# microsoft/aurora

Hardware: AMD Instinct MI355X
Metric: forecast-steps/sec (6h step) 0.25deg ERA5 721x1440x13 (higher is better)
Workload: dtype bf16; 1 GPU; AuroraPretrained(autocast=True) 1.3B, 0.25deg ERA5 721x1440, 13 levels, T=2, batch 1 per GPU, one forward step (BASELINE.json configs[1]); parallelism=1 GPU

## Files before the change

### aurora_amd/build.py

```python

from __future__ import annotations

import os
import subprocess
import sys
from pathlib import Path

PKG = Path(__file__).resolve().parent
CSRC = PKG / "csrc"
LIB = PKG / "_lib" / "libaurora_hip.so"
SOURCES = ("runtime.hip", "gemm.hip", "gemm_f32.hip", "gemm_ln512.hip", "gemm_a4.hip", "attention.hip", "norm.hip", "embed.hip", "perceiver_attention.hip", "perceiver_out.hip", "band.hip",
           "model.hip", "model_weights.hip", "model_grid.hip", "step.hip", "regrid.hip", "conservative_regrid.hip", "planes.hip", "scores.hip", "ensemble_scores.hip", "ensemble_quantiles.hip", "spectra.hip", "event_scores.hip",
           "field_stats.hip", "probability_scores.hip", "diagnostics.hip", "conditional_scores.hip", "region_scores.hip", "objects.hip", "field_quantiles.hip", "object_matches.hip", "nearest_event.hip")
ARCH = "gfx950"
COMPILE_FLAGS = (f"--offload-arch={ARCH}", "-O3", "-std=c++17", "-fPIC", "-mllvm", "-amdgpu-mfma-vgpr-form=1")


def _hipcc() -> str:
    for cand in (os.environ.get("HIPCC"), "/opt/rocm/bin/hipcc", "hipcc"):
        if cand and (os.path.isabs(cand) and os.path.exists(cand) or not os.path.isabs(cand)):
            return cand
    raise RuntimeError("hipcc not found")


def is_stale() -> bool:
    if not LIB.exists():
        return True
    built = LIB.stat().st_mtime
    deps = [d for pat in ("*.hip", "*.h", "*.inc") for d in CSRC.glob(pat)] + [PKG.parent / "include" / "aurora_hip.h"]
    return any(d.stat().st_mtime > built for d in deps)


def build_library(force: bool = False, verbose: bool = True) -> Path:
    if not force and not is_stale():
        return LIB
    LIB.parent.mkdir(parents=True, exist_ok=True)
    objs = []
    procs = []
    for src in SOURCES:
        obj = LIB.parent / (src.replace(".hip", ".o"))
        cmd = [_hipcc(), *COMPILE_FLAGS, *os.environ.get("AURORA_BUILD_FLAGS", "").split(), "-c", str(CSRC / src), "-o", str(obj)]
        if verbose:
            print(" ".join(cmd), flush=True)
        procs.append((src, subprocess.Popen(cmd, stdout=subprocess.PIPE, stderr=subprocess.STDOUT)))
        objs.append(obj)
    for src, pr in procs:
        out, _ = pr.communicate()
        if pr.returncode != 0:
            raise RuntimeError(f"hipcc failed on {src}:\n{out.decode(errors='replace')}")
    cmd = [_hipcc(), f"--offload-arch={ARCH}", "-shared", "-fPIC", *map(str, objs), "-o", str(LIB)]
    if verbose:
        print(" ".join(cmd), flush=True)
    res = subprocess.run(cmd, stdout=subprocess.PIPE, stderr=subprocess.STDOUT)
    if res.returncode != 0:
        raise RuntimeError(f"link failed:\n{res.stdout.decode(errors='replace')}")
    for o in objs:
        o.unlink(missing_ok=True)
    return LIB


if __name__ == "__main__":
    print(build_library(force="--force" in sys.argv))
```

### aurora_amd/csrc/model.h

```cpp
#pragma once

#include <math.h>
#include <stdlib.h>
#include <string.h>

#include <algorithm>
#include <array>
#include <exception>
#include <map>
#include <memory>
#include <stdexcept>
#include <string>
#include <vector>

#include "band.h"
#include "common.h"

namespace aurora {

struct Fail {
  int code;
};
#define REQUIRE(cond, ...)               \
  do {                                   \
    if (!(cond)) {                       \
      ::aurora::set_error(__VA_ARGS__);  \
      throw ::aurora::Fail{AURORA_E_ARG}; \
    }                                    \
  } while (0)
#define GUARDED(...)                                    \
  try {                                                 \
    __VA_ARGS__;                                        \
    return AURORA_OK;                                   \
  } catch (const ::aurora::Fail& f) {                   \
    return f.code;                                      \
  } catch (const std::exception& e) {                   \
    ::aurora::set_error("internal error: %s", e.what()); \
    return AURORA_E_LAUNCH;                             \
  }
inline void ok(int code) {
  if (code != AURORA_OK) throw Fail{code};
}
inline void hip_ok(hipError_t e, const char* what) {
  if (e != hipSuccess) {
    set_error("%s: %s", what, hipGetErrorString(e));
    throw Fail{AURORA_E_LAUNCH};
  }
}
inline int round_up(int x, int m) { return (x + m - 1) / m * m; }

struct DevBuf {
  void* p = nullptr;
  size_t bytes = 0;
  DevBuf() = default;
  explicit DevBuf(size_t n) : bytes(n) { hip_ok(hipMalloc(&p, n ? n : 16), "hipMalloc"); }
  DevBuf(const DevBuf&) = delete;
  DevBuf& operator=(const DevBuf&) = delete;
  DevBuf(DevBuf&& o) noexcept : p(o.p), bytes(o.bytes) { o.p = nullptr; }
  DevBuf& operator=(DevBuf&& o) noexcept {
    if (this != &o) {
      if (p) (void)hipFree(p);
      p = o.p; bytes = o.bytes; o.p = nullptr;
    }
    return *this;
  }
  ~DevBuf() { if (p) (void)hipFree(p); }
  float* f() const { return static_cast<float*>(p); }
};

struct Arena {
  char* base = nullptr;
  size_t cap = 0, top = 0, peak = 0;
  void* take(size_t bytes) {
    const size_t at = (top + 255) & ~size_t(255);
    top = at + bytes;
    if (top > peak) peak = top;
    return base + at;
  }
  ~Arena() { if (base) (void)hipFree(base); }
};

struct Tensor {
  DevBuf buf;
  std::vector<int64_t> shape;
  int64_t numel = 0;
  float* f() const { return buf.f(); }
};

struct Block {
  std::string prefix;
  int dim, stage, heads, hidden;
  bool shifted;
  const float *gain1, *shift1, *gain2, *shift2;
  const float *qkv_b, *proj_b, *fc1_b, *fc2_b;
  const void *fc1_w, *fc2_w;
};
struct AttnSet { std::vector<DevBuf> own; std::vector<const void*> qkv, proj; };
struct Resampler {
  struct Layer {
    const float *to_q, *to_kv, *to_out, *fc1_w, *fc1_b, *fc2_w, *fc2_b, *ln1_w, *ln1_b, *ln2_w, *ln2_b;
    const float *ln_k_w = nullptr, *ln_k_b = nullptr, *ln_q_w = nullptr, *ln_q_b = nullptr;
    int inner, head_dim, hidden, dim, ctx_dim;
    float v_l1;
    int f16_mode;
    const void *to_kv_s = nullptr, *to_out_s = nullptr, *fc1_s = nullptr, *fc2_s = nullptr;
  };
  std::vector<Layer> layers;
  std::vector<DevBuf> own;
  DevBuf vs_w, vs_ws;
  int n_s = 0, n_vs = 0, vs_lq = 0;
};

enum SrcKind { SRC_SURF, SRC_STATIC, SRC_DYN, SRC_ATMOS };
struct Channel {
  std::string name;
  SrcKind kind;
  int src;
  int transform;
  float tw0 = 0.f, tw1 = 0.f, tb = 0.f;
};
struct EmbedPack {
  DevBuf w, ws;
  int K = 0, Kpad = 0, groups = 1;
  float l1 = 0.f;
  std::vector<int> channels;
};
struct HeadGroup {
  std::vector<std::string> names;
  DevBuf w, b;
  int groups = 1;
  DevBuf ws, bs;
  int n_pad = 0;
};

struct DevTables { DevBuf tok, grp; int n_windows = 0, n_tok = 0; bool has_grp = false; };
struct DevPlan {
  DevBuf tok, grp, send_idx;
  int n_windows = 0, n_tok = 0, n_own = 0, n_halo = 0, n_interior = 0;
  int recv_off[2] = {0, 0}, recv_cnt[2] = {0, 0}, send_cnt[2] = {0, 0};
  bool has_grp = false;
};

}

struct aurora_hip_model {
  int D = 0, P = 0, Cl = 0, perceiver_heads = 0, n_stages = 0;
  int enc_depths[4] = {0}, dec_depths[4] = {0}, enc_heads[4] = {0}, dec_heads[4] = {0}, window[3] = {0};
  int enc_depth = 1, dec_depth = 1, max_history = 2, lora_steps = 40, lora_mode = 0;
  bool stabilise = false, use_lora = false, autocast = false;
  float ln_eps = 1e-5f;
  double timestep_hours = 6;
  std::vector<std::string> surf_vars, static_vars, atmos_vars;
  int variant = 0;
  bool dynamic_vars = false, atmos_static_vars = false, clamp_first = false, index_bug = false;
  std::vector<double> level_condition;
  std::vector<std::string> sep_perceiver, mod_heads, pos_surf, pos_atmos, surf_inputs, density_vars, angle_vars;
  std::map<std::string, int> diff_index;
  std::vector<aurora::Channel> surf_channels, atmos_channels;
  std::vector<std::string> surf_heads, surf_out;
  std::vector<std::string> atmos_heads;

  std::map<std::string, aurora::Tensor> w;
  std::map<std::string, aurora::Tensor> w16;
  bool finalized = false;
  std::vector<aurora::Block> blocks;
  aurora::DevBuf mod, lead_emb, enc_q0;
  std::vector<aurora::DevBuf> keep;
  std::map<int, aurora::AttnSet> attn_sets;
  struct Merge { const void* w; const float *ln_w, *ln_b; };
  struct Split { const void *w1, *w2; const float *ln_w, *ln_b; };
  std::vector<Merge> merges;
  std::vector<Split> splits;
  aurora::Resampler enc_rs, dec_rs, dec_rs_alt;
  bool has_alt = false;

  bool have_grid = false;
  int n_lat = 0, n_lon = 0, Hp = 0, Wp = 0, n_levels = 0;
  int full_Hp = 0;
  std::vector<double> levels;
  aurora::DevBuf pos_scale, enc_bias, dec_queries, dec_q, dec_q_alt, stats;
  std::vector<size_t> surf_stat_off, static_stat_off, atmos_stat_off;
  size_t one_stat_off = 0;
  std::vector<size_t> static_lvl_stat_off;
  std::vector<double> static_loc;
  std::map<std::array<int64_t, 3>, aurora::EmbedPack> embed_packs;
  float enc_bias_max = 0.f;
  aurora::DevBuf surf_w0_s, surf_w2_s;
  float surf_l1_0 = 0.f, surf_b0 = 0.f, surf_c = 0.f;
  bool surf_chain = false;
  aurora::HeadGroup head_surf, head_main, head_alt;
  float dec_out_bound = 0.f, dec_out_bound_alt = 0.f;
  std::map<std::pair<int, int>, aurora::DevTables> tables;
  std::vector<aurora::Res> stage_res;
  std::vector<std::array<int, 2>> merge_pad;

  aurora_hip_band band{0, 1, nullptr, nullptr, nullptr};
  std::vector<std::vector<std::array<int, 2>>> rows;
  std::map<std::pair<int, int>, aurora::DevPlan> plans;
  void* stage_send = nullptr;
  void* stage_recv = nullptr;
  int64_t staging_bytes = 0, staging_need = 0;
  bool sharded() const { return band.world > 1; }
  int fuse_ln = 1;
  bool split_attention = false;
  bool qkv_planes = true;
  bool reassoc_out = true;
  bool score_weights = true;

  aurora::DevBuf abs_enc, dyn_planes, ctx_max;
  aurora::DevBuf tickets;
  bool split_k = true;
  int abs_B = 0;
  struct Pinned { float* host = nullptr; size_t bytes = 0; hipEvent_t done = nullptr; };
  Pinned pinned[4];
  int pinned_next = 0;
  ~aurora_hip_model() {
    for (auto& t : timed) { (void)hipEventDestroy(t.e0); (void)hipEventDestroy(t.e1); }
    for (auto& e : event_pool) (void)hipEventDestroy(e);
    for (auto& s : pinned) {
      if (s.host) (void)hipHostFree(s.host);
      if (s.done) (void)hipEventDestroy(s.done);
    }
  }
  aurora::Arena arena;
  bool dry = false;
  int64_t generation = 0;

  struct Timed { int kind; double work; hipEvent_t e0, e1; };
  uint32_t profile_mask = 0;
  std::vector<Timed> timed;
  std::vector<hipEvent_t> event_pool;

  const float* W(const std::string& name) const {
    auto it = w.find(name);
    REQUIRE(it != w.end(), "missing weight '%s'", name.c_str());
    return it->second.f();
  }
  const aurora::Tensor& T_(const std::string& name) const {
    auto it = w.find(name);
    REQUIRE(it != w.end(), "missing weight '%s'", name.c_str());
    return it->second;
  }
  bool has(const std::string& name) const { return w.count(name) != 0; }
  int bb() const { return autocast ? AURORA_BF16 : AURORA_F32; }
  size_t bbs() const { return autocast ? 2 : 4; }
  int stage_dim(int s) const { return D << s; }
};

namespace aurora {

typedef aurora_hip_model Model;

enum Kind { K_LINEAR_BF16, K_LINEAR_F32, K_WINDOW_ATTENTION, K_LAYERNORM, K_MERGE_LN, K_SPLIT_LN, K_PATCHIFY,
            K_PERCEIVER_ATTENTION, K_ASSEMBLE, K_UNPATCHIFY, K_COPY2D, K_ABSMAX, K_LINEAR_LN, K_GATHER, K_PERCEIVER_OUT, K_COUNT };

hipEvent_t take_event(Model& m);

template <typename F>
void timed(Model& m, void* stream, int kind, double work, F&& fn) {
  if (m.dry) return;
  const bool on = (m.profile_mask >> kind) & 1u;
  hipEvent_t e0 = nullptr, e1 = nullptr;
  if (on) {
    e0 = take_event(m);
    e1 = take_event(m);
    hip_ok(hipEventRecord(e0, (hipStream_t)stream), "hipEventRecord");
  }
  ok(fn());
  if (on) {
    hip_ok(hipEventRecord(e1, (hipStream_t)stream), "hipEventRecord");
    m.timed.push_back({kind, work, e0, e1});
  }
}

constexpr int SPLIT_TICKETS = 4096;

struct LinearOp {
  const void *A, *W;
  const float* bias;
  void* C;
  int64_t lda, ldw, ldc, M;
  int N, K, dtype, act = AURORA_ACT_NONE, f32_gemm = -1, batch = 1;
  void* C2 = nullptr;
  const float *res = nullptr, *guard = nullptr;
  int64_t ldc2 = 0, ldr = 0, sa = 0, sw = 0, sbias = 0, sc = 0;
  float limit = 0.f;
  LinearOp(const void* A_, int64_t lda_, const void* W_, int64_t ldw_, const float* bias_, void* C_, int64_t ldc_, int64_t M_, int N_,
           int K_, int dtype_)
      : A(A_), W(W_), bias(bias_), C(C_), lda(lda_), ldw(ldw_), ldc(ldc_), M(M_), N(N_), K(K_), dtype(dtype_) {}
  LinearOp& activation(int a) { act = a; return *this; }
  LinearOp& second_output(void* c2, int64_t ld) { C2 = c2; ldc2 = ld; return *this; }
  LinearOp& residual(const float* r, int64_t ld) { res = r; ldr = ld; return *this; }
  LinearOp& f32_mode(int mode) { f32_gemm = mode; return *this; }
  LinearOp& guarded_by(const float* word, float lim) { guard = word; limit = lim; return *this; }
  LinearOp& batched(int n, int64_t a, int64_t w, int64_t b, int64_t c) { batch = n; sa = a; sw = w; sbias = b; sc = c; return *this; }
};

struct Launcher {
  Model& m;
  void* stream;
  void linear(const LinearOp& o) {
    void* ws = nullptr;
    int64_t ws_bytes = 0;
    const size_t mark = m.arena.top;
    if (m.split_k && o.dtype == AURORA_BF16 && o.batch == 1 && o.f32_gemm == -1 &&
        (ws_bytes = aurora_hip_linear_workspace(o.M, o.N, o.K, o.dtype)) > 0)
      ws = m.arena.take((size_t)ws_bytes);
    timed(m, stream, o.dtype == AURORA_BF16 ? K_LINEAR_BF16 : K_LINEAR_F32, 2.0 * (double)o.M * o.N * o.K * o.batch, [&] {
      if (ws)
        return aurora_hip_linear_ws(o.A, o.lda, o.W, o.ldw, o.bias, o.C, o.ldc, o.C2, o.ldc2, o.res, o.ldr, o.M, o.N, o.K, o.dtype,
                                    o.act, ws, ws_bytes, (int32_t*)m.tickets.p, SPLIT_TICKETS, 0, stream);
      if (o.batch > 1)
        return aurora_hip_linear_batched(o.A, o.lda, o.W, o.ldw, o.bias, o.C, o.ldc, o.M, o.N, o.K, o.dtype, o.act, o.f32_gemm,
                                         o.guard, o.limit, o.batch, o.sa, o.sw, o.sbias, o.sc, stream);
      return aurora_hip_linear_ex(o.A, o.lda, o.W, o.ldw, o.bias, o.C, o.ldc, o.C2, o.ldc2, o.res, o.ldr, o.M, o.N, o.K, o.dtype,
                                  o.act, o.f32_gemm, o.guard, o.limit, stream);
    });
    m.arena.top = mark;
  }
  void guarded_pair(LinearOp op, const void* Ws, int splits, const float* word, float limit) {
    const void* Wf = op.W;
    op.W = Ws;
    linear(op.f32_mode(2 | AURORA_F32_W_SPLIT | splits).guarded_by(word, limit));
    op.W = Wf;
    linear(op.f32_mode(1));
  }
  void linear_planes(const void* A, int64_t lda, const void* Wt, int64_t ldw, const float* bias, void* C, int64_t plane_stride,
                     int heads, int64_t M, int N, int K) {
    timed(m, stream, K_LINEAR_BF16, 2.0 * (double)M * N * K, [&] {
      return aurora_hip_linear_planes(A, lda, Wt, ldw, bias, C, plane_stride, heads, M, N, K, AURORA_BF16, stream);
    });
  }
  void layernorm(const void* y, int64_t ldy, const float* gain, const float* shift, const float* res, int64_t ldr,
                 int64_t res_mod, float* out_f32, int64_t ldo, void* out_t, int64_t ldt, int64_t M, int D, float eps,
                 int dtype) {
    timed(m, stream, K_LAYERNORM, 0.0, [&] {
      return aurora_hip_layernorm(y, ldy, gain, shift, res, ldr, res_mod, out_f32, ldo, out_t, ldt, M, D, eps, dtype, stream);
    });
  }
};

inline void upload(void* dst, const void* src, size_t bytes) {
  hip_ok(hipMemcpy(dst, src, bytes, hipMemcpyHostToDevice), "upload");
}
inline DevBuf to_device(const std::vector<float>& v) {
  DevBuf b(v.size() * sizeof(float));
  upload(b.p, v.data(), v.size() * sizeof(float));
  return b;
}
inline std::vector<float> to_host(const float* dev, size_t n) {
  std::vector<float> h(n);
  hip_ok(hipMemcpy(h.data(), dev, n * 4, hipMemcpyDeviceToHost), "download");
  return h;
}
inline std::vector<float> to_host(const Tensor& t) { return to_host(t.f(), (size_t)t.numel); }
inline bool contains(const std::vector<std::string>& v, const std::string& s) { return std::find(v.begin(), v.end(), s) != v.end(); }

constexpr float F16_SAFE = 16384.0f;
constexpr float PRESPLIT_W_MAX = 1000.0f;
int bounded_mode();
std::string level_to_str(double level);

int lora_key(const Model& m, int step);
float absmax(const float* dev, size_t n);
float absmax(const std::vector<float>& h);
inline float absmax(const Tensor& t) { return absmax(t.f(), (size_t)t.numel); }
float max_row_l1(const std::vector<float>& h, int64_t rows, int64_t K, float floor);
bool presplit_shape(int64_t rows, int64_t K, int row_multiple);
DevBuf presplit(const float* w, int64_t rows, int64_t K, int64_t ld, int row_multiple, int groups = 1);
void score_weights(Model& m, Resampler& r, const float* q0, int Lq, int heads);
void build_atmos_heads(Model& m, bool per_level);
const AttnSet& attn_weights(Model& m, int key, void* stream);
const EmbedPack& embed_pack(Model& m, int kind, int T, const std::vector<char>& present);
enum Expansion { POS, SCALE, LEAD_TIME, LEVELS, ABS_TIME };
void fourier(Expansion kind, const double* x, int64_t n, int d, float* out);
const DevTables& tables_for(Model& m, int stage, bool shifted);
const DevPlan& plan_for(Model& m, int stage, bool shifted);
struct StepIO {
  const aurora_hip_step_io* io;
  int B, T;
};
void run_step(Model& m, const StepIO& s, void* stream);

}
```

### aurora_amd/csrc/model.hip

```cpp
#include "model.h"

namespace aurora {

hipEvent_t take_event(Model& m) {
  if (!m.event_pool.empty()) {
    hipEvent_t e = m.event_pool.back();
    m.event_pool.pop_back();
    return e;
  }
  hipEvent_t e;
  hip_ok(hipEventCreate(&e), "hipEventCreate");
  return e;
}

int bounded_mode() {
  static const int mode = getenv("AURORA_F32_GEMM") ? -1 : 2;
  return mode;
}

std::string level_to_str(double level) {
  const double value = round(level * 1000.0) / 1000.0;
  char buf[64];
  if (value == (double)(long long)value) snprintf(buf, sizeof buf, "%lld", (long long)value);
  else {
// ... 23 lines not shown
      const int depth = part == 0 ? m.enc_depths[i] : m.dec_depths[i];
      const int stage = part == 0 ? i : m.n_stages - 1 - i;
      for (int j = 0; j < depth; ++j) {
        Block b{};
        b.prefix = std::string(part == 0 ? "backbone.encoder_layers." : "backbone.decoder_layers.") + std::to_string(i) +
                   ".blocks." + std::to_string(j);
        b.dim = m.stage_dim(stage);
        b.stage = stage;
        b.heads = part == 0 ? m.enc_heads[i] : m.dec_heads[i];
        b.shifted = j % 2 == 1;
        REQUIRE(b.dim == b.heads * 64, "the window-attention kernel is built for head_dim 64 (dim %d, %d heads)", b.dim,
                b.heads);
        m.blocks.push_back(b);
      }
    }
}

void build_channels(Model& m) {
  m.surf_channels.clear(); m.atmos_channels.clear(); m.surf_heads.clear(); m.surf_out.clear(); m.atmos_heads.clear();
  if (m.variant == 2) {
    std::vector<Channel> kept, appended;
    for (size_t i = 0; i < m.surf_inputs.size(); ++i) {
      const std::string& k = m.surf_inputs[i];
      const bool dens = contains(m.density_vars, k), ang = contains(m.angle_vars, k);
      if (!ang) kept.push_back({k, SRC_SURF, (int)i, dens ? 4 : 0});
      if (dens) appended.push_back({k + "_density", SRC_SURF, (int)i, 3});
      if (ang) {
        appended.push_back({k + "_sin", SRC_SURF, (int)i, 5});
        appended.push_back({k + "_cos", SRC_SURF, (int)i, 6});
      }
    }
    for (const auto& c : kept) { m.surf_channels.push_back(c); m.surf_out.push_back(c.name); }
    for (const auto& c : appended) m.surf_channels.push_back(c);
    for (const auto& c : m.surf_channels) m.surf_heads.push_back(c.name);
    for (const auto& a : m.angle_vars)
      if (contains(m.surf_heads, a + "_sin") && !contains(m.surf_out, a)) m.surf_out.push_back(a);
    for (const auto& c : m.surf_channels)
      REQUIRE(contains(m.surf_vars, c.name), "ocean wave: channel '%s' is not among the model's surf_vars", c.name.c_str());
  } else {
    for (size_t i = 0; i < m.surf_inputs.size(); ++i) {
      const std::string& k = m.surf_inputs[i];
      const int tr = contains(m.pos_surf, k) ? (m.variant == 1 ? 2 : 1) : 0;
      m.surf_channels.push_back({k, SRC_SURF, (int)i, tr});
      m.surf_heads.push_back(k);
      m.surf_out.push_back(k);
    }
    for (const auto& k : m.surf_inputs)
      if (contains(m.mod_heads, k)) m.surf_heads.push_back(k + "_mod");
  }
  for (size_t i = 0; i < m.static_vars.size(); ++i) m.surf_channels.push_back({m.static_vars[i], SRC_STATIC, (int)i, 0});
  if (m.dynamic_vars)
    for (int i = 0; i < 6; ++i) m.surf_channels.push_back({DYNAMIC_NAMES[i], SRC_DYN, i, 0});

  for (size_t i = 0; i < m.atmos_vars.size(); ++i) {
    const std::string& k = m.atmos_vars[i];
    const int tr = contains(m.pos_atmos, k) ? (m.variant == 1 ? 2 : 1) : 0;
    m.atmos_channels.push_back({k, SRC_ATMOS, (int)i, tr});
    m.atmos_heads.push_back(k);
  }
  for (const auto& k : m.atmos_vars)
    if (contains(m.mod_heads, k)) m.atmos_heads.push_back(k + "_mod");
  if (m.atmos_static_vars) {
    const std::string pre = m.dynamic_vars ? "static_" : "";
    for (size_t i = 0; i < m.static_vars.size(); ++i) m.atmos_channels.push_back({pre + m.static_vars[i], SRC_STATIC, (int)i, 0});
    if (m.dynamic_vars)
      for (int i = 0; i < 6; ++i) m.atmos_channels.push_back({pre + DYNAMIC_NAMES[i], SRC_DYN, i, 0});
  }
  if (m.index_bug) {
    int iz = -1, isz = -1;
    for (size_t i = 0; i < m.atmos_channels.size(); ++i) {
      if (m.atmos_channels[i].name == "z") iz = (int)i;
      if (m.atmos_channels[i].name == "static_z") isz = (int)i;
    }
    if (iz >= 0) {
      REQUIRE(isz >= 0, "'static_z' is not in list");
      Channel c = m.atmos_channels[iz];
      c.name = "static_z";
      m.atmos_channels[isz] = c;
    }
  }
}

}

}

using namespace aurora;

extern "C" int aurora_hip_create(const aurora_hip_config* c, aurora_hip_model** out) {
  GUARDED({
    REQUIRE(c != nullptr && out != nullptr, "create: null argument");
    REQUIRE(c->n_stages >= 1 && c->n_stages <= 4, "create: 1..4 backbone stages");
    REQUIRE(c->latent_levels > 1, "At least two latent levels are required.");
    REQUIRE(c->max_history > 0, "At least one history step is required.");
    REQUIRE(c->embed_dim % 32 == 0 && c->patch_size > 0, "create: bad embed_dim / patch_size");
    std::unique_ptr<aurora_hip_model> m(new aurora_hip_model());
    m->D = c->embed_dim; m->P = c->patch_size; m->Cl = c->latent_levels; m->perceiver_heads = c->num_heads;
    m->n_stages = c->n_stages;
    int se = 0, sd = 0;
    for (int i = 0; i < c->n_stages; ++i) {
      m->enc_depths[i] = c->encoder_depths[i]; m->dec_depths[i] = c->decoder_depths[i];
      m->enc_heads[i] = c->encoder_heads[i]; m->dec_heads[i] = c->decoder_heads[i];
      se += c->encoder_depths[i]; sd += c->decoder_depths[i];
    }
    REQUIRE(se == sd, "Encoder and decoder must have the same total depth.");
    for (int a = 0; a < 3; ++a) m->window[a] = c->window[a];
    REQUIRE(m->window[0] * m->window[1] * m->window[2] <= 144, "windows of more than 144 tokens are not supported");
    REQUIRE(m->Cl % m->window[0] == 0, "latent levels must be divisible by the window's level extent");
    m->enc_depth = c->enc_depth; m->dec_depth = c->dec_depth; m->max_history = c->max_history;
    m->ln_eps = c->perceiver_ln_eps; m->timestep_hours = c->timestep_hours;
    m->stabilise = c->stabilise_level_agg != 0; m->use_lora = c->use_lora != 0;
    m->lora_steps = c->lora_steps; m->lora_mode = c->lora_mode; m->autocast = c->autocast != 0;
    REQUIRE(m->lora_mode >= 0 && m->lora_mode <= 2, "create: lora_mode must be 0 (single), 1 (from_second) or 2 (all)");
    auto names = [](const char* const* p, int n, std::vector<std::string>& dst) {
      for (int i = 0; i < n; ++i) dst.push_back(p[i]);
    };
    names(c->surf_vars, c->n_surf, m->surf_vars);
    names(c->static_vars, c->n_static, m->static_vars);
    names(c->atmos_vars, c->n_atmos, m->atmos_vars);
    REQUIRE(!m->surf_vars.empty() && !m->atmos_vars.empty(), "create: variable lists must not be empty");
    m->variant = c->variant;
    REQUIRE(m->variant >= 0 && m->variant <= 2, "create: variant must be 0 (base), 1 (air pollution) or 2 (ocean wave)");
    for (int i = 0; i < c->n_level_condition; ++i) m->level_condition.push_back(c->level_condition[i]);
    m->dynamic_vars = c->dynamic_vars != 0; m->atmos_static_vars = c->atmos_static_vars != 0;
    m->clamp_first = c->clamp_at_first_step != 0; m->index_bug = c->simulate_indexing_bug != 0;
    names(c->separate_perceiver, c->n_separate_perceiver, m->sep_perceiver);
    names(c->modulation_heads, c->n_modulation_heads, m->mod_heads);
    names(c->positive_surf_vars, c->n_positive_surf, m->pos_surf);
    names(c->positive_atmos_vars, c->n_positive_atmos, m->pos_atmos);
    names(c->surf_inputs, c->n_surf_inputs, m->surf_inputs);
    names(c->density_channel_surf_vars, c->n_density, m->density_vars);
    names(c->angle_surf_vars, c->n_angle, m->angle_vars);
    if (m->surf_inputs.empty()) m->surf_inputs = m->surf_vars;
    REQUIRE(m->variant == 2 || m->surf_inputs == m->surf_vars, "create: surf_inputs are for the ocean-wave variant");
    if (c->difference_history)
      for (int i = 0; i < c->n_modulation_heads; ++i)
        if (c->difference_history[i] >= 0) m->diff_index[m->mod_heads[i]] = c->difference_history[i];
    REQUIRE(m->static_vars.size() <= 60 && m->surf_inputs.size() <= 60 && m->atmos_vars.size() <= 60, "create: too many variables");
    build_blocks(*m);
    build_channels(*m);
    m->ctx_max = DevBuf(16);
    const auto& tu = c->tuning;
    REQUIRE(tu.fuse_ln >= 0 && tu.fuse_ln <= 3, "create: tuning.fuse_ln = %d (0 default, 1 never, 2 by the fill rule, 3 always)", tu.fuse_ln);
    auto sw = [](int32_t v, bool dflt, const char* what) {
      REQUIRE(v >= 0 && v <= 2, "create: tuning.%s = %d (0 default, 1 off, 2 on)", what, v);
      return v == 0 ? dflt : v == 2;
    };
    m->fuse_ln = tu.fuse_ln == 0 ? 1 : tu.fuse_ln - 1;
    m->split_attention = sw(tu.band_split_attention, false, "band_split_attention");
    m->qkv_planes = sw(tu.qkv_planes, true, "qkv_planes");
    m->split_k = sw(tu.split_k, true, "split_k");
    m->reassoc_out = sw(tu.perceiver_reassoc, true, "perceiver_reassoc");
    m->score_weights = sw(tu.score_weights, true, "score_weights");
    m->tickets = DevBuf(SPLIT_TICKETS * sizeof(int32_t));
    hip_ok(hipMemset(m->tickets.p, 0, SPLIT_TICKETS * sizeof(int32_t)), "hipMemset");
    *out = m.release();
  })
}

extern "C" void aurora_hip_destroy(aurora_hip_model* m) { delete m; }

extern "C" int aurora_hip_set_band(aurora_hip_model* mp, const aurora_hip_band* band) {
  GUARDED({
    REQUIRE(mp != nullptr, "set_band: null model");
    Model& m = *mp;
    if (band == nullptr || band->world <= 1) {
      m.band = aurora_hip_band{0, 1, nullptr, nullptr, nullptr};
    } else {
      REQUIRE(band->rank >= 0 && band->rank < band->world, "set_band: rank %d of %d", band->rank, band->world);
      REQUIRE(band->post && band->wait, "set_band: the halo transport callbacks are required");
      m.band = *band;
    }
    m.have_grid = false;
    m.plans.clear(); m.rows.clear();
    m.stage_send = m.stage_recv = nullptr;
    m.staging_bytes = m.staging_need = 0;
  })
}

extern "C" int aurora_hip_band_rows(const aurora_hip_model* m, int32_t* row0, int32_t* row1) {
  GUARDED({
    REQUIRE(m && row0 && row1 && m->have_grid, "band_rows: precompute the grid first");
    const int h0 = m->sharded() ? m->rows[0][m->band.rank][0] : 0;
    *row0 = h0 * m->P;
    *row1 = (h0 + m->Hp) * m->P;
  })
}

extern "C" int64_t aurora_hip_band_staging_bytes(const aurora_hip_model* m) { return m ? m->staging_need : 0; }

extern "C" int aurora_hip_set_band_staging(aurora_hip_model* m, void* send, void* recv, int64_t staging_bytes) {
  GUARDED({
    REQUIRE(m != nullptr, "set_band_staging: null model");
    REQUIRE(staging_bytes >= m->staging_need, "set_band_staging: %lld bytes per buffer, %lld needed", (long long)staging_bytes,
            (long long)m->staging_need);
    REQUIRE(m->staging_need == 0 || (send && recv && (uintptr_t)send % 16 == 0 && (uintptr_t)recv % 16 == 0),
            "set_band_staging: two 16-byte aligned device buffers are required");
    m->stage_send = send;
    m->stage_recv = recv;
    m->staging_bytes = staging_bytes;
  })
}

extern "C" int aurora_hip_output_vars(const aurora_hip_model* m, const char** names, int capacity) {
  if (!m) return 0;
  if (names)
    for (int i = 0; i < capacity && i < (int)m->surf_out.size(); ++i) names[i] = m->surf_out[i].c_str();
  return (int)m->surf_out.size();
}

extern "C" int aurora_hip_step(aurora_hip_model* mp, const aurora_hip_step_io* io, void* stream) {
  GUARDED({
    REQUIRE(mp && io, "step: null argument");
    Model& m = *mp;
    REQUIRE(m.finalized && m.have_grid, "step: finalize the weights and precompute the grid first");
    REQUIRE(io->B >= 1 && io->T >= 1, "step: empty batch");
    REQUIRE(io->T <= m.max_history, "%d > %d.", io->T, m.max_history);
    REQUIRE(m.abs_B >= io->B, "step: call aurora_hip_set_time for this batch first");
    REQUIRE(io->surf && io->atmos && io->out_surf && io->out_atmos && (m.static_vars.empty() || io->stat), "step: null field list");
    if (m.sharded()) {
      REQUIRE(io->B == 1, "latitude-band sharding runs one forecast (batch size 1) across the ranks");
      REQUIRE(m.staging_need == 0 || m.staging_bytes >= m.staging_need, "step: hand over the band's staging buffers first "
              "(aurora_hip_set_band_staging, %lld bytes each)", (long long)m.staging_need);
    }
    StepIO s{io, io->B, io->T};
    attn_weights(m, lora_key(m, io->rollout_step), stream);
    m.dry = true;
    m.arena.peak = 0;
    try { run_step(m, s, stream); } catch (...) { m.dry = false; throw; }
    m.dry = false;
    if (m.arena.peak > m.arena.cap) {
      hipStreamCaptureStatus cap = hipStreamCaptureStatusNone;
      (void)hipStreamIsCapturing(as_stream(stream), &cap);
      REQUIRE(cap == hipStreamCaptureStatusNone, "step: the workspace must grow; run one step outside graph capture first");
      hip_ok(hipDeviceSynchronize(), "sync before growing the workspace");
      if (m.arena.base) (void)hipFree(m.arena.base);
      m.arena.base = nullptr;
      m.arena.cap = 0;
      void* p = nullptr;
      hip_ok(hipMalloc(&p, m.arena.peak), "workspace allocation");
      m.arena.base = (char*)p;
      m.arena.cap = m.arena.peak;
      m.generation += 1;
    }
    if (m.sharded() && m.split_k)
      hip_ok(hipMemsetAsync(m.tickets.p, 0, SPLIT_TICKETS * sizeof(int32_t), as_stream(stream)), "zeroing the split-K tickets");
    run_step(m, s, stream);
  })
}

namespace {
const char* const KIND_NAMES[K_COUNT] = {"linear_bf16", "linear_f32", "window_attention_bf16", "layernorm", "merge_ln",
                                         "split_ln", "patchify", "perceiver_attention", "assemble_tokens", "unpatchify",
                                         "copy2d", "absmax", "linear_layernorm_bf16", "gather_rows", "perceiver_out"};
}

extern "C" int aurora_hip_profile_begin(aurora_hip_model* m, uint32_t kind_mask) {
  GUARDED({
    REQUIRE(m != nullptr, "profile_begin: null model");
    for (auto& t : m->timed) { m->event_pool.push_back(t.e0); m->event_pool.push_back(t.e1); }
    m->timed.clear();
    m->profile_mask = kind_mask;
  })
}

extern "C" int aurora_hip_profile_end(aurora_hip_model* m, aurora_hip_profile_entry* out, int capacity, int* n_out) {
  GUARDED({
    REQUIRE(m && out && n_out && capacity >= K_COUNT, "profile_end: need room for %d entries", (int)K_COUNT);
    m->profile_mask = 0;
    hip_ok(hipDeviceSynchronize(), "profile_end");
    for (int k = 0; k < K_COUNT; ++k) out[k] = aurora_hip_profile_entry{KIND_NAMES[k], 0, 0.0, 0.0};
    for (auto& t : m->timed) {
      float ms = 0.f;
      hip_ok(hipEventElapsedTime(&ms, t.e0, t.e1), "hipEventElapsedTime");
      out[t.kind].launches += 1;
      out[t.kind].ms += ms;
      out[t.kind].work += t.work;
      m->event_pool.push_back(t.e0);
      m->event_pool.push_back(t.e1);
    }
    m->timed.clear();
    *n_out = K_COUNT;
  })
}

extern "C" int aurora_hip_profile_end_list(aurora_hip_model* m, aurora_hip_profile_entry* out, int capacity, int* n_out) {
  GUARDED({
    REQUIRE(m && n_out && (out || capacity == 0), "profile_end_list: bad arguments");
    m->profile_mask = 0;
    hip_ok(hipDeviceSynchronize(), "profile_end_list");
    *n_out = (int)m->timed.size();
    if (capacity < *n_out) return AURORA_OK;
    int i = 0;
    for (auto& t : m->timed) {
      float ms = 0.f;
      hip_ok(hipEventElapsedTime(&ms, t.e0, t.e1), "hipEventElapsedTime");
      out[i++] = aurora_hip_profile_entry{KIND_NAMES[t.kind], 1, ms, t.work};
      m->event_pool.push_back(t.e0);
      m->event_pool.push_back(t.e1);
    }
    m->timed.clear();
  })
}

extern "C" int64_t aurora_hip_generation(const aurora_hip_model* m) { return m ? m->generation : 0; }

extern "C" int aurora_hip_abi_sizes(int32_t* out, int capacity) {
  const int32_t sizes[] = {(int32_t)sizeof(aurora_hip_config), (int32_t)sizeof(aurora_hip_grid), (int32_t)sizeof(aurora_hip_step_io),
                           (int32_t)sizeof(aurora_hip_band), (int32_t)sizeof(aurora_hip_halo_msg), (int32_t)sizeof(aurora_hip_plan_info),
                           (int32_t)sizeof(aurora_patch_var), (int32_t)sizeof(aurora_unpatch_var), (int32_t)sizeof(aurora_hip_profile_entry)};
  const int n = (int)(sizeof(sizes) / sizeof(sizes[0]));
  for (int i = 0; i < n && i < capacity; ++i) out[i] = sizes[i];
  return n;
}

extern "C" int64_t aurora_hip_workspace_bytes(const aurora_hip_model* m) { return m ? (int64_t)m->arena.cap : 0; }

extern "C" int aurora_hip_guard_words(const aurora_hip_model* m, float out[4], void* stream) {
  GUARDED({
    REQUIRE(m && out && m->ctx_max.p, "guard_words: bad arguments");
    static_assert(AURORA_F16_SAFE_RANGE == F16_SAFE, "the header's constant is the step's");
    hip_ok(hipMemcpyAsync(out, m->ctx_max.p, 4 * sizeof(float), hipMemcpyDeviceToHost, (hipStream_t)stream), "guard_words");
    hip_ok(hipStreamSynchronize((hipStream_t)stream), "guard_words");
  })
}
```

### aurora_amd/csrc/model_weights.hip

```cpp
#include "model.h"

namespace aurora {

constexpr int LORA_RANK = 8;

float absmax(const std::vector<float>& h) {
  float mx = 0.f;
  for (float v : h) mx = std::max(mx, fabsf(v));
  return mx;
}
float absmax(const float* dev, size_t n) { return absmax(to_host(dev, n)); }
float max_row_l1(const std::vector<float>& h, int64_t rows, int64_t K, float floor) {
  float best = floor;
  for (int64_t r = 0; r < rows; ++r) {
    float sum = 0.f;
    for (int64_t k = 0; k < K; ++k) sum += fabsf(h[(size_t)r * K + k]);
    best = std::max(best, sum);
  }
  return best;
}

bool presplit_shape(int64_t rows, int64_t K, int row_multiple) { return rows % row_multiple == 0 && K % 32 == 0 && K >= 96; }
DevBuf presplit(const float* w, int64_t rows, int64_t K, int64_t ld, int row_multiple, int groups) {
  if (!presplit_shape(rows, K, row_multiple)) return DevBuf();
  DevBuf s((size_t)groups * rows * K * 4);
  ok(aurora_hip_split_f16(w, ld, s.p, K, groups * rows, (int)K, 64.0f, nullptr));
  hip_ok(hipDeviceSynchronize(), "split weights");
  return s;
}

namespace {

const void* compute_weight(Model& m, const std::string& name, void* stream, int64_t* out_shape0 = nullptr) {
  auto h = m.w16.find(name);
  if (h != m.w16.end()) {
    REQUIRE(m.autocast, "'%s' is stored in bf16 only: this packed file serves autocast (bf16 backbone) models", name.c_str());
    if (out_shape0) *out_shape0 = h->second.shape[0];
    return h->second.buf.p;
  }
  const Tensor& t = m.T_(name);
  if (out_shape0) *out_shape0 = t.shape[0];
  if (!m.autocast) return t.f();
  DevBuf b((size_t)t.numel * 2);
  ok(aurora_hip_convert(t.f(), b.p, t.numel, AURORA_F32, stream));
  m.keep.push_back(std::move(b));
  return m.keep.back().p;
}

Resampler pack_resampler(Model& m, const std::string& prefix, int depth, int heads) {
  Resampler r;
  for (int i = 0; i < depth; ++i) {
    const std::string p = prefix + ".layers." + std::to_string(i);
    Resampler::Layer l{};
    l.to_q = m.W(p + ".0.to_q.weight"); l.to_kv = m.W(p + ".0.to_kv.weight"); l.to_out = m.W(p + ".0.to_out.weight");
    l.fc1_w = m.W(p + ".1.net.0.weight"); l.fc1_b = m.W(p + ".1.net.0.bias");
    l.fc2_w = m.W(p + ".1.net.2.weight"); l.fc2_b = m.W(p + ".1.net.2.bias");
    l.ln1_w = m.W(p + ".2.weight"); l.ln1_b = m.W(p + ".2.bias");
    l.ln2_w = m.W(p + ".3.weight"); l.ln2_b = m.W(p + ".3.bias");
    if (m.has(p + ".0.ln_k.weight")) {
      l.ln_k_w = m.W(p + ".0.ln_k.weight"); l.ln_k_b = m.W(p + ".0.ln_k.bias");
      l.ln_q_w = m.W(p + ".0.ln_q.weight"); l.ln_q_b = m.W(p + ".0.ln_q.bias");
    }
    const Tensor& tkv = m.T_(p + ".0.to_kv.weight");
    l.inner = (int)m.T_(p + ".0.to_q.weight").shape[0];
    l.head_dim = l.inner / heads;
    l.hidden = (int)m.T_(p + ".1.net.0.weight").shape[0];
    l.dim = (int)m.T_(p + ".0.to_out.weight").shape[0];
    l.ctx_dim = (int)tkv.shape[1];
    const size_t n_v = (size_t)l.inner * l.ctx_dim;
    l.v_l1 = max_row_l1(to_host(tkv.f() + n_v, n_v), l.inner, l.ctx_dim, 1e-6f);
    const char* const linears[4] = {".0.to_kv.weight", ".0.to_out.weight", ".1.net.0.weight", ".1.net.2.weight"};
    float w_max = 0.f;
    for (const char* nm : linears) w_max = std::max(w_max, absmax(m.T_(p + nm)));
    const float ln_bound = absmax(m.T_(p + ".2.weight")) * sqrtf((float)l.dim) + absmax(m.T_(p + ".2.bias"));
    l.f16_mode = (w_max < PRESPLIT_W_MAX && ln_bound < F16_SAFE) ? bounded_mode() : -1;
    if (l.f16_mode == 2) {
      auto split = [&](const char* nm) -> const void* {
        const Tensor& t = m.T_(p + nm);
        DevBuf s = presplit(t.f(), t.shape[0], t.shape[1], t.shape[1], 256);
        if (!s.p) return nullptr;
        r.own.push_back(std::move(s));
        return r.own.back().p;
      };
      l.to_kv_s = split(linears[0]); l.to_out_s = split(linears[1]); l.fc1_s = split(linears[2]); l.fc2_s = split(linears[3]);
    }
    r.layers.push_back(l);
  }
  return r;
}

void build_heads(Model& m, HeadGroup& hg, const char* kind, const std::vector<std::string>& names, bool per_level) {
  const int PP = m.P * m.P, D2 = 2 * m.D;
  hg.names = names;
  hg.groups = per_level ? m.n_levels : 1;
  if (names.empty()) return;
  const size_t ldb = (size_t)round_up((int)names.size() * PP, 4);
  hg.w = DevBuf((size_t)hg.groups * names.size() * PP * D2 * 4);
  hg.b = DevBuf((size_t)hg.groups * ldb * 4);
  hip_ok(hipMemset(hg.b.p, 0, hg.b.bytes), "memset");
  for (int g = 0; g < hg.groups; ++g)
    for (size_t v = 0; v < names.size(); ++v) {
      std::string p = std::string("decoder.") + kind + "_heads." + names[v];
      if (per_level) p += ".layers." + level_to_str(m.levels[g]);
      const Tensor& wt = m.T_(p + ".weight");
      REQUIRE(wt.shape.size() == 2 && wt.shape[0] == PP && wt.shape[1] == D2, "bad head weight shape for %s", p.c_str());
      hip_ok(hipMemcpy(hg.w.f() + ((size_t)g * names.size() + v) * PP * D2, wt.f(), (size_t)PP * D2 * 4, hipMemcpyDeviceToDevice), "copy");
      hip_ok(hipMemcpy(hg.b.f() + (size_t)g * ldb + v * PP, m.W(p + ".bias"), (size_t)PP * 4, hipMemcpyDeviceToDevice), "copy");
    }
  hg.n_pad = 0;
  hg.ws = DevBuf(); hg.bs = DevBuf();
  const int n = (int)names.size() * PP, n_pad = round_up(n, 128);
  if (std::string(kind) != "atmos" || bounded_mode() != 2 || !presplit_shape(n_pad, D2, 128)) return;
  if (!(absmax(hg.w.f(), (size_t)hg.groups * n * D2) < PRESPLIT_W_MAX)) return;
  DevBuf padded((size_t)hg.groups * n_pad * D2 * 4);
  hip_ok(hipMemset(padded.p, 0, padded.bytes), "memset");
  hg.bs = DevBuf((size_t)hg.groups * n_pad * 4);
  hip_ok(hipMemset(hg.bs.p, 0, hg.bs.bytes), "memset");
  for (int g = 0; g < hg.groups; ++g) {
    hip_ok(hipMemcpy(padded.f() + (size_t)g * n_pad * D2, hg.w.f() + (size_t)g * n * D2, (size_t)n * D2 * 4, hipMemcpyDeviceToDevice), "copy");
    hip_ok(hipMemcpy(hg.bs.f() + (size_t)g * n_pad, hg.b.f() + (size_t)g * ldb, (size_t)n * 4, hipMemcpyDeviceToDevice), "copy");
  }
  hg.ws = presplit(padded.f(), n_pad, D2, D2, 128, hg.groups);
  hg.n_pad = n_pad;
}

}

void score_weights(Model& m, Resampler& r, const float* q0, int Lq, int heads) {
  r.vs_w = DevBuf();
  r.vs_ws = DevBuf();
  r.n_s = r.n_vs = r.vs_lq = 0;
  if (!m.score_weights || r.layers.empty() || q0 == nullptr) return;
  const auto& l = r.layers[0];
  if (l.ln_k_w != nullptr || l.head_dim * heads != l.inner || l.f16_mode < 0) return;
  const int inner = l.inner, hd = l.head_dim, K = l.ctx_dim, n_s = Lq * heads;
  const int n_vs = round_up(inner + n_s, 256);
  if (n_vs >= 2 * inner) return;
  std::vector<float> wkv((size_t)2 * inner * K), q((size_t)Lq * inner), vs((size_t)n_vs * K, 0.f);
  hip_ok(hipMemcpy(wkv.data(), l.to_kv, wkv.size() * 4, hipMemcpyDeviceToHost), "download");
  hip_ok(hipMemcpy(q.data(), q0, q.size() * 4, hipMemcpyDeviceToHost), "download");
  std::copy(wkv.begin() + (size_t)inner * K, wkv.end(), vs.begin());
  const double scale = 1.0 / std::sqrt((double)hd);
  std::vector<double> acc((size_t)K);
  float s_max = 0.f;
  for (int lq = 0; lq < Lq; ++lq)
    for (int h = 0; h < heads; ++h) {
      std::fill(acc.begin(), acc.end(), 0.0);
      for (int d = 0; d < hd; ++d) {
        const double qd = q[(size_t)lq * inner + h * hd + d];
        const float* wr = wkv.data() + (size_t)(h * hd + d) * K;
        for (int c = 0; c < K; ++c) acc[c] += qd * wr[c];
      }
      float* dst = vs.data() + (size_t)(inner + lq * heads + h) * K;
      for (int c = 0; c < K; ++c) {
        dst[c] = (float)(acc[c] * scale);
        s_max = std::max(s_max, fabsf(dst[c]));
      }
    }
  if (!(s_max < PRESPLIT_W_MAX)) return;
  DevBuf w = to_device(vs), ws;
  if (l.to_kv_s != nullptr && l.f16_mode == 2) ws = presplit(w.f(), n_vs, K, K, 256);
  if ((l.to_kv_s != nullptr) != (ws.p != nullptr)) return;
  r.vs_w = std::move(w); r.vs_ws = std::move(ws);
  r.n_s = n_s; r.n_vs = n_vs; r.vs_lq = Lq;
}

const AttnSet& attn_weights(Model& m, int key, void* stream) {
  auto it = m.attn_sets.find(key);
  if (it != m.attn_sets.end()) return it->second;
  AttnSet set;
  for (const Block& blk : m.blocks) {
    for (int which = 0; which < 2; ++which) {
      const std::string name = blk.prefix + (which == 0 ? ".attn.qkv" : ".attn.proj");
      if (key < 0 && m.w16.count(name + ".weight")) {
        (which == 0 ? set.qkv : set.proj).push_back(compute_weight(m, name + ".weight", stream));
        continue;
      }
      const Tensor& wt = m.T_(name + ".weight");
      const int64_t out_f = wt.shape[0], in_f = wt.shape[1];
      const float* src = wt.f();
      DevBuf merged;
      if (key >= 0) {
        const std::string lp = blk.prefix + (which == 0 ? ".attn.lora_qkv.loras." : ".attn.lora_proj.loras.") + std::to_string(key);
        const Tensor& a = m.T_(lp + ".lora_A");
        const Tensor& b = m.T_(lp + ".lora_B");
        std::vector<float> ha((size_t)a.numel), hb((size_t)b.numel);
        hip_ok(hipMemcpy(ha.data(), a.f(), ha.size() * 4, hipMemcpyDeviceToHost), "download");
        hip_ok(hipMemcpy(hb.data(), b.f(), hb.size() * 4, hipMemcpyDeviceToHost), "download");
        std::vector<float> at((size_t)in_f * 32, 0.f), bp((size_t)out_f * 32, 0.f);
        for (int r_ = 0; r_ < LORA_RANK; ++r_)
          for (int64_t k = 0; k < in_f; ++k) at[(size_t)k * 32 + r_] = ha[(size_t)r_ * in_f + k];
        for (int64_t o = 0; o < out_f; ++o)
          for (int r_ = 0; r_ < LORA_RANK; ++r_) bp[(size_t)o * 32 + r_] = hb[(size_t)o * LORA_RANK + r_];
        DevBuf d_at = to_device(at), d_bp = to_device(bp);
        merged = DevBuf((size_t)out_f * in_f * 4);
        ok(aurora_hip_linear_ex(d_bp.p, 32, d_at.p, 32, nullptr, merged.p, in_f, nullptr, 0, src, in_f, out_f, (int)in_f, 32,
                                AURORA_F32, AURORA_ACT_NONE, -1, nullptr, 0.f, stream));
        hip_ok(hipStreamSynchronize(as_stream(stream)), "sync");
        src = merged.f();
      }
      const void* use = src;
      if (m.autocast) {
        DevBuf h((size_t)out_f * in_f * 2);
        ok(aurora_hip_convert(src, h.p, out_f * in_f, AURORA_F32, stream));
        hip_ok(hipStreamSynchronize(as_stream(stream)), "sync");
        use = h.p;
        set.own.push_back(std::move(h));
      } else if (key >= 0) {
        set.own.push_back(std::move(merged));
      }
      (which == 0 ? set.qkv : set.proj).push_back(use);
    }
  }
  while (m.attn_sets.size() > 3) {
    bool erased = false;
    for (auto jt = m.attn_sets.begin(); jt != m.attn_sets.end(); ++jt)
      if (jt->first != -1) { m.attn_sets.erase(jt); erased = true; break; }
    if (!erased) break;
  }
  return m.attn_sets.emplace(key, std::move(set)).first->second;
}

const EmbedPack& embed_pack(Model& m, int kind, int T, const std::vector<char>& present) {
  const std::vector<Channel>& chans = kind == 0 ? m.surf_channels : m.atmos_channels;
  int64_t mask = 0, mask_hi = 0;
  REQUIRE(chans.size() <= 126, "more than 126 input channels");
  for (size_t i = 0; i < chans.size(); ++i)
    if (present[i]) (i < 63 ? mask : mask_hi) |= (int64_t)1 << (i % 63);
  const std::array<int64_t, 3> key{(int64_t)kind * 1024 + T, mask, mask_hi};
  auto it = m.embed_packs.find(key);
  if (it != m.embed_packs.end()) return it->second;
  EmbedPack pk;
  for (size_t i = 0; i < chans.size(); ++i)
    if (present[i]) pk.channels.push_back((int)i);
  REQUIRE(!pk.channels.empty(), "no %s variable given", kind == 0 ? "surface-level" : "atmospheric");
  const bool per_level = kind == 1 && !m.level_condition.empty();
  pk.groups = per_level ? m.n_levels : 1;
  const int V = (int)pk.channels.size(), PP = m.P * m.P;
  pk.K = V * T * PP;
  pk.Kpad = round_up(pk.K, 32);
  std::vector<float> host((size_t)pk.groups * m.D * pk.Kpad, 0.f);
  for (int g = 0; g < pk.groups; ++g) {
    const std::string prefix = kind == 0 ? "encoder.surf_token_embeds.weights."
                               : per_level ? "encoder.atmos_token_embeds.layers." + level_to_str(m.levels[g]) + ".weights."
                                           : "encoder.atmos_token_embeds.weights.";
    for (int v = 0; v < V; ++v) {
      const Tensor& t = m.T_(prefix + chans[pk.channels[v]].name);
      REQUIRE(t.shape.size() == 5 && t.shape[0] == m.D && t.shape[2] >= T && t.shape[3] == m.P, "bad patch-embed weight shape");
      const int64_t Tmax = t.shape[2];
      const std::vector<float> wv = to_host(t);
      for (int d = 0; d < m.D; ++d)
        for (int tt = 0; tt < T; ++tt)
          memcpy(&host[((size_t)g * m.D + d) * pk.Kpad + ((size_t)v * T + tt) * PP], &wv[((size_t)d * Tmax + tt) * PP], PP * sizeof(float));
    }
  }
  pk.l1 = max_row_l1(host, (int64_t)pk.groups * m.D, pk.Kpad, 1e-6f);
  pk.w = to_device(host);
  if (bounded_mode() == 2 && absmax(host) < PRESPLIT_W_MAX)
    pk.ws = presplit(pk.w.f(), m.D, pk.Kpad, pk.Kpad, 256, pk.groups);
  return m.embed_packs.emplace(key, std::move(pk)).first->second;
}

void build_atmos_heads(Model& m, bool per_level) {
  std::vector<std::string> sep = m.sep_perceiver, main_names, alt_names;
  if (!m.mod_heads.empty())
    for (const auto& v : m.sep_perceiver) sep.push_back(v + "_mod");
  for (const auto& n : m.atmos_heads) (contains(sep, n) ? alt_names : main_names).push_back(n);
  build_heads(m, m.head_main, "atmos", main_names, per_level);
  build_heads(m, m.head_alt, "atmos", alt_names, per_level);
}

namespace {

void surface_mlp_chain(Model& m) {
  const Tensor &t0 = m.T_("encoder.surf_mlp.net.0.weight"), &t2 = m.T_("encoder.surf_mlp.net.2.weight");
  const std::vector<float> w0 = to_host(t0), w2 = to_host(t2);
// ... 217 lines not shown
```

### aurora_amd/csrc/step.hip

```cpp
#include <algorithm>

#include "model.h"
#include "resampler_space.h"

namespace aurora {

namespace {

struct CtxGuard { const float* word; float a, c, limit_kv; bool pairs; };

LayerSpace layer_space(const Model& m, const Resampler& rs, size_t i, int B, int64_t cols, int64_t ctx_rows, int Lq, int Lk,
                       int heads) {
  const auto& ly = rs.layers[i];
  LayerShape sh{};
  sh.layer = i;
  sh.dim = ly.dim; sh.inner = ly.inner; sh.hidden = ly.hidden; sh.head_dim = ly.head_dim; sh.heads = heads;
  sh.n_vs = rs.n_vs; sh.vs_lq = rs.vs_lq;
  sh.ln_k = ly.ln_k_w != nullptr; sh.to_out_s = ly.to_out_s != nullptr; sh.fc1_s = ly.fc1_s != nullptr; sh.fc2_s = ly.fc2_s != nullptr;
  sh.f16_mode = ly.f16_mode;
  sh.reassoc_out = m.reassoc_out;
  sh.out_supported = aurora_hip_perceiver_out_supported(Lq, Lk, heads, ly.head_dim, ly.dim) != 0;
  sh.B = B; sh.cols = cols; sh.ctx_rows = ctx_rows; sh.Lq = Lq; sh.Lk = Lk;
  return layer_space(sh);
}

void resampler_mlp(Model& m, Launcher& L, const Resampler::Layer& ly, const LayerSpace& sp, const float* o, const float* res,
                   int64_t res_mod, float* lat1, char* S, float* y, int64_t n_rows, float eps, bool y_pairs) {
  const int Dd = ly.dim;
  if (sp.pairs)
    timed(m, L.stream, K_LAYERNORM, 0.0, [&] {
      return aurora_hip_layernorm_split(o, Dd, ly.ln1_w, ly.ln1_b, res, Dd, res_mod, 0, nullptr, 0, lat1, Dd, n_rows, Dd, eps, L.stream);
    });
  else L.layernorm(o, Dd, ly.ln1_w, ly.ln1_b, res, Dd, res_mod, lat1, Dd, nullptr, 0, n_rows, Dd, eps, AURORA_F32);
  float* hid = (float*)S;
  const int64_t chunk_rows = sp.chunk_rows;
  REQUIRE(chunk_rows >= 1 && (size_t)chunk_rows * sp.hid_row <= sp.s_bytes, "resampler: scratch region too small for the MLP");
  const int all = 2 | AURORA_F32_A_SPLIT | AURORA_F32_W_SPLIT;
  for (int64_t r0 = 0; r0 < n_rows; r0 += chunk_rows) {
    const int64_t nr = std::min(chunk_rows, n_rows - r0);
    LinearOp fc1(lat1 + (size_t)r0 * Dd, Dd, sp.pairs ? ly.fc1_s : ly.fc1_w, Dd, ly.fc1_b, hid, ly.hidden, nr, ly.hidden, Dd, AURORA_F32);
    LinearOp fc2(hid, ly.hidden, sp.pairs ? ly.fc2_s : ly.fc2_w, ly.hidden, ly.fc2_b, y + (size_t)r0 * Dd, Dd, nr, Dd, ly.hidden, AURORA_F32);
    L.linear(fc1.activation(AURORA_ACT_GELU).f32_mode(sp.pairs ? all | AURORA_F32_C_SPLIT : ly.f16_mode));
    L.linear(fc2.f32_mode(sp.pairs ? all : ly.f16_mode));
  }
  if (sp.pairs)
    timed(m, L.stream, K_LAYERNORM, 0.0, [&] {
      return aurora_hip_layernorm_split(y, Dd, ly.ln2_w, ly.ln2_b, lat1, Dd, 0, 1, y_pairs ? nullptr : y, Dd, y_pairs ? y : nullptr, Dd,
                                        n_rows, Dd, eps, L.stream);
    });
  else L.layernorm(y, Dd, ly.ln2_w, ly.ln2_b, lat1, Dd, 0, y, Dd, nullptr, 0, n_rows, Dd, eps, AURORA_F32);
}

float* resampler(Model& m, Launcher& L, const Resampler& rs, const float* ctx, int64_t ctx_rows, int ctx_dim, const float* q0,
                 const float* latents0, int B, int64_t cols, int64_t kv_bstride, int64_t kv_lstride, int Lq, int Lk, int heads,
                 float eps, const CtxGuard* cg = nullptr, bool out_pairs = false, int own_word = 0, bool scan_ctx = true) {
  const int64_t n_cols = (int64_t)B * cols, n_rows = n_cols * Lq;
  const float* ctx_max = cg ? cg->word : m.ctx_max.f() + own_word;
  const float g_a = cg ? cg->a : 1.0f, g_c = cg ? cg->c : 0.0f;
  const bool ctx_pairs = cg && cg->pairs;
  if (!cg && scan_ctx)
    timed(m, L.stream, K_ABSMAX, 0.0, [&] { return aurora_hip_absmax_fold(ctx, ctx_rows * ctx_dim, m.ctx_max.f() + own_word, L.stream); });
  float* lat = nullptr;
  for (size_t i = 0; i < rs.layers.size(); ++i) {
    const auto& ly = rs.layers[i];
    const int inner = ly.inner, Dd = ly.dim;
    const LayerSpace sp = layer_space(m, rs, i, B, cols, ctx_rows, Lq, Lk, heads);
    const bool scores = sp.scores;
    const int kv_ld = sp.kv_ld;
    float* y = (float*)m.arena.take(sp.unit);
    const size_t after_y = m.arena.top;
    float* lat1 = (float*)m.arena.take(sp.unit);
    char* S = (char*)m.arena.take(sp.s_bytes);
    float* kv = (float*)S;
    auto guarded = [&](const float* A, int64_t lda, const float* Wf, const void* Ws, float* C_, int64_t ldc, int64_t M_, int N_,
                       int K_, float limit, bool a_pairs = false) {
      LinearOp op(A, lda, Wf, K_, nullptr, C_, ldc, M_, N_, K_, AURORA_F32);
      if (Ws) {
        L.guarded_pair(op, Ws, a_pairs ? AURORA_F32_A_SPLIT : 0, ctx_max, limit);
      } else if (ly.f16_mode == 2) {
        L.linear(op.f32_mode(2).guarded_by(ctx_max, limit));
      } else {
        L.linear(op.f32_mode(ly.f16_mode));
      }
    };
    REQUIRE(!ctx_pairs || ly.to_kv_s, "resampler: a pair-layout context needs pre-split to_kv weights");
    guarded(ctx, ctx_dim, scores ? rs.vs_w.f() : ly.to_kv, scores ? rs.vs_ws.p : ly.to_kv_s, kv, kv_ld, ctx_rows, kv_ld, ctx_dim,
            ctx_pairs ? cg->limit_kv : (F16_SAFE - g_c) / g_a, ctx_pairs);
    if (ly.ln_k_w)
      L.layernorm(kv, 2 * inner, ly.ln_k_w, ly.ln_k_b, nullptr, 0, 0, kv, 2 * inner, nullptr, 0, ctx_rows, inner, 1e-5f,
                  AURORA_F32);
    const float* q = q0;
    int64_t q_stride = 0;
    if (i > 0) {
      float* qb = (float*)(S + round256(sp.kv_bytes));
      L.linear(LinearOp(lat, Dd, ly.to_q, Dd, nullptr, qb, inner, n_rows, inner, Dd, AURORA_F32));
      if (ly.ln_q_w) L.layernorm(qb, inner, ly.ln_q_w, ly.ln_q_b, nullptr, 0, 0, qb, inner, nullptr, 0, n_rows, inner, 1e-5f, AURORA_F32);
      q = qb;
      q_stride = Lq;
    }
    float* att = sp.att_in_y ? y : (float*)(S + sp.att_off);
    const float lim_out = (F16_SAFE / ly.v_l1 - g_c) / g_a;
    float* o = (float*)S;
    if (sp.reassoc) {
      REQUIRE(sp.p_off >= sp.kv_bytes && sp.p_off >= sp.unit && sp.p_off + sp.p_bytes <= sp.s_bytes,
              "resampler: the softmax weights overlap k | v or to_out's result in the scratch region");
      float* P = (float*)(S + sp.p_off);
      void* Vp = y;
      timed(m, L.stream, K_PERCEIVER_ATTENTION, 0.0, [&] {
        if (scores)
          return aurora_hip_perceiver_probs_scores(kv, kv_ld, inner, P, Vp, B, cols, kv_bstride, kv_lstride, Lq, Lk, heads, ly.head_dim,
                                                   ctx_max, lim_out, L.stream);
        return aurora_hip_perceiver_probs(q, kv, P, Vp, B, cols, kv_bstride, kv_lstride, Lq, Lk, heads, ly.head_dim, ctx_max, lim_out,
                                          L.stream);
      });
      timed(m, L.stream, K_PERCEIVER_OUT, 2.0 * (double)n_cols * Lk * Dd * inner + 2.0 * (double)n_rows * Dd * heads * Lk, [&] {
        return aurora_hip_perceiver_out(Vp, ly.to_out_s, inner, P, nullptr, o, Dd, n_cols, Lq, Lk, heads, ly.head_dim, Dd, ctx_max,
                                        lim_out, L.stream);
      });
      timed(m, L.stream, K_PERCEIVER_ATTENTION, 0.0, [&] {
        if (scores)
          return aurora_hip_perceiver_attention_scores(kv, kv_ld, inner, att, B, cols, kv_bstride, kv_lstride, Lq, Lk, heads,
                                                       ly.head_dim, nullptr, 0.f, ctx_max, lim_out, L.stream);
        return aurora_hip_perceiver_attention_unless(q, q_stride, kv, att, B, cols, kv_bstride, kv_lstride, Lq, Lk, heads,
                                                     ly.head_dim, AURORA_F32, nullptr, 0.f, ctx_max, lim_out, L.stream);
      });
      L.linear(LinearOp(att, inner, ly.to_out, inner, nullptr, o, Dd, n_rows, Dd, inner, AURORA_F32).f32_mode(1).guarded_by(ctx_max, lim_out));
    } else {
      timed(m, L.stream, K_PERCEIVER_ATTENTION, 0.0, [&] {
        if (scores)
          return aurora_hip_perceiver_attention_scores(kv, kv_ld, inner, att, B, cols, kv_bstride, kv_lstride, Lq, Lk, heads,
                                                       ly.head_dim, sp.att_pairs ? ctx_max : nullptr, lim_out, nullptr, 0.f, L.stream);
        return aurora_hip_perceiver_attention_ex(q, q_stride, kv, att, B, cols, kv_bstride, kv_lstride, Lq, Lk, heads, ly.head_dim,
                                                 AURORA_F32, sp.att_pairs ? ctx_max : nullptr, lim_out, L.stream);
      });
      guarded(att, inner, ly.to_out, ly.to_out_s, o, Dd, n_rows, Dd, inner, lim_out, sp.att_pairs);
    }
    resampler_mlp(m, L, ly, sp, o, i == 0 ? latents0 : lat, i == 0 ? Lq : 0, lat1, S, y, n_rows, eps,
                  out_pairs && sp.pairs && i + 1 == rs.layers.size());
    m.arena.top = after_y;
    lat = y;
  }
  return lat;
}

inline int index_of(const std::vector<std::string>& v, const std::string& s) {
  const auto it = std::find(v.begin(), v.end(), s);
  return it == v.end() ? -1 : (int)(it - v.begin());
}

aurora_patch_var channel_desc(const Model& m, const aurora_hip_step_io& io, const Channel& ch, bool atmos_level, int C) {
  const float* st = m.stats.f();
  aurora_patch_var d{};
  d.transform = ch.transform; d.tw0 = ch.tw0; d.tw1 = ch.tw1; d.tb = ch.tb;
  switch (ch.kind) {
    case SRC_SURF:
      d.src = io.surf[ch.src];
      d.stride_b = io.surf_strides[0]; d.stride_t = io.surf_strides[1]; d.stride_h = io.surf_strides[2]; d.stride_w = io.surf_strides[3];
      d.loc = st + m.surf_stat_off[ch.src]; d.inv_scale = d.loc + 2;
      break;
    case SRC_STATIC:
      d.src = io.stat[ch.src];
      d.stride_h = io.static_strides[0]; d.stride_w = io.static_strides[1];
      if (atmos_level) { d.loc = st + m.static_lvl_stat_off[ch.src]; d.inv_scale = d.loc + 2 * C; }
      else { d.loc = st + m.static_stat_off[ch.src]; d.inv_scale = d.loc + 2; }
      break;
    case SRC_DYN:
      d.src = m.dyn_planes.f() + (size_t)ch.src * m.abs_B;
      d.stride_b = 1;
      d.loc = st + m.one_stat_off; d.inv_scale = d.loc + 2 * C;
      break;
    case SRC_ATMOS:
      d.src = io.atmos[ch.src];
      d.stride_b = io.atmos_strides[0]; d.stride_t = io.atmos_strides[1]; d.stride_c = io.atmos_strides[2];
      d.stride_h = io.atmos_strides[3]; d.stride_w = io.atmos_strides[4];
      d.loc = st + m.atmos_stat_off[ch.src]; d.inv_scale = d.loc + 2 * C;
      break;
  }
  return d;
}

bool channel_present(const aurora_hip_step_io& io, const Channel& ch) {
  switch (ch.kind) {
    case SRC_SURF: return io.surf[ch.src] != nullptr;
    case SRC_STATIC: return io.stat != nullptr && io.stat[ch.src] != nullptr;
    case SRC_ATMOS: return io.atmos[ch.src] != nullptr;
    default: return true;
  }
}

struct Step {
  Model& m;
  Launcher L;
  const aurora_hip_step_io& io;
  int B, T, P, D, Hp, Wp, Cl, C, PP;
  int64_t Lp;
  bool sharded;
  int rank, world;
  bool clamp_now, bf;
  int bb;
  size_t es;
  Res local_res(int stage) const {
    Res r = m.stage_res[stage];
    if (sharded) r.h = m.rows[stage][rank][1] - m.rows[stage][rank][0];
    return r;
  }
};

template <typename V, typename F>
void in_launches_of_32(Step& s, int kind, const std::vector<V>& descs, F&& launch) {
  for (size_t i = 0; i < descs.size(); i += 32)
    timed(s.m, s.L.stream, kind, 0.0, [&] { return launch(descs.data() + i, (int)std::min<size_t>(32, descs.size() - i), (int)i); });
}

const EmbedPack& embed_input(Step& s, bool atmos, float*& A) {
  const std::vector<Channel>& channels = atmos ? s.m.atmos_channels : s.m.surf_channels;
  std::vector<char> present(channels.size());
  for (size_t i = 0; i < present.size(); ++i) present[i] = channel_present(s.io, channels[i]);
  const EmbedPack& p = embed_pack(s.m, atmos ? 1 : 0, s.T, present);
  A = (float*)s.m.arena.take((size_t)(atmos ? s.C : 1) * s.B * s.Lp * p.Kpad * 4);
  return p;
}
void patchify(Step& s, const EmbedPack& p, bool atmos, float* A, float* word) {
  const std::vector<Channel>& channels = atmos ? s.m.atmos_channels : s.m.surf_channels;
  std::vector<aurora_patch_var> descs;
  for (int ci : p.channels) descs.push_back(channel_desc(s.m, s.io, channels[ci], atmos, s.C));
  in_launches_of_32(s, K_PATCHIFY, descs, [&](const aurora_patch_var* d, int n, int i0) {
    return aurora_hip_patchify_absmax(d, n, A, p.Kpad, i0 * s.T * s.PP, p.K, s.B, s.T, atmos ? s.C : 1, s.Hp, s.Wp, s.P, AURORA_F32, word,
                                      s.L.stream);
  });
}

const float* encode_surface(Step& s) {
  Model& m = s.m;
  Launcher& L = s.L;
  Arena& A = m.arena;
  const int D = s.D;
  const int64_t R = s.B * s.Lp;
  float* A_s;
  const EmbedPack& ps = embed_input(s, false, A_s);
  const int Kpad_s = ps.Kpad;
  const bool surf_guarded = m.surf_chain && ps.ws.p != nullptr;
  float* word = m.ctx_max.f() + 2;
  patchify(s, ps, false, A_s, surf_guarded ? word : nullptr);
  float* xs0 = (float*)A.take((size_t)R * D * 4);
  const int hid_s = (int)m.T_("encoder.surf_mlp.net.0.weight").shape[0];
  float* hid = (float*)A.take((size_t)R * hid_s * 4);
  float* y = (float*)A.take((size_t)R * D * 4);
  const LinearOp embed = LinearOp(A_s, Kpad_s, ps.w.f(), Kpad_s, m.W("encoder.surf_token_embeds.bias"), xs0, D, R, D, Kpad_s, AURORA_F32)
                             .residual(m.W("encoder.surf_level_encoding"), 0);
  const LinearOp fc1 = LinearOp(xs0, D, m.W("encoder.surf_mlp.net.0.weight"), D, m.W("encoder.surf_mlp.net.0.bias"), hid, hid_s, R, hid_s,
                                D, AURORA_F32).activation(AURORA_ACT_GELU);
  const LinearOp fc2(hid, hid_s, m.W("encoder.surf_mlp.net.2.weight"), hid_s, m.W("encoder.surf_mlp.net.2.bias"), y, D, R, D, hid_s, AURORA_F32);
  if (surf_guarded) {
    const float l1e = ps.l1;
    const float lim_e = F16_SAFE, lim_0 = (F16_SAFE - m.surf_c) / l1e, lim_2 = ((F16_SAFE - m.surf_b0) / m.surf_l1_0 - m.surf_c) / l1e;
    L.guarded_pair(embed, ps.ws.p, 0, word, lim_e);
    L.guarded_pair(fc1, m.surf_w0_s.p, 0, word, lim_0);
    L.guarded_pair(fc2, m.surf_w2_s.p, 0, word, lim_2);
  } else {
    L.linear(embed);
    L.linear(fc1);
    L.linear(fc2);
  }
  L.layernorm(y, D, m.W("encoder.surf_norm.weight"), m.W("encoder.surf_norm.bias"), xs0, D, 0, y, D, nullptr, 0, R, D, 1e-5f,
              AURORA_F32);
  return y;
}

const float* encode_levels(Step& s) {
  Model& m = s.m;
  Launcher& L = s.L;
  const int B = s.B, D = s.D, C = s.C;
  float* A_a;
  const EmbedPack& pa = embed_input(s, true, A_a);
  const int Kpad_a = pa.Kpad;
  bool chain = pa.ws.p != nullptr;
  for (const auto& ly : m.enc_rs.layers) chain = chain && ly.f16_mode == 2 && ly.to_kv_s != nullptr;
  float* word = m.ctx_max.f() + 1;
  patchify(s, pa, true, A_a, chain ? word : nullptr);
  float* xa = (float*)m.arena.take((size_t)C * B * s.Lp * D * 4);
  const int64_t R = (int64_t)B * s.Lp;
  CtxGuard cg{};
  const int64_t sw = pa.groups > 1 ? (int64_t)D * Kpad_a : 0;
  const LinearOp embed = LinearOp(A_a, Kpad_a, pa.w.f(), Kpad_a, m.enc_bias.f(), xa, D, R, D, Kpad_a, AURORA_F32)
                             .batched(C, R * Kpad_a, sw, D, R * D);
  if (chain) {
    const float l1 = pa.l1, cb = m.enc_bias_max;
    cg = CtxGuard{word, l1, cb, std::min(F16_SAFE, (F16_SAFE - cb) / l1), true};
    L.guarded_pair(embed, pa.ws.p, AURORA_F32_C_SPLIT, cg.word, cg.limit_kv);
  } else {
    L.linear(embed);
  }
// ... 163 lines not shown

void merge_stage(Step& s, int i, float*& xf, void*& xb) {
  Model& m = s.m;
  Arena& A = m.arena;
  const Res g = m.stage_res[i], r = s.local_res(i);
  REQUIRE(g.h > 1 && g.w > 1, "grid (%d, %d, %d) too small to merge", g.c, g.h, g.w);
  const int dim = m.stage_dim(i);
  const int H2 = (r.h + 1) / 2, W2 = (r.w + 1) / 2;
  REQUIRE(H2 == s.local_res(i + 1).h, "band rows of stages %d / %d do not nest", i, i + 1);
  const int64_t M2 = (int64_t)s.B * r.c * H2 * W2;
  float* nf = (float*)A.take((size_t)M2 * 2 * dim * 4);
  void* nb = s.bf ? A.take((size_t)M2 * 2 * dim * 2) : nullptr;
  const size_t mark = A.top;
  void* mg = A.take((size_t)M2 * 4 * dim * s.es);
  timed(m, s.L.stream, K_MERGE_LN, 0.0, [&] {
    return aurora_hip_merge_ln(xf, m.merges[i].ln_w, m.merges[i].ln_b, mg, s.B, r.c, r.h, r.w, dim, 1e-5f, s.bb, s.L.stream);
  });
  LinearOp reduce(mg, 4 * dim, m.merges[i].w, 4 * dim, nullptr, s.bf ? nb : (void*)nf, 2 * dim, M2, 2 * dim, 4 * dim, s.bb);
  if (s.bf) reduce.second_output(nf, 2 * dim);
  s.L.linear(reduce);
  A.top = mark;
  xf = nf;
  xb = nb;
}

void split_stage(Step& s, int i, const std::vector<float*>& skips, float*& xf, void*& xb) {
  Model& m = s.m;
  Arena& A = m.arena;
  const int n = m.n_stages, idx = n - 1 - i, B = s.B;
  const Res r = s.local_res(idx);
  const int dim = m.stage_dim(idx);
  const void* a_in = s.bf ? xb : (const void*)xf;
  const int crop_h = (s.sharded && s.rank != s.world - 1) ? 0 : m.merge_pad[idx - 1][0], crop_w = m.merge_pad[idx - 1][1];
  const int Ho = 2 * r.h - crop_h, Wo = 2 * r.w - crop_w;
  REQUIRE(Ho == s.local_res(idx - 1).h && Wo == s.local_res(idx - 1).w, "band rows of stages %d / %d do not nest", idx - 1, idx);
  const int64_t M1 = (int64_t)B * r.c * r.h * r.w, M2 = (int64_t)B * r.c * Ho * Wo;
  float* nf = (float*)A.take((size_t)M2 * (dim / 2) * 4);
  void* nb = s.bf ? A.take((size_t)M2 * (dim / 2) * 2) : nullptr;
  const size_t mark = A.top;
  void* y1 = A.take((size_t)M1 * 2 * dim * s.es);
  s.L.linear(LinearOp(a_in, dim, m.splits[i].w1, dim, nullptr, y1, 2 * dim, M1, 2 * dim, dim, s.bb));
  void* sp = A.take((size_t)M2 * (dim / 2) * s.es);
  timed(m, s.L.stream, K_SPLIT_LN, 0.0, [&] {
    return aurora_hip_split_ln(y1, m.splits[i].ln_w, m.splits[i].ln_b, sp, B, r.c, r.h, r.w, dim / 2, crop_h, crop_w, 1e-5f, s.bb,
                               s.L.stream);
  });
  const float* res_ = (i > 0 && i < n - 1) ? skips[idx - 1] : nullptr;
  LinearOp expand(sp, dim / 2, m.splits[i].w2, dim / 2, nullptr, s.bf ? nb : (void*)nf, dim / 2, M2, dim / 2, dim / 2, s.bb);
  if (s.bf) expand.second_output(nf, dim / 2);
  s.L.linear(expand.residual(res_, dim / 2));
  A.top = mark;
  xf = nf;
  xb = nb;
}

aurora_unpatch_var plain_unpatch(float* dst, const float* loc, int n_lvl, bool clamp_min0, int col0) {
  aurora_unpatch_var d{};
  d.dst = dst; d.loc = loc; d.scale = loc + n_lvl; d.clamp_min0 = clamp_min0; d.col0 = col0;
  d.mod_col0 = d.angle_col0 = d.dens_col0 = -1;
  return d;
}

void diff_fields(const Step& s, aurora_unpatch_var& d, const std::string& name, const std::vector<std::string>& heads, bool atmos,
                 int src, int n_lvl) {
  const Model& m = s.m;
  const aurora_hip_step_io& io = s.io;
  const auto it = m.diff_index.find(name);
  const int mod = index_of(heads, name + "_mod");
  if (m.variant != 1 || it == m.diff_index.end() || mod < 0) return;
  d.mod_col0 = mod * s.PP;
  const int idx = it->second;
  if (atmos) {
    d.prev = io.atmos[src] + (int64_t)idx * io.atmos_strides[1];
    d.prev_sb = io.atmos_strides[0]; d.prev_sc = io.atmos_strides[2]; d.prev_sh = io.atmos_strides[3];
    REQUIRE(io.atmos_strides[4] == 1, "difference prediction needs unit longitude stride");
  } else {
    d.prev = io.surf[src] + (int64_t)idx * io.surf_strides[1];
    d.prev_sb = io.surf_strides[0]; d.prev_sc = 0; d.prev_sh = io.surf_strides[2];
    REQUIRE(io.surf_strides[3] == 1, "difference prediction needs unit longitude stride");
  }
  REQUIRE(idx < s.T, "difference prediction of '%s' refers to history index %d, %d states given", name.c_str(), idx, s.T);
  d.inv_scale = d.loc + 2 * n_lvl;
}

aurora_unpatch_var surf_unpatch(const Step& s, const HeadGroup& hs, size_t v, int src) {
  const Model& m = s.m;
  const aurora_hip_step_io& io = s.io;
  const std::string& name = m.surf_out[v];
  aurora_unpatch_var d = plain_unpatch(io.out_surf[v], m.stats.f() + m.surf_stat_off[src], 1, s.clamp_now && index_of(m.pos_surf, name) >= 0, 0);
  const int plain = index_of(hs.names, name);
  if (m.variant == 2 && plain < 0) {
    d.col0 = index_of(hs.names, name + "_sin") * s.PP;
    d.angle_col0 = index_of(hs.names, name + "_cos") * s.PP;
  } else {
    REQUIRE(plain >= 0, "no decoder head for '%s'", name.c_str());
    d.col0 = plain * s.PP;
  }
  diff_fields(s, d, name, hs.names, false, src, 1);
  const int dens = m.variant == 2 ? index_of(hs.names, name + "_density") : -1;
  if (dens >= 0) {
    const int wmb = index_of(m.static_vars, "wmb");
    REQUIRE(wmb >= 0 && io.stat && io.stat[wmb], "the ocean-wave variant needs the static variable 'wmb'");
    REQUIRE(io.static_strides[1] == 1, "the water-body mask needs unit longitude stride");
    d.dens_col0 = dens * s.PP;
    d.mask = io.stat[wmb];
    d.mask_sh = io.static_strides[0];
    d.mask_thresh = (float)m.static_loc[wmb];
  }
  return d;
}

aurora_unpatch_var atmos_unpatch(const Step& s, const HeadGroup& hg, size_t hi, int v) {
  const Model& m = s.m;
  const std::string& name = hg.names[hi];
  aurora_unpatch_var d = plain_unpatch(s.io.out_atmos[v], m.stats.f() + m.atmos_stat_off[v], s.C,
                                       s.clamp_now && index_of(m.pos_atmos, name) >= 0, (int)hi * s.PP);
  diff_fields(s, d, name, hg.names, true, v, s.C);
  if (m.variant == 1 && m.use_lora && name == "so2")
    for (int c = 0; c < s.C; ++c)
      if (m.levels[c] >= 850) d.clamp_max1_levels |= 1u << c;
  return d;
}

void decode_surface(Step& s, const float* x_cat) {
  Model& m = s.m;
  const int B = s.B, D2 = 2 * s.D;
  const int64_t Lp = s.Lp;
  const HeadGroup& hs = m.head_surf;
  const int n_s = (int)hs.names.size() * s.PP, ld_s = round_up(n_s, 4);
  float* y_s = (float*)m.arena.take((size_t)B * Lp * ld_s * 4);
  for (int b = 0; b < B; ++b)
    s.L.linear(LinearOp(x_cat + (size_t)b * s.Cl * Lp * D2, D2, hs.w.f(), D2, hs.b.f(), y_s + (size_t)b * Lp * ld_s, ld_s, Lp, n_s, D2,
                        AURORA_F32));
  std::vector<aurora_unpatch_var> ud;
  for (size_t v = 0; v < m.surf_out.size(); ++v) {
    const int src = index_of(m.surf_inputs, m.surf_out[v]);
    REQUIRE(src >= 0, "surface output '%s' is not a surface input", m.surf_out[v].c_str());
    if (s.io.out_surf[v] == nullptr || s.io.surf[src] == nullptr) continue;
    ud.push_back(surf_unpatch(s, hs, v, src));
  }
  in_launches_of_32(s, K_UNPATCHIFY, ud, [&](const aurora_unpatch_var* d, int n, int) {
    return aurora_hip_unpatchify(y_s, ld_s, d, n, B, 1, s.Hp, s.Wp, s.P, s.L.stream);
  });
}

void decode_group(Step& s, const HeadGroup& hg, const Resampler& rs, const float* q, float out_bound, bool scan_ctx, const float* ctx) {
  Model& m = s.m;
  const int B = s.B, C = s.C, Cl = s.Cl, D2 = 2 * s.D;
  const int64_t Lp = s.Lp;
  const size_t gmark = m.arena.top;
  const auto& last_ly = rs.layers.back();
  const bool last_pairs = last_ly.fc1_s && last_ly.fc2_s && last_ly.dim % 32 == 0;
  const bool two_term = hg.n_pad > 0 && last_pairs && out_bound < F16_SAFE;
  float* lat = resampler(m, s.L, rs, ctx, (int64_t)B * (Cl - 1) * Lp, D2, q, m.dec_queries.f(), B, Lp, (int64_t)(Cl - 1) * Lp, Lp, C,
                         Cl - 1, m.perceiver_heads, m.ln_eps, nullptr, two_term, 3, scan_ctx);
  const int n_a = two_term ? hg.n_pad : (int)hg.names.size() * s.PP, ld_a = round_up(n_a, 4);
  const float* hw = two_term ? (const float*)hg.ws.p : hg.w.f();
  const float* hb = two_term ? hg.bs.f() : hg.b.f();
  const int mode = two_term ? (2 | AURORA_F32_A_SPLIT | AURORA_F32_W_SPLIT) : -1;
  float* y_a = (float*)m.arena.take((size_t)B * Lp * C * ld_a * 4);
  if (hg.groups > 1)
    s.L.linear(LinearOp(lat, (int64_t)C * D2, hw, D2, hb, y_a, (int64_t)C * ld_a, (int64_t)B * Lp, n_a, D2, AURORA_F32)
                   .f32_mode(mode).batched(C, D2, (int64_t)n_a * D2, ld_a, ld_a));
  else
    s.L.linear(LinearOp(lat, D2, hw, D2, hb, y_a, ld_a, (int64_t)B * Lp * C, n_a, D2, AURORA_F32).f32_mode(mode));
  std::vector<aurora_unpatch_var> ad;
  for (size_t hi = 0; hi < hg.names.size(); ++hi) {
    const int v = index_of(m.atmos_vars, hg.names[hi]);
    if (v < 0) continue;
    if (s.io.out_atmos[v] == nullptr || s.io.atmos[v] == nullptr) continue;
    ad.push_back(atmos_unpatch(s, hg, hi, v));
  }
  in_launches_of_32(s, K_UNPATCHIFY, ad, [&](const aurora_unpatch_var* d, int n, int) {
    return aurora_hip_unpatchify(y_a, ld_a, d, n, B, C, s.Hp, s.Wp, s.P, s.L.stream);
  });
  m.arena.top = gmark;
}

void decode_levels(Step& s, const float* x_cat) {
  Model& m = s.m;
  const int B = s.B, Cl = s.Cl, D2 = 2 * s.D;
  const int64_t Lp = s.Lp;
  const float* ctx = x_cat + (size_t)Lp * D2;
  if (B > 1) {
    float* ctx_copy = (float*)m.arena.take((size_t)B * (Cl - 1) * Lp * D2 * 4);
    for (int b = 0; b < B; ++b)
      timed(m, s.L.stream, K_COPY2D, 0.0, [&] {
        return aurora_hip_copy2d(x_cat + ((size_t)b * Cl * Lp + Lp) * D2, D2, ctx_copy + (size_t)b * (Cl - 1) * Lp * D2, D2,
                                 (int64_t)(Cl - 1) * Lp, D2, AURORA_F32, s.L.stream);
      });
    ctx = ctx_copy;
  }
  if (!m.head_main.names.empty()) decode_group(s, m.head_main, m.dec_rs, m.dec_q.f(), m.dec_out_bound, true, ctx);
  if (m.has_alt && !m.head_alt.names.empty())
    decode_group(s, m.head_alt, m.dec_rs_alt, m.dec_q_alt.f(), m.dec_out_bound_alt, m.head_main.names.empty(), ctx);
}

}

void run_step(Model& m, const StepIO& sio, void* stream) {
  const aurora_hip_step_io& io = *sio.io;
  const int new_step = io.rollout_step + 1;
  Step s{m, Launcher{m, stream}, io, sio.B, sio.T, m.P, m.D, m.Hp, m.Wp, m.Cl, m.n_levels, m.P * m.P, (int64_t)m.Hp * m.Wp,
         m.sharded(), m.band.rank, m.band.world,
         m.clamp_first ? new_step >= 1 : new_step > 1,
         m.autocast, m.bb(), m.bbs()};
  Arena& A = m.arena;
  A.top = 0;
  const int B = s.B, D = s.D, n = m.n_stages;
  const int64_t L0 = (int64_t)s.Cl * s.Lp;
  if (!m.dry) ok(aurora_hip_zero_words(m.ctx_max.f(), 4, stream));

  float* xf = (float*)A.take((size_t)B * L0 * D * 4);
  void* xb = s.bf ? A.take((size_t)B * L0 * D * 2) : nullptr;
  const size_t after_x = A.top;
  const float* xs1 = encode_surface(s);
  const float* lat = encode_levels(s);
  assemble(s, xs1, lat, xf, xb);
  A.top = after_x;

  const AttnSet& aw = attn_weights(m, lora_key(m, io.rollout_step), stream);
  float* x_cat = (float*)A.take((size_t)B * L0 * 2 * D * 4);
  std::vector<float*> skips;
  size_t bi = 0;
  for (int i = 0; i < n; ++i) {
    for (int k = 0; k < m.enc_depths[i]; ++k, ++bi) block(s, m.blocks[bi], aw.qkv[bi], aw.proj[bi], i, xf, xb, nullptr, 0);
    skips.push_back(xf);
    if (i < n - 1) merge_stage(s, i, xf, xb);
  }
  for (int i = 0; i < n; ++i) {
    const bool last_layer = i == n - 1;
    for (int k = 0; k < m.dec_depths[i]; ++k, ++bi)
      block(s, m.blocks[bi], aw.qkv[bi], aw.proj[bi], n - 1 - i, xf, xb, last_layer && k == m.dec_depths[i] - 1 ? x_cat : nullptr, 2 * D);
    if (last_layer && m.dec_depths[i] == 0 && !m.dry) ok(aurora_hip_copy2d(xf, D, x_cat, 2 * D, (int64_t)B * L0, D, AURORA_F32, stream));
    if (i < n - 1) split_stage(s, i, skips, xf, xb);
  }
  timed(m, stream, K_COPY2D, 0.0, [&] { return aurora_hip_copy2d(skips[0], D, x_cat + D, 2 * D, (int64_t)B * L0, D, AURORA_F32, stream); });

  const size_t mark = A.top;
  decode_surface(s, x_cat);
  decode_levels(s, x_cat);
  A.top = mark;
}

}
```

### aurora_amd/engine/lib.py

```python

from __future__ import annotations

import ctypes
import os
import threading
from collections import OrderedDict, namedtuple
from ctypes import c_float, c_int, c_int32, c_int64, c_void_p
from pathlib import Path
from typing import Optional

import numpy as np
import torch

F32, BF16, F64 = 0, 1, 2
ACT_NONE, ACT_GELU, ACT_SILU = 0, 1, 2

_LIB_PATH = Path(__file__).resolve().parents[1] / "_lib" / "libaurora_hip.so"


class PatchVar(ctypes.Structure):
    _fields_ = [
        ("src", c_void_p), ("stride_b", c_int64), ("stride_t", c_int64), ("stride_c", c_int64),
        ("stride_h", c_int64), ("stride_w", c_int64), ("loc", c_void_p), ("inv_scale", c_void_p),
        ("transform", c_int32), ("tw0", c_float), ("tw1", c_float), ("tb", c_float),
    ]


class UnpatchVar(ctypes.Structure):
    _fields_ = [("dst", c_void_p), ("loc", c_void_p), ("scale", c_void_p),
                ("clamp_min0", c_int32), ("col0", c_int32), ("lvl_stride", c_int32), ("mod_col0", c_int32),
                ("prev", c_void_p), ("prev_sb", c_int64), ("prev_sc", c_int64), ("prev_sh", c_int64),
                ("inv_scale", c_void_p), ("clamp_max1_levels", ctypes.c_uint32),
                ("angle_col0", c_int32), ("dens_col0", c_int32), ("mask", c_void_p), ("mask_sh", c_int64),
                ("mask_thresh", c_float)]


def unpatch_var(dst: int, loc: int, scale: int, clamp_min0: int, col0: int) -> UnpatchVar:
    d = UnpatchVar(dst, loc, scale, clamp_min0, col0)
    d.mod_col0 = d.angle_col0 = d.dens_col0 = -1
    return d


_SIGNATURES = {
    "aurora_hip_version": (c_int, []),
    "aurora_hip_last_error": (ctypes.c_char_p, []),
    "aurora_hip_default_f32_gemm": (c_int, []),
    "aurora_hip_linear_ex": (c_int, [c_void_p, c_int64, c_void_p, c_int64, c_void_p, c_void_p, c_int64,
                                     c_void_p, c_int64, c_void_p, c_int64, c_int64, c_int, c_int, c_int,
                                     c_int, c_int, c_void_p, c_float, c_void_p]),
    "aurora_hip_linear_workspace": (c_int64, [c_int64, c_int, c_int, c_int]),
    "aurora_hip_linear_ws": (c_int, [c_void_p, c_int64, c_void_p, c_int64, c_void_p, c_void_p, c_int64, c_void_p, c_int64,
                                     c_void_p, c_int64, c_int64, c_int, c_int, c_int, c_int, c_void_p, c_int64, c_void_p,
                                     c_int, c_int, c_void_p]),
    "aurora_hip_linear_batched": (c_int, [c_void_p, c_int64, c_void_p, c_int64, c_void_p, c_void_p, c_int64, c_int64, c_int,
                                          c_int, c_int, c_int, c_int, c_void_p, c_float, c_int, c_int64, c_int64, c_int64,
                                          c_int64, c_void_p]),
    "aurora_hip_linear_plan": (c_int, [c_int64, c_int, c_int, c_int, c_int, c_int, c_int, c_int64, c_int64, c_int64, c_int64,
                                       c_int64, c_int64, c_int64, c_int, c_int, c_int64, c_int, c_int,
                                       ctypes.POINTER(c_int32)]),
    "aurora_hip_absmax": (c_int, [c_void_p, c_int64, c_void_p, c_void_p]),
    "aurora_hip_absmax_fold": (c_int, [c_void_p, c_int64, c_void_p, c_void_p]),
    "aurora_hip_zero_words": (c_int, [c_void_p, c_int, c_void_p]),
    "aurora_hip_linear_layernorm": (c_int, [c_void_p, c_int64, c_void_p, c_int64, c_void_p, c_void_p, c_void_p, c_void_p,
                                            c_int64, c_void_p, c_int64, c_void_p, c_int64, c_int64, c_int, c_int, c_float,
                                            c_void_p]),
    "aurora_hip_split_f16": (c_int, [c_void_p, c_int64, c_void_p, c_int64, c_int64, c_int, c_float, c_void_p]),
    "aurora_hip_layernorm_split": (c_int, [c_void_p, c_int64, c_void_p, c_void_p, c_void_p, c_int64, c_int64, c_int,
                                           c_void_p, c_int64, c_void_p, c_int64, c_int64, c_int, c_float, c_void_p]),
    "aurora_hip_linear": (c_int, [c_void_p, c_int64, c_void_p, c_int64, c_void_p, c_void_p, c_int64,
                                  c_void_p, c_int64, c_void_p, c_int64, c_int64, c_int, c_int, c_int,
                                  c_int, c_void_p]),
    "aurora_hip_window_attention": (c_int, [c_void_p, c_void_p, c_void_p, c_void_p, c_void_p, c_int,
                                            c_int64, c_int64, c_int, c_int, c_int, c_int, c_int, c_void_p]),
    "aurora_hip_window_attention_planes": (c_int, [c_void_p, c_int64, c_void_p, c_void_p, c_void_p, c_void_p, c_int,
                                                   c_int64, c_int64, c_int, c_int, c_int, c_int, c_int, c_void_p]),
    "aurora_hip_linear_planes": (c_int, [c_void_p, c_int64, c_void_p, c_int64, c_void_p, c_void_p, c_int64, c_int, c_int64,
                                         c_int, c_int, c_int, c_void_p]),
    "aurora_hip_gather_rows": (c_int, [c_void_p, c_int64, c_void_p, c_void_p, c_int64, c_int64, c_int64,
                                       c_void_p]),
    "aurora_hip_layernorm": (c_int, [c_void_p, c_int64, c_void_p, c_void_p, c_void_p, c_int64, c_int64,
                                     c_void_p, c_int64, c_void_p, c_int64, c_int64, c_int, c_float,
                                     c_int, c_void_p]),
    "aurora_hip_merge_ln": (c_int, [c_void_p, c_void_p, c_void_p, c_void_p, c_int, c_int, c_int, c_int,
                                    c_int, c_float, c_int, c_void_p]),
    "aurora_hip_split_ln": (c_int, [c_void_p, c_void_p, c_void_p, c_void_p, c_int, c_int, c_int, c_int,
                                    c_int, c_int, c_int, c_float, c_int, c_void_p]),
    "aurora_hip_patchify": (c_int, [ctypes.POINTER(PatchVar), c_int, c_void_p, c_int64, c_int, c_int,
                                    c_int, c_int, c_int, c_int, c_int, c_int, c_int, c_void_p]),
    "aurora_hip_patchify_absmax": (c_int, [ctypes.POINTER(PatchVar), c_int, c_void_p, c_int64, c_int, c_int,
                                           c_int, c_int, c_int, c_int, c_int, c_int, c_int, c_void_p, c_void_p]),
    "aurora_hip_perceiver_attention": (c_int, [c_void_p, c_int64, c_void_p, c_void_p, c_int, c_int64,
                                               c_int64, c_int64, c_int, c_int, c_int, c_int, c_int,
                                               c_void_p]),
    "aurora_hip_perceiver_attention_ex": (c_int, [c_void_p, c_int64, c_void_p, c_void_p, c_int, c_int64,
                                                  c_int64, c_int64, c_int, c_int, c_int, c_int, c_int,
                                                  c_void_p, c_float, c_void_p]),
    "aurora_hip_perceiver_attention_unless": (c_int, [c_void_p, c_int64, c_void_p, c_void_p, c_int, c_int64,
                                                      c_int64, c_int64, c_int, c_int, c_int, c_int, c_int,
                                                      c_void_p, c_float, c_void_p, c_float, c_void_p]),
    "aurora_hip_perceiver_out_supported": (c_int, [c_int, c_int, c_int, c_int, c_int]),
    "aurora_hip_perceiver_probs": (c_int, [c_void_p, c_void_p, c_void_p, c_void_p, c_int, c_int64, c_int64, c_int64,
                                           c_int, c_int, c_int, c_int, c_void_p, c_float, c_void_p]),
    "aurora_hip_perceiver_attention_scores": (c_int, [c_void_p, c_int64, c_int, c_void_p, c_int, c_int64, c_int64, c_int64,
                                                      c_int, c_int, c_int, c_int, c_void_p, c_float, c_void_p, c_float,
                                                      c_void_p]),
    "aurora_hip_perceiver_probs_scores": (c_int, [c_void_p, c_int64, c_int, c_void_p, c_void_p, c_int, c_int64, c_int64,
                                                  c_int64, c_int, c_int, c_int, c_int, c_void_p, c_float, c_void_p]),
    "aurora_hip_perceiver_out": (c_int, [c_void_p, c_void_p, c_int64, c_void_p, c_void_p, c_void_p, c_int64, c_int64,
                                         c_int, c_int, c_int, c_int, c_int, c_void_p, c_float, c_void_p]),
    "aurora_hip_assemble_tokens": (c_int, [c_void_p, c_void_p, c_void_p, c_void_p, c_void_p, c_void_p,
                                           c_int, c_int, c_int64, c_int, c_int, c_void_p]),
    "aurora_hip_unpatchify": (c_int, [c_void_p, c_int64, ctypes.POINTER(UnpatchVar), c_int, c_int,
                                      c_int, c_int, c_int, c_int, c_void_p]),
    "aurora_hip_copy2d": (c_int, [c_void_p, c_int64, c_void_p, c_int64, c_int64, c_int64, c_int,
                                  c_void_p]),
    "aurora_hip_convert": (c_int, [c_void_p, c_void_p, c_int64, c_int, c_void_p]),
    "aurora_hip_regrid_plan": (c_int, [c_void_p, c_int, c_void_p, c_int, c_void_p, c_int, c_void_p, c_int, c_void_p,
                                       c_void_p, c_void_p, c_void_p]),
    "aurora_hip_regrid": (c_int, [c_void_p, c_int, c_void_p, c_int, c_int, c_int, c_void_p, c_void_p, c_int, c_void_p,
                                  c_void_p, c_int, c_void_p]),
    "aurora_hip_conservative_regrid": (c_int, [c_void_p, c_int, c_void_p, c_int, c_int, c_int, c_int, c_int, c_void_p, c_void_p,
                                               c_void_p, c_void_p, c_void_p, c_void_p, c_void_p, c_void_p, ctypes.c_double,
                                               c_void_p]),
    "aurora_hip_scores_workspace_bytes": (ctypes.c_size_t, [c_int, c_int, c_int]),
    "aurora_hip_scores": (c_int, [c_void_p, c_void_p, c_void_p, c_int, c_int, c_int, c_void_p, c_void_p, c_void_p, c_void_p]),
    "aurora_hip_ensemble_scores_workspace_bytes": (ctypes.c_size_t, [c_int, c_int, c_int, c_int]),
    "aurora_hip_ensemble_scores": (c_int, [c_void_p, c_void_p, c_int, c_int, c_int, c_int, c_void_p, c_void_p, c_void_p, c_void_p,
                                           c_void_p]),
    "aurora_hip_ensemble_quantiles": (c_int, [c_void_p, c_void_p, c_int, c_int, c_int, c_int, c_void_p, c_int, c_void_p, c_void_p,
                                              c_void_p]),
    "aurora_hip_spectra_workspace_bytes": (ctypes.c_size_t, [c_int, c_int, c_int, c_int, c_int]),
    "aurora_hip_spectra": (c_int, [c_void_p, c_void_p, c_int, c_int, c_int, c_int, c_void_p, c_void_p, c_void_p, c_void_p,
                                   c_void_p, ctypes.c_size_t, c_void_p]),
    "aurora_hip_event_scores_workspace_bytes": (ctypes.c_size_t, [c_int, c_int, c_int, c_int, c_int]),
    "aurora_hip_event_scores": (c_int, [c_void_p, c_void_p, c_int, c_int, c_int, c_void_p, c_int, c_void_p, c_int, c_int,
                                        c_void_p, c_void_p, c_void_p, ctypes.c_size_t, c_void_p]),
    "aurora_hip_field_stats_update": (c_int, [c_void_p, c_void_p, c_void_p, c_int, c_int, c_int64, c_void_p, c_int, c_int,
                                              c_void_p, c_void_p, c_void_p, c_void_p, c_void_p, c_void_p, c_void_p, c_void_p,
                                              c_void_p, c_void_p, c_void_p, c_void_p, c_void_p]),
    "aurora_hip_probability_scores": (c_int, [c_void_p, c_void_p, c_int, c_int, c_int, c_int, c_void_p, c_int, c_int, c_void_p,
                                              c_void_p]),
    "aurora_hip_diagnostics": (c_int, [c_void_p, c_void_p, c_void_p, c_void_p, c_void_p, c_int, c_void_p, ctypes.c_double, c_int,
                                       c_void_p, c_void_p, c_void_p, c_void_p, c_void_p, c_void_p, c_void_p, c_int, c_int,
                                       c_void_p, c_int, c_int, c_void_p]),
    "aurora_hip_conditional_scores_workspace_bytes": (ctypes.c_size_t, [c_int, c_int, c_int, c_int]),
    "aurora_hip_conditional_scores": (c_int, [c_void_p, c_void_p, c_void_p, c_void_p, c_int, c_int, c_int, c_void_p, c_int, c_int,
                                              c_void_p, c_void_p, c_void_p, c_void_p]),
    "aurora_hip_region_scores_workspace_bytes": (ctypes.c_size_t, [c_int, c_int, c_int, c_int]),
    "aurora_hip_region_scores": (c_int, [c_void_p, c_void_p, c_void_p, c_int, c_int, c_int, c_void_p, c_void_p, c_void_p, c_int,
                                         c_void_p, c_void_p, c_void_p, c_void_p]),
    "aurora_hip_objects_workspace_bytes": (ctypes.c_size_t, [c_int, c_int, c_int, c_int]),
    "aurora_hip_objects": (c_int, [c_void_p, c_int, c_int, c_int, c_void_p, c_int, c_void_p, c_int, c_int, c_int, c_int, c_void_p,
                                   c_void_p, c_void_p, c_void_p, ctypes.c_size_t, c_void_p]),
    "aurora_hip_field_quantiles_workspace_bytes": (ctypes.c_size_t, [c_int, c_int]),
    "aurora_hip_field_quantiles": (c_int, [c_void_p, c_int, c_int, c_int, c_void_p, c_void_p, c_int, c_void_p, c_void_p, c_void_p,
                                           c_void_p, ctypes.c_size_t, c_void_p]),
    "aurora_hip_object_matches_workspace_bytes": (ctypes.c_size_t, [c_int64, c_int]),
    "aurora_hip_object_matches": (c_int, [c_void_p, c_void_p, c_int64, c_int, c_int, c_void_p, c_int, c_int, c_int, c_void_p,
                                          c_void_p, c_void_p, ctypes.c_size_t, c_void_p]),
    "aurora_hip_nearest_event_workspace_bytes": (ctypes.c_size_t, [c_int64, c_int, c_int]),
    "aurora_hip_nearest_event": (c_int, [c_void_p, c_int64, c_int, c_int, c_void_p, c_int, ctypes.c_double, c_void_p, c_void_p,
                                         c_void_p, ctypes.c_size_t, c_void_p]),
    "aurora_hip_object_separations": (c_int, [c_void_p, c_void_p, c_void_p, c_void_p, c_int64, c_int, c_int, c_int, c_void_p,
                                              c_void_p, c_void_p]),
}

EXPORTED_SYMBOLS = tuple(_SIGNATURES)

_lib: Optional[ctypes.CDLL] = None


def library_path() -> Path:
    return _LIB_PATH


def load() -> ctypes.CDLL:
    global _lib
    if _lib is None:
        if not _LIB_PATH.exists():
            raise RuntimeError(
                f"{_LIB_PATH} is missing: build it with `python -m aurora_amd.build` "
                "(hipcc, gfx950). aurora_amd has no fallback compute path."
            )
        lib = ctypes.CDLL(os.environ.get("AURORA_HIP_LIB") or str(_LIB_PATH))
        for name, (res, args) in _SIGNATURES.items():
            fn = getattr(lib, name)
            fn.restype, fn.argtypes = res, args
        _lib = lib
    return _lib


class HipError(RuntimeError):
    pass


def _check(code: int) -> None:
    if code != 0:
        msg = load().aurora_hip_last_error().decode(errors="replace")
        raise (ValueError if code == -1 else HipError)(f"libaurora_hip: {msg} (code {code})")


def dtype_code(dt: torch.dtype) -> int:
    if dt == torch.float32:
        return F32
    if dt == torch.bfloat16:
        return BF16
    raise TypeError(f"unsupported compute dtype {dt}: the HIP engine computes in fp32 or bf16")


def _ptr(t: Optional[torch.Tensor]) -> Optional[int]:
    if t is None:
        return None
    assert t.is_cuda, "tensor must live on the HIP device"
    return t.data_ptr()


def _stream() -> int:
    return torch.cuda.current_stream().cuda_stream


def _rows(t: torch.Tensor) -> tuple[int, int]:
# ... 152 lines not shown
    assert a.dtype == w.dtype == out.dtype and tickets.dtype == torch.int32 and workspace.is_contiguous()
    ldc, _ = _rows(out)
    ldc2 = ldr = 0
    if out2 is not None:
        ldc2, _ = _rows(out2)
    if residual is not None:
        ldr, _ = _rows(residual)
    with _Timed("linear_bf16" if a.dtype == torch.bfloat16 else "linear_f32", 2.0 * M * N * K):
        _check(load().aurora_hip_linear_ws(_ptr(a), lda, _ptr(w), ldw, _ptr(bias), _ptr(out), ldc, _ptr(out2), ldc2,
                                           _ptr(residual), ldr, M, N, K, dtype_code(a.dtype), act, _ptr(workspace),
                                           workspace.numel() * workspace.element_size(), _ptr(tickets), tickets.numel(), split,
                                           _stream()))
    return out


def linear_batched(a: torch.Tensor, w: torch.Tensor, bias: Optional[torch.Tensor], out: torch.Tensor, *,
                   act: int = ACT_NONE) -> torch.Tensor:
    assert a.dim() == w.dim() == out.dim() == 3 and a.dtype == w.dtype == out.dtype, (a.dtype, w.dtype, out.dtype)
    G, M, N, K = out.shape[0], a.shape[1], w.shape[1], a.shape[2]
    assert w.shape[2] == K and out.shape[1] == M and out.shape[2] == N
    for t in (a, w):
        assert t.shape[0] in (1, G) and t.stride(2) == 1, (t.shape, t.stride())
    assert out.stride(2) == 1
    bstride = lambda t: 0 if t.shape[0] == 1 else t.stride(0)
    lda, _ = _rows(a[0])
    ldw, _ = _rows(w[0])
    ldc, _ = _rows(out[0])
    sb = 0
    if bias is not None:
        assert bias.dtype == torch.float32 and bias.dim() == 2 and bias.shape[0] in (1, G) and bias.shape[1] >= N
        assert bias.stride(1) == 1
        sb = bstride(bias)
    name = "linear_bf16" if a.dtype == torch.bfloat16 else "linear_f32"
    with _Timed(name, 2.0 * G * M * N * K):
        mode, guard, limit = _f32_state()
        _check(load().aurora_hip_linear_batched(_ptr(a), lda, _ptr(w), ldw, _ptr(bias), _ptr(out), ldc, M, N, K,
                                                dtype_code(a.dtype), act, mode, _ptr(guard), limit, G, bstride(a),
                                                bstride(w), sb, bstride(out), _stream()))
    return out


PLAN_KERNELS = ("f32_three", "f32_two", "f32_pp", "f32_pp_w", "f32_pp_aw", "f32_pp_w_tall", "f32_pp_aw_tall", "tile128",
                "ring", "ring_mid", "pp", "pp_splitk", "a4")
LinearPlan = namedtuple("LinearPlan", "kernel twin bm bn ksplit vec_store")


def linear_plan(M: int, N: int, K: int, dtype: torch.dtype, *, f32_gemm: int = -1, guard: bool = False, batch: int = 1,
                ldc: Optional[int] = None, c_offset: int = 0, ldc2: Optional[int] = None, c2_offset: int = 0,
                ldr: Optional[int] = None, residual_offset: int = 0, workspace_bytes: int = -1, n_tickets: int = 0,
                split: int = 0, plane_stride: int = 0, plane_heads: int = 0, cus: int = 0) -> LinearPlan:
    out = (c_int32 * 6)()
    _check(load().aurora_hip_linear_plan(M, N, K, dtype_code(dtype), f32_gemm, int(guard), batch, N if ldc is None else ldc,
                                         16 + c_offset, ldc2 or 0, 0 if ldc2 is None else 16 + c2_offset, ldr or 0,
                                         0 if ldr is None else 16 + residual_offset, workspace_bytes, n_tickets, split,
                                         plane_stride, plane_heads, cus, out))
    return LinearPlan(PLAN_KERNELS[out[0]], bool(out[1]), out[2], out[3], out[4], bool(out[5]))


def linear_layernorm(a: torch.Tensor, w: torch.Tensor, bias: Optional[torch.Tensor], gain: Optional[torch.Tensor],
                     shift: Optional[torch.Tensor], x: torch.Tensor, x_out: torch.Tensor,
                     x_bf16: Optional[torch.Tensor], eps: float = 1e-5) -> torch.Tensor:
    lda, K = _rows(a)
    ldw, _ = _rows(w)
    M, N = a.shape[0], w.shape[0]
    assert a.dtype == w.dtype == torch.bfloat16 and x.dtype == x_out.dtype == torch.float32
    ldx, _ = _rows(x)
    ldo, _ = _rows(x_out)
    ldb = 0
    if x_bf16 is not None:
        assert x_bf16.dtype == torch.bfloat16
        ldb, _ = _rows(x_bf16)
    with _Timed("linear_layernorm_bf16", 2.0 * M * N * K):
        _check(load().aurora_hip_linear_layernorm(_ptr(a), lda, _ptr(w), ldw, _ptr(bias), _ptr(gain), _ptr(shift), _ptr(x),
                                                  ldx, _ptr(x_out), ldo, _ptr(x_bf16), ldb, M, N, K, eps, _stream()))
    return x_out


def linear_planes(a: torch.Tensor, w: torch.Tensor, bias: Optional[torch.Tensor], out: torch.Tensor, sel0: int = 0) -> torch.Tensor:
    M, K = a.shape
    N = w.shape[0]
    heads = out.shape[0]
    assert a.dtype == w.dtype == out.dtype == torch.bfloat16 and a.stride(1) == 1 and w.stride(1) == 1 and w.shape[1] == K
    assert out.dim() == 4 and out.shape[2:] == (3, 64) and out.shape[1] >= M and N == (3 - sel0) * 64 * heads
    assert out.stride(3) == 1 and out.stride(2) == 64 and out.stride(1) == 192
    c = out[0, 0, sel0]
    with _Timed("linear_bf16", 2.0 * M * N * K):
        _check(load().aurora_hip_linear_planes(_ptr(a), a.stride(0), _ptr(w), w.stride(0), _ptr(bias), _ptr(c), out.stride(0), heads,
                                               M, N, K, dtype_code(a.dtype), _stream()))
    return out


def window_attention(qkv: torch.Tensor, qkv_bias: Optional[torch.Tensor], out: torch.Tensor,
                     tok: torch.Tensor, grp: Optional[torch.Tensor], B: int, L: int, D: int,
                     heads: int, L_out: Optional[int] = None, planes: bool = False) -> torch.Tensor:
    L_out = L if L_out is None else L_out
    if planes:
        assert qkv.is_contiguous() and qkv.shape == (heads, B * L, 3, 64) and qkv.dtype == torch.bfloat16
        assert out.numel() == B * L_out * D and out.dtype == qkv.dtype and tok.dtype == torch.int32 and tok.dim() == 2
        n_windows, n_tok = tok.shape
        plane_stride = qkv.stride(0) if heads > 1 else B * L * 192
        with _Timed("window_attention_bf16", 4.0 * B * n_windows * n_tok * D * 2):
            _check(load().aurora_hip_window_attention_planes(_ptr(qkv), plane_stride, _ptr(qkv_bias), _ptr(out), _ptr(tok), _ptr(grp),
                                                             B, L, L_out, D, heads, n_windows, n_tok, dtype_code(qkv.dtype),
                                                             _stream()))
        return out
    assert qkv.is_contiguous() and out.is_contiguous() and qkv.numel() == B * L * 3 * D
    assert out.numel() == B * L_out * D and out.dtype == qkv.dtype
    assert tok.dtype == torch.int32 and tok.is_contiguous() and tok.dim() == 2
    assert grp is None or (grp.dtype == torch.uint8 and grp.shape == tok.shape and grp.is_contiguous())
    assert qkv_bias is None or (qkv_bias.dtype == torch.float32 and qkv_bias.numel() == 3 * D)
    n_windows, n_tok = tok.shape
    name = "window_attention_bf16" if qkv.dtype == torch.bfloat16 else "window_attention_f32"
    with _Timed(name, 4.0 * B * n_windows * n_tok * D * qkv.element_size()):
        _check(load().aurora_hip_window_attention(_ptr(qkv), _ptr(qkv_bias), _ptr(out), _ptr(tok), _ptr(grp),
                                                  B, L, L_out, D, heads, n_windows, n_tok,
                                                  dtype_code(qkv.dtype), _stream()))
    return out


def layernorm(y: torch.Tensor, gain: Optional[torch.Tensor], shift: Optional[torch.Tensor], *,
              res: Optional[torch.Tensor] = None, res_mod: int = 0,
              out_f32: Optional[torch.Tensor] = None, out_t: Optional[torch.Tensor] = None,
              eps: float = 1e-5, d: Optional[int] = None, split_t: bool = False, split_res: bool = False) -> None:
    ldy, dy = _rows(y)
    D = d if d is not None else dy
    M = y.shape[0]
    for v in (gain, shift):
        assert v is None or (v.dtype == torch.float32 and v.numel() >= D and v.is_contiguous())
    ldr = ldo = ldt = 0
    if res is not None:
        assert res.dtype == torch.float32
        ldr, _ = _rows(res)
    if out_f32 is not None:
        assert out_f32.dtype == torch.float32 and out_f32.shape[0] == M
        ldo, _ = _rows(out_f32)
    if out_t is not None:
        assert out_t.dtype == y.dtype and out_t.shape[0] == M
        ldt, _ = _rows(out_t)
    nbytes = M * D * (y.element_size() + (4 if res is not None else 0) + (4 if out_f32 is not None else 0)
                      + (y.element_size() if out_t is not None else 0))
    if split_t or split_res:
        assert y.dtype == torch.float32 and (out_t is not None) == split_t and (res is not None or not split_res)
        with _Timed("layernorm", float(nbytes)):
            _check(load().aurora_hip_layernorm_split(_ptr(y), ldy, _ptr(gain), _ptr(shift), _ptr(res), ldr, res_mod,
                                                     1 if split_res else 0, _ptr(out_f32), ldo, _ptr(out_t), ldt, M, D,
                                                     eps, _stream()))
        return
    with _Timed("layernorm", float(nbytes)):
        _check(load().aurora_hip_layernorm(_ptr(y), ldy, _ptr(gain), _ptr(shift), _ptr(res), ldr, res_mod,
                                           _ptr(out_f32), ldo, _ptr(out_t), ldt, M, D, eps,
                                           dtype_code(y.dtype), _stream()))


def merge_ln(x: torch.Tensor, ln_w: torch.Tensor, ln_b: torch.Tensor, out: torch.Tensor,
             B: int, C: int, H: int, W: int, D: int, eps: float = 1e-5) -> torch.Tensor:
    assert x.dtype == torch.float32 and x.is_contiguous() and x.numel() == B * C * H * W * D
    assert out.is_contiguous() and out.numel() == B * C * ((H + 1) // 2) * ((W + 1) // 2) * 4 * D
    with _Timed("merge_ln", 0.0):
        _check(load().aurora_hip_merge_ln(_ptr(x), _ptr(ln_w), _ptr(ln_b), _ptr(out), B, C, H, W, D, eps,
                                          dtype_code(out.dtype), _stream()))
    return out


def split_ln(y: torch.Tensor, ln_w: torch.Tensor, ln_b: torch.Tensor, out: torch.Tensor,
             B: int, C: int, H: int, W: int, Dq: int, crop_h: int, crop_w: int,
             eps: float = 1e-5) -> torch.Tensor:
    assert y.is_contiguous() and y.numel() == B * C * H * W * 4 * Dq and y.dtype == out.dtype
    assert out.is_contiguous() and out.numel() == B * C * (2 * H - crop_h) * (2 * W - crop_w) * Dq
    with _Timed("split_ln", 0.0):
        _check(load().aurora_hip_split_ln(_ptr(y), _ptr(ln_w), _ptr(ln_b), _ptr(out), B, C, H, W, Dq,
                                          crop_h, crop_w, eps, dtype_code(y.dtype), _stream()))
    return out


def patchify(desc: list[PatchVar], out: torch.Tensor, k_offset: int, k_total: int, B: int, T: int,
             n_lvl: int, Hp: int, Wp: int, P: int, absmax: Optional[torch.Tensor] = None) -> None:
    Kpad = out.shape[1]
    assert out.is_contiguous() and out.shape[0] == n_lvl * B * Hp * Wp
    assert absmax is None or (absmax.dtype == torch.float32 and absmax.numel() >= 1)
    arr = (PatchVar * len(desc))(*desc)
    with _Timed("patchify", 0.0):
        _check(load().aurora_hip_patchify_absmax(arr, len(desc), _ptr(out), Kpad, k_offset, k_total, B, T, n_lvl,
                                                 Hp, Wp, P, dtype_code(out.dtype), _ptr(absmax), _stream()))


def perceiver_attention(q: torch.Tensor, q_col_stride: int, kv: torch.Tensor, out: torch.Tensor,
                        B: int, cols_per_b: int, kv_bstride: int, kv_lstride: int, Lq: int, Lk: int,
                        heads: int, head_dim: int, pair_guard=None, skip_guard=None) -> torch.Tensor:
    assert q.is_contiguous() and kv.is_contiguous() and out.is_contiguous()
    assert q.dtype == kv.dtype == out.dtype
    word, limit = pair_guard if pair_guard is not None else (None, 0.0)
    sword, slimit = skip_guard if skip_guard is not None else (None, 0.0)
    with _Timed("perceiver_attention", 0.0):
        _check(load().aurora_hip_perceiver_attention_unless(_ptr(q), q_col_stride, _ptr(kv), _ptr(out), B,
                                                            cols_per_b, kv_bstride, kv_lstride, Lq, Lk, heads,
                                                            head_dim, dtype_code(q.dtype), _ptr(word), float(limit),
                                                            _ptr(sword), float(slimit), _stream()))
    return out


def perceiver_probs(q: torch.Tensor, kv: torch.Tensor, B: int, cols_per_b: int, kv_bstride: int, kv_lstride: int,
                    Lq: int, Lk: int, heads: int, head_dim: int, guard=None):
    assert q.is_contiguous() and kv.is_contiguous() and q.dtype == kv.dtype == torch.float32
    n_cols, inner = B * cols_per_b, heads * head_dim
    P = torch.zeros((n_cols, heads, 64), device=kv.device, dtype=torch.float32)
    Vp = torch.zeros((n_cols * Lk, inner), device=kv.device, dtype=torch.float32)
    word, limit = guard if guard is not None else (None, 0.0)
    with _Timed("perceiver_attention", 0.0):
        _check(load().aurora_hip_perceiver_probs(_ptr(q), _ptr(kv), _ptr(P), _ptr(Vp), B, cols_per_b, kv_bstride,
                                                 kv_lstride, Lq, Lk, heads, head_dim, _ptr(word), float(limit), _stream()))
    return P, Vp


def perceiver_attention_scores(vs: torch.Tensor, s_off: int, out: torch.Tensor, B: int, cols_per_b: int, kv_bstride: int,
                               kv_lstride: int, Lq: int, Lk: int, heads: int, head_dim: int, pair_guard=None,
                               skip_guard=None) -> torch.Tensor:
    assert vs.is_contiguous() and out.is_contiguous() and vs.dtype == out.dtype == torch.float32
    word, limit = pair_guard if pair_guard is not None else (None, 0.0)
    sword, slimit = skip_guard if skip_guard is not None else (None, 0.0)
    with _Timed("perceiver_attention", 0.0):
        _check(load().aurora_hip_perceiver_attention_scores(_ptr(vs), vs.shape[1], s_off, _ptr(out), B, cols_per_b, kv_bstride,
                                                            kv_lstride, Lq, Lk, heads, head_dim, _ptr(word), float(limit),
                                                            _ptr(sword), float(slimit), _stream()))
    return out


def perceiver_probs_scores(vs: torch.Tensor, s_off: int, B: int, cols_per_b: int, kv_bstride: int, kv_lstride: int,
                           Lq: int, Lk: int, heads: int, head_dim: int, guard=None):
    assert vs.is_contiguous() and vs.dtype == torch.float32
    n_cols, inner = B * cols_per_b, heads * head_dim
    P = torch.zeros((n_cols, heads, 64), device=vs.device, dtype=torch.float32)
    Vp = torch.zeros((n_cols * Lk, inner), device=vs.device, dtype=torch.float32)
    word, limit = guard if guard is not None else (None, 0.0)
    with _Timed("perceiver_attention", 0.0):
        _check(load().aurora_hip_perceiver_probs_scores(_ptr(vs), vs.shape[1], s_off, _ptr(P), _ptr(Vp), B, cols_per_b,
                                                        kv_bstride, kv_lstride, Lq, Lk, heads, head_dim, _ptr(word),
                                                        float(limit), _stream()))
    return P, Vp


def perceiver_out(Vp: torch.Tensor, w_pairs: torch.Tensor, P: torch.Tensor, out: torch.Tensor, n_cols: int, Lq: int,
                  Lk: int, heads: int, head_dim: int, bias: Optional[torch.Tensor] = None, guard=None) -> torch.Tensor:
    assert Vp.is_contiguous() and w_pairs.is_contiguous() and P.is_contiguous()
    ldo, N = _rows(out)
    word, limit = guard if guard is not None else (None, 0.0)
    with _Timed("perceiver_out", 2.0 * n_cols * Lk * N * heads * head_dim):
        _check(load().aurora_hip_perceiver_out(_ptr(Vp), _ptr(w_pairs), w_pairs.shape[1], _ptr(P), _ptr(bias), _ptr(out),
                                               ldo, n_cols, Lq, Lk, heads, head_dim, N, _ptr(word), float(limit),
                                               _stream()))
    return out


def assemble_tokens(surf: torch.Tensor, agg: torch.Tensor, pos_scale: torch.Tensor,
                    time_emb: torch.Tensor, out_f32: torch.Tensor, out_t: Optional[torch.Tensor],
                    B: int, Cl: int, L: int, D: int) -> None:
    for t in (surf, agg, pos_scale, time_emb, out_f32):
        assert t.dtype == torch.float32 and t.is_contiguous()
    code = BF16 if out_t is not None else F32
    with _Timed("assemble_tokens", 0.0):
        _check(load().aurora_hip_assemble_tokens(_ptr(surf), _ptr(agg), _ptr(pos_scale), _ptr(time_emb),
                                                 _ptr(out_f32), _ptr(out_t), B, Cl, L, D, code, _stream()))


def unpatchify(y: torch.Tensor, desc: list[UnpatchVar], B: int, n_lvl: int, Hp: int, Wp: int,
               P: int) -> None:
    ldy, _ = _rows(y)
    assert y.dtype == torch.float32
    arr = (UnpatchVar * len(desc))(*desc)
    with _Timed("unpatchify", 0.0):
        _check(load().aurora_hip_unpatchify(_ptr(y), ldy, arr, len(desc), B, n_lvl, Hp, Wp, P, _stream()))


def copy2d(src: torch.Tensor, dst: torch.Tensor, cols: Optional[int] = None) -> None:
    lds_, cs = _rows(src)
    ldd, _ = _rows(dst)
    assert src.dtype == dst.dtype and src.shape[0] == dst.shape[0]
    with _Timed("copy2d", 0.0):
        _check(load().aurora_hip_copy2d(_ptr(src), lds_, _ptr(dst), ldd, src.shape[0],
                                        cols if cols is not None else cs, dtype_code(src.dtype), _stream()))


def gather_rows(src: torch.Tensor, idx: torch.Tensor, dst: torch.Tensor) -> torch.Tensor:
    lds_, w = _rows(src)
    ldd, wd = _rows(dst)
    assert w == wd and src.dtype == dst.dtype and idx.dtype == torch.int32 and idx.is_contiguous()
    assert dst.shape[0] == idx.numel()
    es = src.element_size()
    with _Timed("gather_rows", 0.0):
        _check(load().aurora_hip_gather_rows(_ptr(src), lds_ * es, _ptr(idx), _ptr(dst), ldd * es, idx.numel(), w * es,
                                             _stream()))
    return dst


def convert(src: torch.Tensor, dst: torch.Tensor) -> torch.Tensor:
    assert src.is_contiguous() and dst.is_contiguous() and src.numel() == dst.numel()
    assert {src.dtype, dst.dtype} == {torch.float32, torch.bfloat16}
    with _Timed("convert", 0.0):
        _check(load().aurora_hip_convert(_ptr(src), _ptr(dst), src.numel(), dtype_code(src.dtype), _stream()))
    return dst


def regrid_plan(lat, lon, lat_new, lon_new) -> tuple[np.ndarray, np.ndarray, np.ndarray, np.ndarray]:
    lat, lon, lat_new, lon_new = (np.ascontiguousarray(x, dtype=np.float64) for x in (lat, lon, lat_new, lon_new))
    assert lat.ndim == lon.ndim == lat_new.ndim == lon_new.ndim == 1, "regrid_plan: coordinates must be vectors"
    rows, cols = np.zeros((len(lat_new), 2), np.int32), np.zeros((len(lon_new), 2), np.int32)
    row_w, col_w = np.zeros(len(lat_new)), np.zeros(len(lon_new))
# ... 535 lines not shown
                                                     workspace.numel(), _stream()))
    return values, valid, total


def probability_rows(members: list[list[torch.Tensor]], truth: list[torch.Tensor], thresholds: torch.Tensor,
                     below: bool = False) -> torch.Tensor:
    assert thresholds.is_cuda and thresholds.dtype == torch.float32 and thresholds.dim() == 2 and thresholds.is_contiguous(), \
        "probability_rows: thresholds must be a contiguous (n_planes, T) fp32 matrix on the device"
    dev, (n_thr_planes, T) = thresholds.device, thresholds.shape
    M = len(members)
    assert 2 <= M <= ENSEMBLE_MAX_MEMBERS, f"probability_rows: members must hold 2..{ENSEMBLE_MAX_MEMBERS} lists, got {M}"
    assert 1 <= T <= EVENT_MAX_THRESHOLDS, f"probability_rows: 1..{EVENT_MAX_THRESHOLDS} thresholds, got {T}"
    assert truth and all(len(fs) == len(truth) for fs in members), "probability_rows: the lists differ in length or are empty"
    n_lat, n_lon = truth[0].shape[-2:]
    lists = [(f"member {m}", fs) for m, fs in enumerate(members)] + [("truth", truth)]
    n, addresses = _plane_lists("probability_rows", lists, dev, "thresholds", n_lat, n_lon, like=-1)
    assert n == n_thr_planes, f"probability_rows: {n} planes but thresholds for {n_thr_planes}"
    rows = torch.empty(n, n_lat, T, 2, M + 1, dtype=torch.int32, device=dev)
    if n == 0:
        return rows
    with torch.cuda.device(dev):
        table = _plane_table("probability_rows", tuple(addresses), dev)
        base = table.data_ptr()
        with _Timed("probability_scores", 0.0):
            _check(load().aurora_hip_probability_scores(base, base + 8 * M * n, M, n, n_lat, n_lon, _ptr(thresholds), T,
                                                        1 if below else 0, _ptr(rows), _stream()))
    return rows


FIELD_STATS_MAX_SAMPLES, FIELD_STATS_MAX_THRESHOLDS = 64, 8
FIELD_STATS_STATE = {"n": (torch.int32, False), "origin": (torch.float32, False), "s1": (torch.float64, False),
                     "s2": (torch.float64, False), "vmin": (torch.float32, False), "vmax": (torch.float32, False),
                     "argmin": (torch.int32, False), "argmax": (torch.int32, False), "exceed": (torch.int32, True),
                     "run": (torch.int32, True), "longest": (torch.int32, True)}


def field_stats_update(samples: list[list[torch.Tensor]], ref: Optional[list[torch.Tensor]],
                       second: Optional[list[list[Optional[torch.Tensor]]]], thresholds: Optional[torch.Tensor], below: bool,
                       sample_index: torch.Tensor, state: dict[str, torch.Tensor]) -> None:
    S = len(samples)
    assert 1 <= S <= FIELD_STATS_MAX_SAMPLES, f"field_stats_update: 1..{FIELD_STATS_MAX_SAMPLES} samples a call, got {S}"
    assert samples[0], "field_stats_update: no fields"
    dev = sample_index.device
    assert sample_index.is_cuda and sample_index.dtype == torch.int64 and sample_index.numel() == 1, \
        "field_stats_update: sample_index must be one int64 on the device"
    n_lat, n_lon = samples[0][0].shape[-2:]
    lists = [(f"sample {s}", fs) for s, fs in enumerate(samples)] + ([("reference", ref)] if ref is not None else [])
    n, addresses = _plane_lists("field_stats_update", lists, dev, "sample_index", n_lat, n_lon)
    if second is not None:
        assert len(second) == S and all(len(fs) == len(samples[0]) for fs in second), \
            "field_stats_update: the second operands differ from the samples in number"
        for s, fs in enumerate(second):
            for v, p in zip(fs, samples[s]):
                if v is None:
                    addresses += [0] * (p.numel() // (n_lat * n_lon))
                    continue
                assert v.device == dev and v.shape == p.shape, "field_stats_update: a second operand differs from its sample"
                addresses += _plane_addresses("field_stats_update", [v], n_lat, n_lon, "second operand")
    T = 0
    if thresholds is not None:
        assert thresholds.device == dev and thresholds.dtype == torch.float32 and thresholds.dim() == 2 and \
            thresholds.is_contiguous() and thresholds.shape[0] == n, \
            f"field_stats_update: thresholds must be a contiguous ({n}, T) fp32 matrix on the device"
        T = thresholds.shape[1]
        assert T <= FIELD_STATS_MAX_THRESHOLDS, f"field_stats_update: at most {FIELD_STATS_MAX_THRESHOLDS} thresholds, got {T}"
    for name, (dt, per_thr) in FIELD_STATS_STATE.items():
        if per_thr and T == 0:
            continue
        t = state[name]
        want = (n, T, n_lat * n_lon) if per_thr else (n, n_lat * n_lon)
        assert t.device == dev and t.dtype == dt and t.is_contiguous() and t.numel() == int(np.prod(want)), \
            f"field_stats_update: state {name!r} must be contiguous {dt} of {want} on the device"
    if n == 0:
        return
    with torch.cuda.device(dev):
        table = _plane_table("field_stats_update", tuple(addresses), dev)
        base = table.data_ptr()
        ref_at = base + 8 * S * n if ref is not None else None
        second_at = base + 8 * (S + (ref is not None)) * n if second is not None else None
        arrays = [_ptr(state[k]) if (T or not per_thr) else None for k, (_, per_thr) in FIELD_STATS_STATE.items()]
        with _Timed("field_stats", float(n * n_lat * n_lon * (4 * S + 2 * (36 + 12 * T)))):
            _check(load().aurora_hip_field_stats_update(base, ref_at, second_at, S, n, n_lat * n_lon,
                                                        _ptr(thresholds) if T else None, T, 1 if below else 0,
                                                        _ptr(sample_index), *arrays, _stream()))


DIAGNOSTICS_MAX_LEVELS = 64


def diagnostics(n_lat: int, n_lon: int, *, u: Optional[list[torch.Tensor]] = None, v: Optional[list[torch.Tensor]] = None,
                vo: Optional[list[torch.Tensor]] = None, div: Optional[list[torch.Tensor]] = None,
                ws: Optional[list[torch.Tensor]] = None, row_table: Optional[torch.Tensor] = None, L: float = 0.0,
                wrap: bool = False, q: Optional[list[torch.Tensor]] = None, col_u: Optional[list[torch.Tensor]] = None,
                col_v: Optional[list[torch.Tensor]] = None, tcwv: Optional[list[torch.Tensor]] = None,
                ivtu: Optional[list[torch.Tensor]] = None, ivtv: Optional[list[torch.Tensor]] = None,
                ivt: Optional[list[torch.Tensor]] = None, level_w: Optional[torch.Tensor] = None) -> None:
    groups = (("u", u), ("v", v), ("vo", vo), ("div", div), ("ws", ws), ("q", q), ("col_u", col_u), ("col_v", col_v),
              ("tcwv", tcwv), ("ivtu", ivtu), ("ivtv", ivtv), ("ivt", ivt))
    tensors = [t for _, fs in groups if fs is not None for t in fs if t is not None]
    if not tensors:
        return
    dev = tensors[0].device
    assert all(t.device == dev for t in tensors), "diagnostics: every tensor must be on one device"
    for what, t, shape in (("row_table", row_table, (n_lat, 4)), ("level_w", level_w, None)):
        assert t is None or (t.device == dev and t.dtype == torch.float64 and t.is_contiguous() and
                             (t.dim() == 1 if shape is None else tuple(t.shape) == shape)), \
            f"diagnostics: {what} must be a contiguous fp64 {'vector' if shape is None else shape} on the device of the fields"
    addr = {}
    for what, fs in groups:
        if fs is None:
            continue
        if what in ("vo", "div", "ws") and any(t is None for t in fs):
            assert u is not None and len(fs) == len(u), f"diagnostics: {what} with None entries must have an entry per u entry"
            addr[what] = [a for t, like in zip(fs, u) for a in
                          ([0] * (like.numel() // (n_lat * n_lon)) if t is None else _plane_addresses("diagnostics", [t], n_lat, n_lon, what))]
        else:
            addr[what] = _plane_addresses("diagnostics", fs, n_lat, n_lon, what)
    n_wind, n_cols = len(addr.get("u", ())), 0
    C = 0 if level_w is None else level_w.shape[0]
    for what in ("v", "vo", "div", "ws"):
        assert what not in addr or len(addr[what]) == n_wind, f"diagnostics: {what} holds {len(addr[what])} planes, u {n_wind}"
    if q is not None:
        assert C >= 1 and len(addr["q"]) % C == 0, f"diagnostics: q holds {len(addr['q'])} planes, which is no multiple of the {C} level weights"
        n_cols = len(addr["q"]) // C
        for what in ("col_u", "col_v"):
            assert what not in addr or len(addr[what]) == n_cols * C, f"diagnostics: {what} holds {len(addr[what])} planes, q {n_cols * C}"
        for what in ("tcwv", "ivtu", "ivtv", "ivt"):
            assert what not in addr or len(addr[what]) == n_cols, f"diagnostics: {what} holds {len(addr[what])} planes for {n_cols} columns"
    if n_wind == 0 and n_cols == 0:
        return
    with torch.cuda.device(dev):
        order = [what for what, _ in groups if what in addr]
        table = _plane_table("diagnostics", tuple(a for what in order for a in addr[what]), dev)
        at, first = {}, table.data_ptr()
        for what in order:
            at[what], first = first, first + 8 * len(addr[what])
        moved = 4.0 * n_lat * n_lon * (n_wind * (2 + sum(k in addr for k in ("vo", "div", "ws"))) +
                                       n_cols * (C * (1 + sum(k in addr for k in ("col_u", "col_v"))) +
                                                 sum(k in addr for k in ("tcwv", "ivtu", "ivtv", "ivt"))))
        with _Timed("diagnostics", moved):
            _check(load().aurora_hip_diagnostics(at.get("u"), at.get("v"), at.get("vo"), at.get("div"), at.get("ws"), n_wind,
                                                 _ptr(row_table), float(L), 1 if wrap else 0, at.get("q"), at.get("col_u"),
                                                 at.get("col_v"), at.get("tcwv"), at.get("ivtu"), at.get("ivtv"), at.get("ivt"),
                                                 n_cols, C, _ptr(level_w), n_lat, n_lon, _stream()))


_PD =ctypes.POINTER(ctypes.c_double)
_PF = ctypes.POINTER(ctypes.c_float)
_PS = ctypes.POINTER(ctypes.c_char_p)


class HipTuning(ctypes.Structure):
    _fields_ = [("fuse_ln", c_int32), ("band_split_attention", c_int32), ("qkv_planes", c_int32), ("split_k", c_int32),
                ("perceiver_reassoc", c_int32), ("score_weights", c_int32), ("reserved", c_int32 * 2)]


def tuning_from_env() -> HipTuning:
    t = HipTuning()

    def value(var: str, allowed: tuple[int, ...]):
        raw = os.environ.get(var)
        if raw is None:
            return None
        try:
            v = int(raw.strip())
        except ValueError:
            v = None
        if v not in allowed:
            raise ValueError(f"{var}={raw!r}: expected one of {', '.join(map(str, allowed))}")
        return v

    v = value("AURORA_FUSE_LN", (0, 1, 2))
    if v is not None:
        t.fuse_ln = v + 1
    for field, var in (("band_split_attention", "AURORA_BAND_SPLIT_ATTENTION"), ("qkv_planes", "AURORA_QKV_PLANES"),
                       ("split_k", "AURORA_SPLIT_K"), ("perceiver_reassoc", "AURORA_PERCEIVER_REASSOC"),
                       ("score_weights", "AURORA_SCORE_WEIGHTS")):
        v = value(var, (0, 1))
        if v is not None:
            setattr(t, field, 2 if v else 1)
    return t


class HipConfig(ctypes.Structure):
    _fields_ = [("embed_dim", c_int32), ("patch_size", c_int32), ("latent_levels", c_int32), ("num_heads", c_int32),
                ("n_stages", c_int32), ("encoder_depths", c_int32 * 4), ("encoder_heads", c_int32 * 4),
                ("decoder_depths", c_int32 * 4), ("decoder_heads", c_int32 * 4), ("window", c_int32 * 3),
                ("enc_depth", c_int32), ("dec_depth", c_int32), ("perceiver_ln_eps", c_float),
                ("max_history", c_int32), ("timestep_hours", ctypes.c_double), ("stabilise_level_agg", c_int32),
                ("use_lora", c_int32), ("lora_steps", c_int32), ("lora_mode", c_int32), ("autocast", c_int32),
                ("n_surf", c_int32), ("n_static", c_int32), ("n_atmos", c_int32),
                ("surf_vars", _PS), ("static_vars", _PS), ("atmos_vars", _PS),
                ("variant", c_int32), ("n_level_condition", c_int32), ("level_condition", _PD),
                ("dynamic_vars", c_int32), ("atmos_static_vars", c_int32), ("clamp_at_first_step", c_int32),
                ("simulate_indexing_bug", c_int32),
                ("n_separate_perceiver", c_int32), ("separate_perceiver", _PS),
                ("n_modulation_heads", c_int32), ("modulation_heads", _PS),
                ("difference_history", ctypes.POINTER(c_int32)),
                ("n_positive_surf", c_int32), ("positive_surf_vars", _PS),
                ("n_positive_atmos", c_int32), ("positive_atmos_vars", _PS),
                ("n_surf_inputs", c_int32), ("surf_inputs", _PS),
                ("n_density", c_int32), ("density_channel_surf_vars", _PS),
                ("n_angle", c_int32), ("angle_surf_vars", _PS), ("tuning", HipTuning)]


class HipHaloMsg(ctypes.Structure):
    _fields_ = [("peer", c_int32), ("reserved", c_int32), ("offset", c_int64), ("bytes", c_int64)]


HALO_POST_FN = ctypes.CFUNCTYPE(c_int, c_void_p, ctypes.POINTER(HipHaloMsg), c_int32, ctypes.POINTER(HipHaloMsg), c_int32,
                                c_void_p)
HALO_WAIT_FN = ctypes.CFUNCTYPE(c_int, c_void_p, c_void_p)


class HipBand(ctypes.Structure):
    _fields_ = [("rank", c_int32), ("world", c_int32), ("post", HALO_POST_FN), ("wait", HALO_WAIT_FN), ("user", c_void_p)]


class HipGrid(ctypes.Structure):
    _fields_ = [("n_lat", c_int32), ("n_lon", c_int32), ("lat", _PD), ("lon", _PD), ("n_levels", c_int32),
                ("levels", _PD), ("levels_float32", c_int32), ("surf_loc", _PD), ("surf_scale", _PD),
                ("static_loc", _PD), ("static_scale", _PD), ("atmos_loc", _PD), ("atmos_scale", _PD),
                ("pos_encoding", _PF), ("scale_encoding", _PF)]


class HipStepIO(ctypes.Structure):
    _fields_ = [("B", c_int32), ("T", c_int32), ("surf", ctypes.POINTER(c_void_p)), ("surf_strides", c_int64 * 4),
                ("stat", ctypes.POINTER(c_void_p)), ("static_strides", c_int64 * 2),
                ("atmos", ctypes.POINTER(c_void_p)), ("atmos_strides", c_int64 * 5),
                ("out_surf", ctypes.POINTER(c_void_p)), ("out_atmos", ctypes.POINTER(c_void_p)),
                ("rollout_step", c_int32)]


class HipProfileEntry(ctypes.Structure):
    _fields_ = [("kernel", ctypes.c_char_p), ("launches", c_int64), ("ms", ctypes.c_double), ("work", ctypes.c_double)]


class HipPlanInfo(ctypes.Structure):
    _fields_ = [("n_windows", c_int32), ("win_tokens", c_int32), ("n_own", c_int32), ("n_halo", c_int32),
                ("n_interior", c_int32), ("recv_offset", c_int32 * 2), ("recv_count", c_int32 * 2),
                ("send_count", c_int32 * 2), ("has_groups", c_int32)]


PROFILE_KINDS = ("linear_bf16", "linear_f32", "window_attention_bf16", "layernorm", "merge_ln", "split_ln", "patchify",
                 "perceiver_attention", "assemble_tokens", "unpatchify", "copy2d", "absmax", "linear_layernorm_bf16",
                 "gather_rows", "perceiver_out")

_SIGNATURES.update({
    "aurora_hip_profile_begin": (c_int, [c_void_p, ctypes.c_uint32]),
    "aurora_hip_profile_end": (c_int, [c_void_p, ctypes.POINTER(HipProfileEntry), c_int, ctypes.POINTER(c_int)]),
    "aurora_hip_profile_end_list": (c_int, [c_void_p, ctypes.POINTER(HipProfileEntry), c_int, ctypes.POINTER(c_int)]),
    "aurora_hip_create": (c_int, [ctypes.POINTER(HipConfig), ctypes.POINTER(c_void_p)]),
    "aurora_hip_destroy": (None, [c_void_p]),
    "aurora_hip_pack_weights": (c_int, [c_void_p, ctypes.c_char_p, c_void_p, ctypes.POINTER(c_int64), c_int, c_int, c_int]),
    "aurora_hip_finalize": (c_int, [c_void_p, c_void_p]),
    "aurora_hip_save_packed": (c_int, [c_void_p, ctypes.c_char_p, c_void_p]),
    "aurora_hip_load_packed": (c_int, [c_void_p, ctypes.c_char_p]),
    "aurora_hip_precompute": (c_int, [c_void_p, ctypes.POINTER(HipGrid), c_void_p]),
    "aurora_hip_set_time": (c_int, [c_void_p, _PD, c_int, c_void_p]),
    "aurora_hip_step": (c_int, [c_void_p, ctypes.POINTER(HipStepIO), c_void_p]),
    "aurora_hip_workspace_bytes": (c_int64, [c_void_p]),
    "aurora_hip_guard_words": (c_int, [c_void_p, ctypes.POINTER(c_float), c_void_p]),
    "aurora_hip_abi_sizes": (c_int, [ctypes.POINTER(c_int32), c_int]),
    "aurora_hip_generation": (c_int64, [c_void_p]),
    "aurora_hip_output_vars": (c_int, [c_void_p, _PS, c_int]),
    "aurora_hip_set_time_ex": (c_int, [c_void_p, _PD, ctypes.POINTER(c_int32), c_int, c_void_p]),
    "aurora_hip_set_band": (c_int, [c_void_p, ctypes.POINTER(HipBand)]),
    "aurora_hip_band_rows": (c_int, [c_void_p, ctypes.POINTER(c_int32), ctypes.POINTER(c_int32)]),
    "aurora_hip_band_staging_bytes": (c_int64, [c_void_p]),
    "aurora_hip_set_band_staging": (c_int, [c_void_p, c_void_p, c_void_p, c_int64]),
    "aurora_hip_pos_scale_encoding": (c_int, [_PD, _PD, c_int, c_int, c_int, c_int, _PF, _PF]),
    "aurora_hip_band_partition": (c_int, [c_int, ctypes.POINTER(c_int32), ctypes.POINTER(c_int32), c_int, c_int, c_int,
                                          ctypes.POINTER(c_int32), ctypes.POINTER(c_int32)]),
    "aurora_hip_band_plan": (c_int, [ctypes.POINTER(c_int32), ctypes.POINTER(c_int32), c_int, c_int, c_int,
                                     ctypes.POINTER(c_int32), ctypes.POINTER(HipPlanInfo), c_void_p, c_void_p, c_void_p,
                                     c_void_p]),
})
EXPORTED_SYMBOLS = tuple(_SIGNATURES)
```

### include/aurora_hip.h

```cpp
#ifndef AURORA_HIP_H
#define AURORA_HIP_H

#include <stddef.h>
#include <stdint.h>

#ifdef __cplusplus
extern "C" {
#endif

#define AURORA_F32 0
#define AURORA_BF16 1
#define AURORA_F64 2

#define AURORA_OK 0
#define AURORA_E_ARG (-1)
#define AURORA_E_LAUNCH (-2)

#define AURORA_ACT_NONE 0
#define AURORA_ACT_GELU 1
#define AURORA_ACT_SILU 2

const char* aurora_hip_last_error(void);
int aurora_hip_version(void);

int aurora_hip_linear(const void* A, int64_t lda, const void* W, int64_t ldw, const float* bias,
                      void* C, int64_t ldc, void* C2, int64_t ldc2,
                      const float* residual, int64_t ldr,
                      int64_t M, int N, int K, int dtype, int act, void* stream);

int aurora_hip_linear_ex(const void* A, int64_t lda, const void* W, int64_t ldw, const float* bias,
                         void* C, int64_t ldc, void* C2, int64_t ldc2,
                         const float* residual, int64_t ldr,
                         int64_t M, int N, int K, int dtype, int act,
                         int f32_gemm, const float* guard, float guard_limit, void* stream);
int aurora_hip_default_f32_gemm(void);
int aurora_hip_linear_batched(const void* A, int64_t lda, const void* W, int64_t ldw, const float* bias, void* C, int64_t ldc,
                              int64_t M, int N, int K, int dtype, int act, int f32_gemm, const float* guard,
                              float guard_limit, int batch, int64_t stride_a, int64_t stride_w, int64_t stride_bias,
                              int64_t stride_c, void* stream);

#define AURORA_PLAN_F32_THREE 0
#define AURORA_PLAN_F32_TWO 1
#define AURORA_PLAN_F32_PP 2
#define AURORA_PLAN_F32_PP_W 3
#define AURORA_PLAN_F32_PP_AW 4
#define AURORA_PLAN_F32_PP_W_TALL 5
#define AURORA_PLAN_F32_PP_AW_TALL 6
#define AURORA_PLAN_TILE128 7
#define AURORA_PLAN_RING 8
#define AURORA_PLAN_RING_MID 9
#define AURORA_PLAN_PP 10
#define AURORA_PLAN_PP_SPLITK 11
#define AURORA_PLAN_A4 12
int aurora_hip_linear_plan(int64_t M, int N, int K, int dtype, int f32_gemm, int has_guard, int batch, int64_t ldc,
                           int64_t c_addr, int64_t ldc2, int64_t c2_addr, int64_t ldr, int64_t residual_addr,
                           int64_t workspace_bytes, int n_tickets, int split, int64_t plane_stride, int plane_heads,
                           int cus, int32_t* plan_out);

int64_t aurora_hip_linear_workspace(int64_t M, int N, int K, int dtype);
int aurora_hip_linear_ws(const void* A, int64_t lda, const void* W, int64_t ldw, const float* bias, void* C, int64_t ldc,
                         void* C2, int64_t ldc2, const float* residual, int64_t ldr, int64_t M, int N, int K, int dtype,
                         int act, void* workspace, int64_t workspace_bytes, int32_t* tickets, int n_tickets, int split,
                         void* stream);

int aurora_hip_linear_planes(const void* A, int64_t lda, const void* W, int64_t ldw, const float* bias, void* C,
                             int64_t plane_stride, int heads, int64_t M, int N, int K, int dtype, void* stream);

#define AURORA_F32_A_SPLIT 4
#define AURORA_F32_W_SPLIT 8
#define AURORA_F32_C_SPLIT 16
int aurora_hip_split_f16(const float* src, int64_t ld_src, void* dst, int64_t ld_dst, int64_t rows, int K,
                         float scale, void* stream);

int aurora_hip_absmax(const float* x, int64_t n, float* out, void* stream);
int aurora_hip_absmax_fold(const float* x, int64_t n, float* out, void* stream);
int aurora_hip_zero_words(float* words, int n, void* stream);

int aurora_hip_window_attention(const void* qkv, const float* qkv_bias, void* out,
                                const int32_t* tok, const uint8_t* grp,
                                int B, int64_t L, int64_t L_out, int D, int heads, int n_windows,
                                int win_tokens, int dtype, void* stream);
int aurora_hip_window_attention_planes(const void* qkv, int64_t plane_stride, const float* qkv_bias, void* out,
                                       const int32_t* tok, const uint8_t* grp,
                                       int B, int64_t L, int64_t L_out, int D, int heads, int n_windows,
                                       int win_tokens, int dtype, void* stream);

int aurora_hip_layernorm(const void* y, int64_t ldy, const float* gain, const float* shift,
                         const float* res, int64_t ldr, int64_t res_mod,
                         float* out_f32, int64_t ldo, void* out_t, int64_t ldt,
                         int64_t M, int D, float eps, int dtype, void* stream);
int aurora_hip_linear_layernorm(const void* A, int64_t lda, const void* W, int64_t ldw, const float* bias,
                                const float* gain, const float* shift,
                                const float* x_in, int64_t ldx, float* x_out, int64_t ldo,
                                void* x_bf16, int64_t ldb, int64_t M, int N, int K, float eps, void* stream);

int aurora_hip_layernorm_split(const float* y, int64_t ldy, const float* gain, const float* shift,
                               const void* res, int64_t ldr, int64_t res_mod, int res_is_split,
                               float* out_f32, int64_t ldo, void* out_split, int64_t ld_split,
                               int64_t M, int D, float eps, void* stream);

int aurora_hip_merge_ln(const float* x, const float* ln_w, const float* ln_b, void* out,
                        int B, int C, int H, int W, int D, float eps, int dtype, void* stream);

int aurora_hip_split_ln(const void* y, const float* ln_w, const float* ln_b, void* out,
                        int B, int C, int H, int W, int Dq, int crop_h, int crop_w, float eps,
                        int dtype, void* stream);

typedef struct aurora_patch_var {
  const float* src;
  int64_t stride_b;
  int64_t stride_t;
  int64_t stride_c;
  int64_t stride_h;
  int64_t stride_w;
  const float* loc;
  const float* inv_scale;
  int32_t transform;
  float tw0, tw1, tb;
} aurora_patch_var;

int aurora_hip_patchify(const aurora_patch_var* desc, int n_vars, void* out, int64_t Kpad,
                        int k_offset, int K_total, int B, int T, int n_lvl, int Hp, int Wp, int P,
                        int dtype, void* stream);
int aurora_hip_patchify_absmax(const aurora_patch_var* desc, int n_vars, void* out, int64_t Kpad,
                               int k_offset, int K_total, int B, int T, int n_lvl, int Hp, int Wp, int P,
                               int dtype, float* absmax, void* stream);

int aurora_hip_perceiver_attention(const void* q, int64_t q_col_stride, const void* kv, void* out,
                                   int B, int64_t cols_per_b, int64_t kv_bstride, int64_t kv_lstride,
                                   int Lq, int Lk, int heads, int head_dim, int dtype, void* stream);
int aurora_hip_perceiver_attention_ex(const void* q, int64_t q_col_stride, const void* kv, void* out,
                                      int B, int64_t cols_per_b, int64_t kv_bstride, int64_t kv_lstride,
                                      int Lq, int Lk, int heads, int head_dim, int dtype,
                                      const float* pair_guard, float pair_limit, void* stream);
int aurora_hip_perceiver_attention_unless(const void* q, int64_t q_col_stride, const void* kv, void* out,
                                          int B, int64_t cols_per_b, int64_t kv_bstride, int64_t kv_lstride,
                                          int Lq, int Lk, int heads, int head_dim, int dtype,
                                          const float* pair_guard, float pair_limit, const float* skip_guard,
                                          float skip_limit, void* stream);

int aurora_hip_perceiver_out_supported(int Lq, int Lk, int heads, int head_dim, int N);
int aurora_hip_perceiver_probs(const float* q, const float* kv, float* P, void* Vp, int B, int64_t cols_per_b,
                               int64_t kv_bstride, int64_t kv_lstride, int Lq, int Lk, int heads, int head_dim,
                               const float* guard, float guard_limit, void* stream);
int aurora_hip_perceiver_attention_scores(const float* vs, int64_t ld_vs, int s_off, void* out, int B, int64_t cols_per_b,
                                          int64_t kv_bstride, int64_t kv_lstride, int Lq, int Lk, int heads, int head_dim,
                                          const float* pair_guard, float pair_limit, const float* skip_guard, float skip_limit,
                                          void* stream);
int aurora_hip_perceiver_probs_scores(const float* vs, int64_t ld_vs, int s_off, float* P, void* Vp, int B, int64_t cols_per_b,
                                      int64_t kv_bstride, int64_t kv_lstride, int Lq, int Lk, int heads, int head_dim,
                                      const float* guard, float guard_limit, void* stream);
int aurora_hip_perceiver_out(const void* Vp, const void* W_pairs, int64_t ldw, const float* P, const float* bias,
                             float* out, int64_t ldo, int64_t n_cols, int Lq, int Lk, int heads, int head_dim, int N,
                             const float* guard, float guard_limit, void* stream);

int aurora_hip_assemble_tokens(const float* surf, const float* agg, const float* pos_scale,
                               const float* time_emb, float* out_f32, void* out_t,
                               int B, int Cl, int64_t L, int D, int dtype, void* stream);

typedef struct aurora_unpatch_var {
  float* dst;
  const float* loc;
  const float* scale;
  int32_t clamp_min0;
  int32_t col0;
  int32_t lvl_stride;
  int32_t mod_col0;
  const float* prev;
  int64_t prev_sb, prev_sc, prev_sh;
  const float* inv_scale;
  uint32_t clamp_max1_levels;
  int32_t angle_col0;
  int32_t dens_col0;
  const float* mask;
  int64_t mask_sh;
  float mask_thresh;
} aurora_unpatch_var;

int aurora_hip_unpatchify(const float* y, int64_t ldy, const aurora_unpatch_var* desc, int n_vars,
                          int B, int n_lvl, int Hp, int Wp, int P, void* stream);

int aurora_hip_copy2d(const void* src, int64_t lds_, void* dst, int64_t ldd, int64_t rows,
                      int64_t cols, int dtype, void* stream);
int aurora_hip_gather_rows(const void* src, int64_t src_pitch_bytes, const int32_t* idx, void* dst,
                           int64_t dst_pitch_bytes, int64_t n_rows, int64_t row_bytes, void* stream);
int aurora_hip_convert(const void* src, void* dst, int64_t n, int src_dtype, void* stream);

typedef struct aurora_hip_model aurora_hip_model;

typedef struct aurora_hip_config {
  int32_t embed_dim, patch_size, latent_levels, num_heads;
  int32_t n_stages;
  int32_t encoder_depths[4], encoder_heads[4], decoder_depths[4], decoder_heads[4];
  int32_t window[3];
  int32_t enc_depth, dec_depth;
  float perceiver_ln_eps;
  int32_t max_history;
  double timestep_hours;
  int32_t stabilise_level_agg, use_lora, lora_steps, lora_mode;
  int32_t autocast;
  int32_t n_surf, n_static, n_atmos;
  const char* const* surf_vars;
  const char* const* static_vars;
  const char* const* atmos_vars;
  int32_t variant;
  int32_t n_level_condition;
  const double* level_condition;
  int32_t dynamic_vars, atmos_static_vars, clamp_at_first_step, simulate_indexing_bug;
  int32_t n_separate_perceiver;  const char* const* separate_perceiver;
  int32_t n_modulation_heads;    const char* const* modulation_heads;
  const int32_t* difference_history;
  int32_t n_positive_surf;       const char* const* positive_surf_vars;
  int32_t n_positive_atmos;      const char* const* positive_atmos_vars;
  int32_t n_surf_inputs;         const char* const* surf_inputs;
  int32_t n_density;             const char* const* density_channel_surf_vars;
  int32_t n_angle;               const char* const* angle_surf_vars;
  struct aurora_hip_tuning {
    int32_t fuse_ln;
    int32_t band_split_attention;
    int32_t qkv_planes;
    int32_t split_k;
    int32_t perceiver_reassoc;
    int32_t score_weights;
    int32_t reserved[2];
  } tuning;
} aurora_hip_config;

typedef struct aurora_hip_grid {
  int32_t n_lat, n_lon;
  const double* lat;
  const double* lon;
  int32_t n_levels;
  const double* levels;
  int32_t levels_float32;
  const double* surf_loc;
  const double* surf_scale;
  const double* static_loc;
  const double* static_scale;
  const double* atmos_loc;
  const double* atmos_scale;
  const float* pos_encoding;
  const float* scale_encoding;
} aurora_hip_grid;

typedef struct aurora_hip_step_io {
  int32_t B, T;
  const float* const* surf;
  int64_t surf_strides[4];
  const float* const* stat;
  int64_t static_strides[2];
  const float* const* atmos;
  int64_t atmos_strides[5];
  float* const* out_surf;
  float* const* out_atmos;
  int32_t rollout_step;
} aurora_hip_step_io;

int aurora_hip_create(const aurora_hip_config* config, aurora_hip_model** out);
void aurora_hip_destroy(aurora_hip_model* model);
int aurora_hip_pack_weights(aurora_hip_model* model, const char* name, const void* data, const int64_t* shape, int ndim,
                            int dtype, int on_device);
int aurora_hip_finalize(aurora_hip_model* model, void* stream);
int aurora_hip_save_packed(aurora_hip_model* model, const char* path, void* stream);
int aurora_hip_load_packed(aurora_hip_model* model, const char* path);
int aurora_hip_precompute(aurora_hip_model* model, const aurora_hip_grid* grid, void* stream);
int aurora_hip_pos_scale_encoding(const double* lat, const double* lon, int n_lat, int n_lon, int patch_size,
                                  int embed_dim, float* pos_out, float* scale_out);
int aurora_hip_set_time(aurora_hip_model* model, const double* time_hours, int B, void* stream);
int aurora_hip_step(aurora_hip_model* model, const aurora_hip_step_io* io, void* stream);
int64_t aurora_hip_workspace_bytes(const aurora_hip_model* model);
#define AURORA_F16_SAFE_RANGE 16384.0f
int aurora_hip_guard_words(const aurora_hip_model* model, float out[4], void* stream);
int64_t aurora_hip_generation(const aurora_hip_model* model);
int aurora_hip_abi_sizes(int32_t* out, int capacity);
int aurora_hip_output_vars(const aurora_hip_model* model, const char** names, int capacity);
int aurora_hip_set_time_ex(aurora_hip_model* model, const double* time_hours, const int32_t* calendar, int B, void* stream);

typedef struct aurora_hip_halo_msg {
  int32_t peer;
  int32_t reserved;
  int64_t offset;
  int64_t bytes;
} aurora_hip_halo_msg;
typedef int (*aurora_hip_halo_post_fn)(void* user, const aurora_hip_halo_msg* sends, int32_t n_sends,
                                       const aurora_hip_halo_msg* recvs, int32_t n_recvs, void* stream);
typedef int (*aurora_hip_halo_wait_fn)(void* user, void* stream);
typedef struct aurora_hip_band {
  int32_t rank, world;
  aurora_hip_halo_post_fn post;
  aurora_hip_halo_wait_fn wait;
  void* user;
} aurora_hip_band;
int aurora_hip_set_band(aurora_hip_model* model, const aurora_hip_band* band);
int aurora_hip_band_rows(const aurora_hip_model* model, int32_t* row0, int32_t* row1);
int64_t aurora_hip_band_staging_bytes(const aurora_hip_model* model);
int aurora_hip_set_band_staging(aurora_hip_model* model, void* send, void* recv, int64_t staging_bytes);
typedef struct aurora_hip_plan_info {
  int32_t n_windows, win_tokens, n_own, n_halo, n_interior;
  int32_t recv_offset[2], recv_count[2], send_count[2];
  int32_t has_groups;
} aurora_hip_plan_info;
int aurora_hip_band_partition(int n_stages, const int32_t res0[3], const int32_t window[3], int world, int rank, int stage,
                              int32_t* h0, int32_t* h1);
int aurora_hip_band_plan(const int32_t res[3], const int32_t window[3], int shifted, int world, int rank,
                         const int32_t* rows, aurora_hip_plan_info* info, int32_t* tok, uint8_t* grp,
                         int32_t* send_idx_prev, int32_t* send_idx_next);

typedef struct aurora_hip_profile_entry {
  const char* kernel;
  int64_t launches;
  double ms;
  double work;
} aurora_hip_profile_entry;
int aurora_hip_profile_begin(aurora_hip_model* model, uint32_t kind_mask);
int aurora_hip_profile_end(aurora_hip_model* model, aurora_hip_profile_entry* out, int capacity, int* n_out);
int aurora_hip_profile_end_list(aurora_hip_model* model, aurora_hip_profile_entry* out, int capacity, int* n_out);

int aurora_hip_regrid_plan(const double* lat, int n_lat, const double* lon, int n_lon, const double* lat_new, int n_lat_new,
                           const double* lon_new, int n_lon_new, int32_t* rows, double* row_w, int32_t* cols,
                           double* col_w);
int aurora_hip_regrid(const void* const* src_planes, int src_dtype, float* const* dst_planes, int n_planes, int n_lat,
                      int n_lon, const int32_t* rows, const double* row_w, int n_rows_out, const int32_t* cols,
                      const double* col_w, int n_cols_out, void* stream);

int aurora_hip_conservative_regrid(const void* const* src_planes, int src_dtype, float* const* dst_planes, int n_planes,
                                   int n_lat, int n_lon, int n_rows_out, int n_cols_out, const int32_t* row_first,
                                   const int32_t* row_count, const double* row_w, const double* row_measure,
                                   const int32_t* col_first, const int32_t* col_count, const double* col_w,
                                   const double* col_measure, double min_valid, void* stream);

size_t aurora_hip_scores_workspace_bytes(int n_planes, int n_lat, int n_lon);
int aurora_hip_scores(const float* const* pred_planes, const float* const* truth_planes, const float* const* clim_planes,
                      int n_planes, int n_lat, int n_lon, const double* row_w, double* sums, void* workspace, void* stream);

size_t aurora_hip_ensemble_scores_workspace_bytes(int n_members, int n_planes, int n_lat, int n_lon);
int aurora_hip_ensemble_scores(const float* const* member_planes, const float* const* truth_planes, int n_members, int n_planes,
                               int n_lat, int n_lon, const double* row_w, double* sums, int64_t* hist, void* workspace,
                               void* stream);

int aurora_hip_ensemble_quantiles(const float* const* member_planes, const float* const* truth_planes, int n_members,
                                  int n_planes, int n_lat, int n_lon, const double* q, int n_q, float* quantiles, int8_t* rank,
                                  void* stream);

size_t aurora_hip_spectra_workspace_bytes(int n_planes, int n_lat, int n_lon, int n_bands, int has_truth);
int aurora_hip_spectra(const float* const* pred_planes, const float* const* truth_planes, int n_planes, int n_lat, int n_lon,
                       int n_bands, const double* band_w, const double* twiddle, double* power, int64_t* rows, void* workspace,
                       size_t workspace_bytes, void* stream);

size_t aurora_hip_event_scores_workspace_bytes(int n_planes, int n_lat, int n_lon, int n_thresholds, int n_scales);
int aurora_hip_event_scores(const float* const* pred_planes, const float* const* truth_planes, int n_planes, int n_lat,
                            int n_lon, const float* thresholds, int n_thresholds, const int32_t* scales, int n_scales, int below,
                            int64_t* rowsums, int64_t* valid, void* workspace, size_t workspace_bytes, void* stream);

int aurora_hip_field_stats_update(const float* const* sample_planes, const float* const* ref_planes,
                                  const float* const* second_planes, int n_samples, int n_planes, int64_t n_points,
                                  const float* thresholds, int n_thresholds, int below, int64_t* sample_index, int32_t* n,
                                  float* origin, double* s1, double* s2, float* vmin, float* vmax, int32_t* argmin,
                                  int32_t* argmax, int32_t* exceed, int32_t* run, int32_t* longest, void* stream);

int aurora_hip_probability_scores(const float* const* member_planes, const float* const* truth_planes, int n_members,
                                  int n_planes, int n_lat, int n_lon, const float* thresholds, int n_thresholds, int below,
                                  int32_t* rows, void* stream);

size_t aurora_hip_conditional_scores_workspace_bytes(int n_planes, int n_lat, int n_lon, int n_edges);
int aurora_hip_conditional_scores(const float* const* pred_planes, const float* const* truth_planes,
                                  const float* const* centre_planes, const float* const* scale_planes, int n_planes, int n_lat,
                                  int n_lon, const float* edges, int n_edges, int by_pred, const double* row_w, double* sums,
                                  void* workspace, void* stream);

int aurora_hip_diagnostics(const float* const* wind_u, const float* const* wind_v, float* const* vo_planes,
                           float* const* div_planes, float* const* ws_planes, int n_wind, const double* row_table, double L,
                           int wrap, const float* const* q_planes, const float* const* col_u, const float* const* col_v,
                           float* const* tcwv_planes, float* const* ivtu_planes, float* const* ivtv_planes,
                           float* const* ivt_planes, int n_cols, int n_levels, const double* level_w, int n_lat, int n_lon,
                           void* stream);

size_t aurora_hip_region_scores_workspace_bytes(int n_planes, int n_lat, int n_lon, int n_regions);
// ... 32 lines not shown
```

Before: 7.953 forecast-steps/s.

## Fuse decoder's final LayerNorm, residual add and output-head GEMM into one kernel

Adds a kernel that applies the last de-aggregation LayerNorm plus the split-f16 residual, writes the normalised rows into LDS as hi/lo f16 pairs, and multiplies them against pre-packed head weights with f16 MFMA (three-term split). The resampler now leaves its last LayerNorm open so the separate LN pass and the head linear run as one launch. The aim is to cut a full write and reread of the latent activations and one kernel launch in the decoder tail. It needs a weight-packing step, relies on warp specialisation inside the kernel, and carries precision risk from the split-f16 arithmetic.

```diff
diff --git a/aurora_amd/build.py b/aurora_amd/build.py
--- a/aurora_amd/build.py
+++ b/aurora_amd/build.py
@@ -9,7 +9,7 @@
 PKG = Path(__file__).resolve().parent
 CSRC = PKG / "csrc"
 LIB = PKG / "_lib" / "libaurora_hip.so"
-SOURCES = ("runtime.hip", "gemm.hip", "gemm_f32.hip", "gemm_ln512.hip", "gemm_a4.hip", "attention.hip", "norm.hip", "embed.hip", "perceiver_attention.hip", "perceiver_out.hip", "band.hip",
+SOURCES = ("runtime.hip", "gemm.hip", "gemm_f32.hip", "gemm_ln512.hip", "gemm_a4.hip", "attention.hip", "norm.hip", "decoder_tail.hip", "embed.hip", "perceiver_attention.hip", "perceiver_out.hip", "band.hip",
            "model.hip", "model_weights.hip", "model_grid.hip", "step.hip", "regrid.hip", "conservative_regrid.hip", "planes.hip", "scores.hip", "ensemble_scores.hip", "ensemble_quantiles.hip", "spectra.hip", "event_scores.hip",
            "field_stats.hip", "probability_scores.hip", "diagnostics.hip", "conditional_scores.hip", "region_scores.hip", "objects.hip", "field_quantiles.hip", "object_matches.hip", "nearest_event.hip")
 ARCH = "gfx950"
diff --git a/aurora_amd/csrc/decoder_tail.hip b/aurora_amd/csrc/decoder_tail.hip
--- /dev/null
+++ b/aurora_amd/csrc/decoder_tail.hip
@@ -0,0 +1,316 @@
+#include <algorithm>
+
+#include "common.h"
+
+namespace aurora {
+namespace {
+
+typedef _Float16 f16x8_t __attribute__((ext_vector_type(8)));
+
+constexpr int TAIL_RING = 8, TAIL_ROWS = 32, TAIL_THREADS = 512, TAIL_SLOTS = 4, TAIL_WAVE_ROWS = 8, TAIL_MAX_D = 1024;
+
+struct TailArgs {
+  const float* y; int64_t ldy; const float* gain; const float* shift;
+  const char* res; int64_t ldr;
+  const u32x4* w;
+  const float* bias;
+  float* out; int64_t ldo;
+  int64_t M; int D; int n_cols; float eps; int64_t n_tiles;
+};
+
+__host__ __device__ inline int tail_k_steps(int D) { return ((D >> 5) + TAIL_RING - 1) / TAIL_RING * TAIL_RING; }
+
+struct TailRow { float v[4][4]; u32x2 h[4], l[4]; };
+
+__device__ __forceinline__ void lds_barrier() {
+  asm volatile("s_waitcnt lgkmcnt(0)" ::: "memory");
+  __builtin_amdgcn_s_barrier();
+  asm volatile("" ::: "memory");
+}
+
+__device__ __forceinline__ f32x4 tail_mma(u32x4 a, u32x4 b, f32x4 c) {
+  return __builtin_amdgcn_mfma_f32_16x16x32_f16(__builtin_bit_cast(f16x8_t, a), __builtin_bit_cast(f16x8_t, b), c, 0, 0, 0);
+}
+
+template <int NF, int DEPTH, int PASSES>
+__global__ __launch_bounds__(TAIL_THREADS, 2) void ln_heads_kernel(const TailArgs p) {
+  extern __shared__ __attribute__((aligned(16))) char smem[];
+  const int lane = threadIdx.x & 63;
+  const int wave = __builtin_amdgcn_readfirstlane(threadIdx.x >> 6);
+  const bool normalises = wave < 4;
+  const int n_pieces = p.D >> 2, k_steps = tail_k_steps(p.D);
+  const int row_bytes = k_steps * 128 + 16;
+  const int64_t stride = gridDim.x;
+  int64_t tile = blockIdx.x;
+
+  const int pw = wave & 3;
+  TailRow slot[TAIL_SLOTS];
+  float gn[4][4], sh[4][4];
+  auto request = [&](TailRow& r, int64_t row) {
+    row = row < p.M ? row : p.M - 1;
+    const float* yr = p.y + row * p.ldy;
+    const char* rr = p.res + row * p.ldr * 4;
+#pragma unroll
+    for (int i = 0; i < 4; ++i) {
+        const int e = min(lane + 64 * i, n_pieces - 1) * 4;
+        load4(yr + e, r.v[i]);
+        const char* s = rr + (e & ~31) * 4 + (e & 31) * 2;
+        r.h[i] = *reinterpret_cast<const u32x2*>(s);
+        r.l[i] = *reinterpret_cast<const u32x2*>(s + 64);
+      }
+  };
+  auto normalise = [&](const TailRow& r, int lds_row) {
+    float s = 0.f;
+#pragma unroll
+    for (int i = 0; i < 4; ++i)
+      if (lane + 64 * i < n_pieces) s += (r.v[i][0] + r.v[i][1]) + (r.v[i][2] + r.v[i][3]);
+    const float inv_d = 1.0f / p.D;
+    const float mean = wave_sum(s) * inv_d;
+    float q = 0.f;
+#pragma unroll
+    for (int i = 0; i < 4; ++i)
+      if (lane + 64 * i < n_pieces) {
+#pragma unroll
+        for (int j = 0; j < 4; ++j) {
+          const float d = r.v[i][j] - mean;
+          q = fmaf(d, d, q);
+        }
+      }
+    const float rstd = rsqrtf(wave_sum(q) * inv_d + p.eps);
+    char* lrow = smem + lds_row * row_bytes;
+#pragma unroll
+    for (int i = 0; i < 4; ++i) {
+      const int e = (lane + 64 * i) * 4;
+      if (lane + 64 * i < n_pieces) {
+        float o[4];
+#pragma unroll
+        for (int j = 0; j < 4; ++j) {
+          float t = (r.v[i][j] - mean) * rstd;
+          if (p.gain) t *= gn[i][j];
+          if (p.shift) t += sh[i][j];
+          o[j] = t;
+        }
+        auto half = [](uint32_t w, int hi) { return (float)__builtin_bit_cast(_Float16, (uint16_t)(hi ? w >> 16 : w & 0xffffu)); };
+        const uint32_t hw[2] = {r.h[i].x, r.h[i].y}, lw[2] = {r.l[i].x, r.l[i].y};
+#pragma unroll
+        for (int j = 0; j < 4; ++j) o[j] += half(hw[j >> 1], j & 1) + half(lw[j >> 1], j & 1);
+        uint32_t h0, h1, l0, l1;
+        split_pair_f16(o[0], o[1], h0, l0);
+        split_pair_f16(o[2], o[3], h1, l1);
+        const bool odd = (lane & 1) != 0;
+        auto swap1 = [](uint32_t x) { return (uint32_t)__builtin_amdgcn_update_dpp(0, (int)x, 0xB1, 0xf, 0xf, true); };
+        const uint32_t r0 = swap1(odd ? h0 : l0), r1 = swap1(odd ? h1 : l1);
+        const int e8 = e & ~7;
+        char* d = lrow + (e8 & ~31) * 4 + (e8 & 31) * 2 + (odd ? 64 : 0);
+        *reinterpret_cast<u32x4*>(d) = odd ? u32x4{r0, r1, l0, l1} : u32x4{h0, h1, r0, r1};
+      }
+    }
+  };
+
+  const int cw = wave & 3, rf = cw & 1, nh = cw >> 1;
+  const int i16 = lane & 15, g = lane >> 4;
+  constexpr int NFT = 2 * NF * PASSES;
+  u32x4 bh[DEPTH][NF], bl[DEPTH][NF];
+  float bias_r[NF][4];
+  const int ld_cols = (p.n_cols + 3) & ~3;
+  static_assert(TAIL_RING % DEPTH == 0, "a ring slot must meet the same K-steps in every pass");
+  int fetch_k = 0, fetch_pass = 0;
+  auto fetch_w = [&](int d) {
+    const u32x4* src = p.w + ((int64_t)(fetch_k * NFT + (nh * PASSES + fetch_pass) * NF) * 2) * 64 + lane;
+#pragma unroll
+    for (int f = 0; f < NF; ++f) {
+      bh[d][f] = src[(2 * f) * 64];
+      bl[d][f] = src[(2 * f + 1) * 64];
+    }
+    const bool wrap = fetch_k + 1 == k_steps;
+    fetch_k = wrap ? 0 : fetch_k + 1;
+    if (PASSES > 1) fetch_pass = !wrap ? fetch_pass : fetch_pass + 1 == PASSES ? 0 : fetch_pass + 1;
+  };
+  auto bias_of = [&](int fbase, int f, float (&b)[4]) {
+    const int col = (fbase + f) * 16 + 4 * g;
+#pragma unroll
+    for (int t = 0; t < 4; ++t) b[t] = (p.bias != nullptr && col + t < p.n_cols) ? p.bias[col + t] : 0.f;
+  };
+
+  if (k_steps * 32 > p.D) {
+    const int pad = (k_steps * 32 - p.D) >> 2;
+    for (int id = threadIdx.x; id < TAIL_ROWS * pad; id += TAIL_THREADS)
+      *reinterpret_cast<u32x4*>(smem + (id / pad) * row_bytes + p.D * 4 + (id % pad) * 16) = u32x4{0, 0, 0, 0};
+  }
+  if (normalises) {
+#pragma unroll
+    for (int i = 0; i < 4; ++i) {
+      const int e = min(lane + 64 * i, n_pieces - 1) * 4;
+      if (p.gain) load4(p.gain + e, gn[i]);
+      if (p.shift) load4(p.shift + e, sh[i]);
+    }
+#pragma unroll
+    for (int s = 0; s < TAIL_SLOTS; ++s) request(slot[s], tile * TAIL_ROWS + pw * TAIL_WAVE_ROWS + s);
+    for (; tile < p.n_tiles; tile += stride) {
+#pragma unroll
+      for (int j = 0; j < TAIL_WAVE_ROWS; ++j) {
+        TailRow& r = slot[j % TAIL_SLOTS];
+        normalise(r, pw * TAIL_WAVE_ROWS + j);
+        const int64_t next = j + TAIL_SLOTS < TAIL_WAVE_ROWS ? tile * TAIL_ROWS + pw * TAIL_WAVE_ROWS + j + TAIL_SLOTS
+                                                             : (tile + stride) * TAIL_ROWS + pw * TAIL_WAVE_ROWS + j + TAIL_SLOTS - TAIL_WAVE_ROWS;
+        request(r, next);
+      }
+      lds_barrier();
+      lds_barrier();
+    }
+    return;
+  }
+
+  if constexpr (PASSES == 1) {
+#pragma unroll
+    for (int f = 0; f < NF; ++f) bias_of(nh * NF, f, bias_r[f]);
+  }
+  const char* xrow = smem + (rf * 16 + i16) * row_bytes + g * 16;
+#pragma unroll
+  for (int d = 0; d < DEPTH; ++d) fetch_w(d);
+  for (; tile < p.n_tiles; tile += stride) {
+    lds_barrier();
+    const int64_t m = tile * TAIL_ROWS + rf * 16 + i16;
+#pragma unroll 1
+    for (int pass = 0; pass < PASSES; ++pass) {
+      const int fbase = (nh * PASSES + pass) * NF;
+      f32x4 acc[NF];
+#pragma unroll
+      for (int f = 0; f < NF; ++f) acc[f] = f32x4{0.f, 0.f, 0.f, 0.f};
+      for (int k0 = 0; k0 < k_steps; k0 += DEPTH) {
+#pragma unroll
+        for (int d = 0; d < DEPTH; ++d) {
+          const int k = k0 + d;
+          {
+            const u32x4 xh = *reinterpret_cast<const u32x4*>(xrow + k * 128);
+            const u32x4 xl = *reinterpret_cast<const u32x4*>(xrow + k * 128 + 64);
+#pragma unroll
+            for (int f = 0; f < NF; ++f) acc[f] = tail_mma(bl[d][f], xh, acc[f]);
+#pragma unroll
+            for (int f = 0; f < NF; ++f) acc[f] = tail_mma(bh[d][f], xl, acc[f]);
+#pragma unroll
+            for (int f = 0; f < NF; ++f) acc[f] = tail_mma(bh[d][f], xh, acc[f]);
+            __builtin_amdgcn_sched_barrier(0);
+            fetch_w(d);
+            __builtin_amdgcn_sched_barrier(0);
+          }
+        }
+      }
+#pragma unroll
+      for (int f = 0; f < NF; ++f) {
+        const int col = (fbase + f) * 16 + 4 * g;
+        float b[4];
+        if constexpr (PASSES == 1) { b[0] = bias_r[f][0]; b[1] = bias_r[f][1]; b[2] = bias_r[f][2]; b[3] = bias_r[f][3]; }
+        else bias_of(fbase, f, b);
+        if (m < p.M && col < ld_cols)
+          *reinterpret_cast<f32x4*>(p.out + m * p.ldo + col) =
+              f32x4{fmaf(acc[f].x, 0.015625f, b[0]), fmaf(acc[f].y, 0.015625f, b[1]), fmaf(acc[f].z, 0.015625f, b[2]),
+                    fmaf(acc[f].w, 0.015625f, b[3])};
+      }
+    }
+    lds_barrier();
+  }
+}
+
+__global__ __launch_bounds__(256) void pack_heads_kernel(const float* __restrict__ w, int64_t ldw, int n_cols, int K, int width,
+                                                         u32x4* __restrict__ dst) {
+  const int nft = width >> 4;
+  const int64_t id = (int64_t)blockIdx.x * 256 + threadIdx.x;
+  if (id >= (int64_t)tail_k_steps(K) * nft * 64) return;
+  const int lane = (int)(id & 63);
+  const int64_t kf = id >> 6;
+  const int f = (int)(kf % nft), k32 = (int)(kf / nft);
+  const int n = 16 * f + (lane & 15), k = 32 * k32 + 8 * (lane >> 4);
+  uint32_t h[4] = {0, 0, 0, 0}, l[4] = {0, 0, 0, 0};
+  if (n < n_cols && k < K) {
+    const f32x4 a = *reinterpret_cast<const f32x4*>(w + n * ldw + k);
+    const f32x4 b = *reinterpret_cast<const f32x4*>(w + n * ldw + k + 4);
+    split_pair_f16(a.x * 64.0f, a.y * 64.0f, h[0], l[0]);
+    split_pair_f16(a.z * 64.0f, a.w * 64.0f, h[1], l[1]);
+    split_pair_f16(b.x * 64.0f, b.y * 64.0f, h[2], l[2]);
+    split_pair_f16(b.z * 64.0f, b.w * 64.0f, h[3], l[3]);
+  }
+  dst[(kf * 2) * 64 + lane] = u32x4{h[0], h[1], h[2], h[3]};
+  dst[(kf * 2 + 1) * 64 + lane] = u32x4{l[0], l[1], l[2], l[3]};
+}
+
+struct TailForm { int nf, passes; };
+bool tail_form(int n_cols, TailForm& t) {
+  if (n_cols < 1 || n_cols > 512) return false;
+  const int half = (n_cols + 31) / 32;
+  t.passes = (half + 3) / 4;
+  t.nf = (half + t.passes - 1) / t.passes;
+  return true;
+}
+
+template <int NF, int DEPTH, int PASSES>
+void launch_tail(const TailArgs& p, unsigned grid, size_t lds, hipStream_t stream) {
+  once_per_device([] {
+    (void)hipFuncSetAttribute((const void*)ln_heads_kernel<NF, DEPTH, PASSES>, hipFuncAttributeMaxDynamicSharedMemorySize,
+                              TAIL_ROWS * (tail_k_steps(TAIL_MAX_D) * 128 + 16));
+  });
+  hipLaunchKernelGGL((ln_heads_kernel<NF, DEPTH, PASSES>), dim3(grid), dim3(TAIL_THREADS), lds, stream, p);
+}
+
+}
+}
+
+using namespace aurora;
+
+extern "C" int aurora_hip_layernorm_heads_width(int n_cols) {
+  TailForm t;
+  return tail_form(n_cols, t) ? 32 * t.nf * t.passes : 0;
+}
+
+extern "C" int64_t aurora_hip_pack_heads_bytes(int n_cols, int K) {
+  const int width = aurora_hip_layernorm_heads_width(n_cols);
+  return K > 0 && K % 32 == 0 ? (int64_t)tail_k_steps(K) * (width >> 4) * 2048 : 0;
+}
+
+extern "C" int aurora_hip_layernorm_heads_applies(int two_term, int groups, int D, int n_cols) {
+  return two_term != 0 && groups == 1 && D > 0 && D % 32 == 0 && D <= TAIL_MAX_D && n_cols >= 1 && n_cols <= 512;
+}
+
+extern "C" int aurora_hip_pack_heads(const float* w, int64_t ldw, int n_cols, int K, void* dst, void* stream) {
+  const int width = aurora_hip_layernorm_heads_width(n_cols);
+  AURORA_CHECK_ARG(width > 0, "pack_heads: n_cols=%d must be in 1..512", n_cols);
+  AURORA_CHECK_ARG(w != nullptr && dst != nullptr && K > 0 && K % 32 == 0, "pack_heads: K=%d must be a positive multiple of 32", K);
+  AURORA_CHECK_ARG(ldw >= K && ldw % 4 == 0 && ((uintptr_t)w % 16) == 0 && ((uintptr_t)dst % 16) == 0, "pack_heads: strides / alignment");
+  const int64_t n = (int64_t)tail_k_steps(K) * (width >> 4) * 64;
+  hipLaunchKernelGGL(pack_heads_kernel, dim3((unsigned)((n + 255) / 256)), dim3(256), 0, as_stream(stream), w, ldw, n_cols, K, width,
+                     (u32x4*)dst);
+  return check_launch("pack_heads");
+}
+
+extern "C" int aurora_hip_layernorm_heads(const float* y, int64_t ldy, const float* gain, const float* shift, const void* res_split,
+                                          int64_t ldr, const void* w_packed, const float* bias, float* out, int64_t ldo, int64_t M,
+                                          int D, int n_cols, float eps, void* stream) {
+  TailForm t;
+  AURORA_CHECK_ARG(tail_form(n_cols, t), "layernorm_heads: n_cols=%d must be in 1..512", n_cols);
+  AURORA_CHECK_ARG(D > 0 && D % 32 == 0 && D <= TAIL_MAX_D, "layernorm_heads: D=%d must be a multiple of 32, <= %d", D, TAIL_MAX_D);
+  AURORA_CHECK_ARG(y != nullptr && res_split != nullptr && w_packed != nullptr && out != nullptr, "layernorm_heads: null operand");
+  AURORA_CHECK_ARG(ldy >= D && ldy % 4 == 0 && ((uintptr_t)y % 16) == 0, "layernorm_heads: unaligned input rows");
+  AURORA_CHECK_ARG(ldr >= D && ldr % 32 == 0 && ((uintptr_t)res_split % 16) == 0,
+                   "layernorm_heads: the pair-layout residual stride must be a multiple of 32, >= D");
+  AURORA_CHECK_ARG(ldo >= ((n_cols + 3) & ~3) && ldo % 4 == 0 && ((uintptr_t)out % 16) == 0 && ((uintptr_t)w_packed % 16) == 0 &&
+                       (gain == nullptr || (uintptr_t)gain % 16 == 0) && (shift == nullptr || (uintptr_t)shift % 16 == 0),
+                   "layernorm_heads: output stride (>= n_cols rounded up to 4, a multiple of 4) / alignment");
+  if (M <= 0) return AURORA_OK;
+  const int64_t n_tiles = (M + TAIL_ROWS - 1) / TAIL_ROWS;
+  TailArgs p{y, ldy, gain, shift, (const char*)res_split, ldr, (const u32x4*)w_packed, bias, out, ldo, M, D, n_cols, eps, n_tiles};
+  const unsigned grid = (unsigned)std::min<int64_t>(n_tiles, device_cus());
+  const size_t lds = (size_t)TAIL_ROWS * (tail_k_steps(D) * 128 + 16);
+  hipStream_t s = as_stream(stream);
+  switch (t.passes * 10 + t.nf) {
+    case 11: launch_tail<1, 8, 1>(p, grid, lds, s); break;
+    case 12: launch_tail<2, 8, 1>(p, grid, lds, s); break;
+    case 13: launch_tail<3, 8, 1>(p, grid, lds, s); break;
+    case 14: launch_tail<4, 4, 1>(p, grid, lds, s); break;
+    case 23: launch_tail<3, 8, 2>(p, grid, lds, s); break;
+    case 24: launch_tail<4, 4, 2>(p, grid, lds, s); break;
+    case 33: launch_tail<3, 8, 3>(p, grid, lds, s); break;
+    case 34: launch_tail<4, 4, 3>(p, grid, lds, s); break;
+    default: launch_tail<4, 4, 4>(p, grid, lds, s); break;
+  }
+  return check_launch("layernorm_heads");
+}
diff --git a/aurora_amd/csrc/model.h b/aurora_amd/csrc/model.h
--- a/aurora_amd/csrc/model.h
+++ b/aurora_amd/csrc/model.h
@@ -131,6 +131,7 @@
   int groups = 1;
   DevBuf ws, bs;
   int n_pad = 0;
+  DevBuf wt;
 };
 
 struct DevTables { DevBuf tok, grp; int n_windows = 0, n_tok = 0; bool has_grp = false; };
@@ -205,6 +206,7 @@
   bool split_attention = false;
   bool qkv_planes = true;
   bool reassoc_out = true;
+  bool decoder_tail = true;
   bool score_weights = true;
 
   aurora::DevBuf abs_enc, dyn_planes, ctx_max;
@@ -252,7 +254,7 @@
 typedef aurora_hip_model Model;
 
 enum Kind { K_LINEAR_BF16, K_LINEAR_F32, K_WINDOW_ATTENTION, K_LAYERNORM, K_MERGE_LN, K_SPLIT_LN, K_PATCHIFY,
-            K_PERCEIVER_ATTENTION, K_ASSEMBLE, K_UNPATCHIFY, K_COPY2D, K_ABSMAX, K_LINEAR_LN, K_GATHER, K_PERCEIVER_OUT, K_COUNT };
+            K_PERCEIVER_ATTENTION, K_ASSEMBLE, K_UNPATCHIFY, K_COPY2D, K_ABSMAX, K_LINEAR_LN, K_GATHER, K_PERCEIVER_OUT, K_LAYERNORM_HEADS, K_COUNT };
 
 hipEvent_t take_event(Model& m);
 
diff --git a/aurora_amd/csrc/model.hip b/aurora_amd/csrc/model.hip
--- a/aurora_amd/csrc/model.hip
+++ b/aurora_amd/csrc/model.hip
@@ -199,6 +199,7 @@
     m->split_k = sw(tu.split_k, true, "split_k");
     m->reassoc_out = sw(tu.perceiver_reassoc, true, "perceiver_reassoc");
     m->score_weights = sw(tu.score_weights, true, "score_weights");
+    m->decoder_tail = sw(tu.decoder_tail, true, "decoder_tail");
     m->tickets = DevBuf(SPLIT_TICKETS * sizeof(int32_t));
     hip_ok(hipMemset(m->tickets.p, 0, SPLIT_TICKETS * sizeof(int32_t)), "hipMemset");
     *out = m.release();
@@ -299,7 +300,7 @@
 namespace {
 const char* const KIND_NAMES[K_COUNT] = {"linear_bf16", "linear_f32", "window_attention_bf16", "layernorm", "merge_ln",
                                          "split_ln", "patchify", "perceiver_attention", "assemble_tokens", "unpatchify",
-                                         "copy2d", "absmax", "linear_layernorm_bf16", "gather_rows", "perceiver_out"};
+                                         "copy2d", "absmax", "linear_layernorm_bf16", "gather_rows", "perceiver_out", "layernorm_heads"};
 }
 
 extern "C" int aurora_hip_profile_begin(aurora_hip_model* m, uint32_t kind_mask) {
diff --git a/aurora_amd/csrc/model_weights.hip b/aurora_amd/csrc/model_weights.hip
--- a/aurora_amd/csrc/model_weights.hip
+++ b/aurora_amd/csrc/model_weights.hip
@@ -122,6 +122,12 @@
   }
   hg.ws = presplit(padded.f(), n_pad, D2, D2, 128, hg.groups);
   hg.n_pad = n_pad;
+  hg.wt = DevBuf();
+  if (hg.ws.p && aurora_hip_layernorm_heads_applies(1, hg.groups, D2, n)) {
+    hg.wt = DevBuf((size_t)aurora_hip_pack_heads_bytes(n, D2));
+    ok(aurora_hip_pack_heads(hg.w.f(), D2, n, D2, hg.wt.p, nullptr));
+    hip_ok(hipDeviceSynchronize(), "pack head weights");
+  }
 }
 
 }
diff --git a/aurora_amd/csrc/step.hip b/aurora_amd/csrc/step.hip
--- a/aurora_amd/csrc/step.hip
+++ b/aurora_amd/csrc/step.hip
@@ -25,7 +25,7 @@
 }
 
 void resampler_mlp(Model& m, Launcher& L, const Resampler::Layer& ly, const LayerSpace& sp, const float* o, const float* res,
-                   int64_t res_mod, float* lat1, char* S, float* y, int64_t n_rows, float eps, bool y_pairs) {
+                   int64_t res_mod, float* lat1, char* S, float* y, int64_t n_rows, float eps, bool y_pairs, bool skip_ln2) {
   const int Dd = ly.dim;
   if (sp.pairs)
     timed(m, L.stream, K_LAYERNORM, 0.0, [&] {
@@ -43,6 +43,7 @@
     L.linear(fc1.activation(AURORA_ACT_GELU).f32_mode(sp.pairs ? all | AURORA_F32_C_SPLIT : ly.f16_mode));
     L.linear(fc2.f32_mode(sp.pairs ? all : ly.f16_mode));
   }
+  if (skip_ln2) return;
   if (sp.pairs)
     timed(m, L.stream, K_LAYERNORM, 0.0, [&] {
       return aurora_hip_layernorm_split(y, Dd, ly.ln2_w, ly.ln2_b, lat1, Dd, 0, 1, y_pairs ? nullptr : y, Dd, y_pairs ? y : nullptr, Dd,
@@ -53,7 +54,8 @@
 
 float* resampler(Model& m, Launcher& L, const Resampler& rs, const float* ctx, int64_t ctx_rows, int ctx_dim, const float* q0,
                  const float* latents0, int B, int64_t cols, int64_t kv_bstride, int64_t kv_lstride, int Lq, int Lk, int heads,
-                 float eps, const CtxGuard* cg = nullptr, bool out_pairs = false, int own_word = 0, bool scan_ctx = true) {
+                 float eps, const CtxGuard* cg = nullptr, bool out_pairs = false, int own_word = 0, bool scan_ctx = true,
+                 const float** open_lat1 = nullptr) {
   const int64_t n_cols = (int64_t)B * cols, n_rows = n_cols * Lq;
   const float* ctx_max = cg ? cg->word : m.ctx_max.f() + own_word;
   const float g_a = cg ? cg->a : 1.0f, g_c = cg ? cg->c : 0.0f;
@@ -70,6 +72,7 @@
     float* y = (float*)m.arena.take(sp.unit);
     const size_t after_y = m.arena.top;
     float* lat1 = (float*)m.arena.take(sp.unit);
+    const size_t after_lat1 = m.arena.top;
     char* S = (char*)m.arena.take(sp.s_bytes);
     float* kv = (float*)S;
     auto guarded = [&](const float* A, int64_t lda, const float* Wf, const void* Ws, float* C_, int64_t ldc, int64_t M_, int N_,
@@ -135,9 +138,10 @@
       });
       guarded(att, inner, ly.to_out, ly.to_out_s, o, Dd, n_rows, Dd, inner, lim_out, sp.att_pairs);
     }
-    resampler_mlp(m, L, ly, sp, o, i == 0 ? latents0 : lat, i == 0 ? Lq : 0, lat1, S, y, n_rows, eps,
-                  out_pairs && sp.pairs && i + 1 == rs.layers.size());
-    m.arena.top = after_y;
+    const bool last = i + 1 == rs.layers.size(), open = last && open_lat1 != nullptr && sp.pairs;
+    resampler_mlp(m, L, ly, sp, o, i == 0 ? latents0 : lat, i == 0 ? Lq : 0, lat1, S, y, n_rows, eps, out_pairs && sp.pairs && last, open);
+    if (open_lat1) *open_lat1 = open ? lat1 : nullptr;
+    m.arena.top = open ? after_lat1 : after_y;
     lat = y;
   }
   return lat;
@@ -607,14 +611,24 @@
   const auto& last_ly = rs.layers.back();
   const bool last_pairs = last_ly.fc1_s && last_ly.fc2_s && last_ly.dim % 32 == 0;
   const bool two_term = hg.n_pad > 0 && last_pairs && out_bound < F16_SAFE;
+  const int n_cols = (int)hg.names.size() * s.PP;
+  const bool fused = m.decoder_tail && hg.wt.p != nullptr && aurora_hip_layernorm_heads_applies(two_term, hg.groups, D2, n_cols) != 0;
+  const float* lat1 = nullptr;
   float* lat = resampler(m, s.L, rs, ctx, (int64_t)B * (Cl - 1) * Lp, D2, q, m.dec_queries.f(), B, Lp, (int64_t)(Cl - 1) * Lp, Lp, C,
-                         Cl - 1, m.perceiver_heads, m.ln_eps, nullptr, two_term, 3, scan_ctx);
-  const int n_a = two_term ? hg.n_pad : (int)hg.names.size() * s.PP, ld_a = round_up(n_a, 4);
+                         Cl - 1, m.perceiver_heads, m.ln_eps, nullptr, two_term, 3, scan_ctx, fused ? &lat1 : nullptr);
+  const int n_a = fused ? n_cols : two_term ? hg.n_pad : n_cols, ld_a = round_up(n_a, 4);
   const float* hw = two_term ? (const float*)hg.ws.p : hg.w.f();
   const float* hb = two_term ? hg.bs.f() : hg.b.f();
   const int mode = two_term ? (2 | AURORA_F32_A_SPLIT | AURORA_F32_W_SPLIT) : -1;
   float* y_a = (float*)m.arena.take((size_t)B * Lp * C * ld_a * 4);
-  if (hg.groups > 1)
+  if (fused) {
+    REQUIRE(lat1 != nullptr, "decoder: the last de-aggregation layer did not leave its LayerNorm open");
+    const int64_t rows = (int64_t)B * Lp * C;
+    timed(m, s.L.stream, K_LAYERNORM_HEADS, 2.0 * (double)rows * n_cols * D2, [&] {
+      return aurora_hip_layernorm_heads(lat, D2, last_ly.ln2_w, last_ly.ln2_b, lat1, D2, hg.wt.p, hg.b.f(), y_a, ld_a, rows, D2, n_cols,
+                                        m.ln_eps, s.L.stream);
+    });
+  } else if (hg.groups > 1)
     s.L.linear(LinearOp(lat, (int64_t)C * D2, hw, D2, hb, y_a, (int64_t)C * ld_a, (int64_t)B * Lp, n_a, D2, AURORA_F32)
                    .f32_mode(mode).batched(C, D2, (int64_t)n_a * D2, ld_a, ld_a));
   else
diff --git a/aurora_amd/engine/lib.py b/aurora_amd/engine/lib.py
--- a/aurora_amd/engine/lib.py
+++ b/aurora_amd/engine/lib.py
@@ -67,6 +67,12 @@
     "aurora_hip_split_f16": (c_int, [c_void_p, c_int64, c_void_p, c_int64, c_int64, c_int, c_float, c_void_p]),
     "aurora_hip_layernorm_split": (c_int, [c_void_p, c_int64, c_void_p, c_void_p, c_void_p, c_int64, c_int64, c_int,
                                            c_void_p, c_int64, c_void_p, c_int64, c_int64, c_int, c_float, c_void_p]),
+    "aurora_hip_layernorm_heads": (c_int, [c_void_p, c_int64, c_void_p, c_void_p, c_void_p, c_int64, c_void_p, c_void_p,
+                                           c_void_p, c_int64, c_int64, c_int, c_int, c_float, c_void_p]),
+    "aurora_hip_pack_heads": (c_int, [c_void_p, c_int64, c_int, c_int, c_void_p, c_void_p]),
+    "aurora_hip_pack_heads_bytes": (c_int64, [c_int, c_int]),
+    "aurora_hip_layernorm_heads_width": (c_int, [c_int]),
+    "aurora_hip_layernorm_heads_applies": (c_int, [c_int, c_int, c_int, c_int]),
     "aurora_hip_linear": (c_int, [c_void_p, c_int64, c_void_p, c_int64, c_void_p, c_void_p, c_int64,
                                   c_void_p, c_int64, c_void_p, c_int64, c_int64, c_int, c_int, c_int,
                                   c_int, c_void_p]),
@@ -525,6 +531,31 @@
                                            dtype_code(y.dtype), _stream()))
 
 
+def pack_heads(w: torch.Tensor) -> torch.Tensor:
+    assert w.dtype == torch.float32 and w.dim() == 2 and w.is_contiguous()
+    n_cols, K = w.shape
+    nbytes = load().aurora_hip_pack_heads_bytes(n_cols, K)
+    assert nbytes > 0, (n_cols, K)
+    dst = torch.empty(nbytes // 4, dtype=torch.int32, device=w.device)
+    _check(load().aurora_hip_pack_heads(_ptr(w), K, n_cols, K, _ptr(dst), _stream()))
+    return dst
+
+
+def layernorm_heads(y: torch.Tensor, gain: Optional[torch.Tensor], shift: Optional[torch.Tensor], res_split: torch.Tensor,
+                    w_packed: torch.Tensor, bias: Optional[torch.Tensor], out: torch.Tensor, n_cols: int,
+                    eps: float = 1e-5) -> torch.Tensor:
+    ldy, D = _rows(y)
+    ldr, _ = _rows(res_split)
+    ldo, _ = _rows(out)
+    M = y.shape[0]
+    assert y.dtype == torch.float32 and out.dtype == torch.float32 and out.shape[0] == M and res_split.shape[0] == M
+    assert bias is None or (bias.dtype == torch.float32 and bias.numel() >= n_cols)
+    with _Timed("layernorm_heads", float(M) * D * 8 + float(M) * n_cols * 4):
+        _check(load().aurora_hip_layernorm_heads(_ptr(y), ldy, _ptr(gain), _ptr(shift), _ptr(res_split), ldr, _ptr(w_packed),
+                                                 _ptr(bias), _ptr(out), ldo, M, D, n_cols, eps, _stream()))
+    return out
+
+
 def merge_ln(x: torch.Tensor, ln_w: torch.Tensor, ln_b: torch.Tensor, out: torch.Tensor,
              B: int, C: int, H: int, W: int, D: int, eps: float = 1e-5) -> torch.Tensor:
     assert x.dtype == torch.float32 and x.is_contiguous() and x.numel() == B * C * H * W * D
@@ -1366,7 +1397,7 @@
 
 class HipTuning(ctypes.Structure):
     _fields_ = [("fuse_ln", c_int32), ("band_split_attention", c_int32), ("qkv_planes", c_int32), ("split_k", c_int32),
-                ("perceiver_reassoc", c_int32), ("score_weights", c_int32), ("reserved", c_int32 * 2)]
+                ("perceiver_reassoc", c_int32), ("score_weights", c_int32), ("decoder_tail", c_int32), ("reserved", c_int32 * 1)]
 
 
 def tuning_from_env() -> HipTuning:
@@ -1389,7 +1420,7 @@
         t.fuse_ln = v + 1
     for field, var in (("band_split_attention", "AURORA_BAND_SPLIT_ATTENTION"), ("qkv_planes", "AURORA_QKV_PLANES"),
                        ("split_k", "AURORA_SPLIT_K"), ("perceiver_reassoc", "AURORA_PERCEIVER_REASSOC"),
-                       ("score_weights", "AURORA_SCORE_WEIGHTS")):
+                       ("score_weights", "AURORA_SCORE_WEIGHTS"), ("decoder_tail", "AURORA_DECODER_TAIL")):
         v = value(var, (0, 1))
         if v is not None:
             setattr(t, field, 2 if v else 1)
@@ -1458,7 +1489,7 @@
 
 PROFILE_KINDS = ("linear_bf16", "linear_f32", "window_attention_bf16", "layernorm", "merge_ln", "split_ln", "patchify",
                  "perceiver_attention", "assemble_tokens", "unpatchify", "copy2d", "absmax", "linear_layernorm_bf16",
-                 "gather_rows", "perceiver_out")
+                 "gather_rows", "perceiver_out", "layernorm_heads")
 
 _SIGNATURES.update({
     "aurora_hip_profile_begin": (c_int, [c_void_p, ctypes.c_uint32]),
diff --git a/include/aurora_hip.h b/include/aurora_hip.h
--- a/include/aurora_hip.h
+++ b/include/aurora_hip.h
@@ -98,6 +98,14 @@
                                const void* res, int64_t ldr, int64_t res_mod, int res_is_split,
                                float* out_f32, int64_t ldo, void* out_split, int64_t ld_split,
                                int64_t M, int D, float eps, void* stream);
+
+int aurora_hip_layernorm_heads(const float* y, int64_t ldy, const float* gain, const float* shift,
+                               const void* res_split, int64_t ldr, const void* w_packed, const float* bias,
+                               float* out, int64_t ldo, int64_t M, int D, int n_cols, float eps, void* stream);
+int aurora_hip_pack_heads(const float* w, int64_t ldw, int n_cols, int K, void* dst, void* stream);
+int64_t aurora_hip_pack_heads_bytes(int n_cols, int K);
+int aurora_hip_layernorm_heads_width(int n_cols);
+int aurora_hip_layernorm_heads_applies(int two_term, int groups, int D, int n_cols);
 
 int aurora_hip_merge_ln(const float* x, const float* ln_w, const float* ln_b, void* out,
                         int B, int C, int H, int W, int D, float eps, int dtype, void* stream);
@@ -222,7 +230,8 @@
     int32_t split_k;
     int32_t perceiver_reassoc;
     int32_t score_weights;
-    int32_t reserved[2];
+    int32_t decoder_tail;
+    int32_t reserved[1];
   } tuning;
 } aurora_hip_config;
 
```

Result: no change. 7.994 forecast-steps/s (median of 6 runs) (+0.5%).
